# Dave-he/unet-watermark

Hardware: AMD Instinct MI355X
Metric: train_images_per_sec (higher is better)
Workload: dtype f32 storage and accumulation; the convolution products of the encoder and decoder layers (3x3, 7x7 stem, stride-2 and 1x1 layers: forward, data gradients, and the weight gradients of the stride-1 3x3 layers and the stem) as fp16x3 splits - every fp32 operand = two fp16 halves (22 mantissa bits), a*b; 1 GPU; Unet-resnet34 512x512 bs16/GPU train step: fwd + Dice + bwd + Adam (BASELINE.json configs[1]); global_batch=16, parallelism=dp1, grad_allreduce=none

## Files before the change

### include/uwm.h

```cpp
#ifndef UWM_H
#define UWM_H
#include <stddef.h>
#include <stdint.h>

#ifdef __cplusplus
extern "C" {
#endif

typedef struct uwm_model* uwm_handle;
typedef void* uwm_stream;

enum { UWM_ENC_RESNET18 = 18, UWM_ENC_RESNET34 = 34, UWM_ENC_RESNET50 = 50,
       UWM_ENC_EFFICIENTNET_B0 = 100, UWM_ENC_EFFICIENTNET_B1 = 101, UWM_ENC_EFFICIENTNET_B2 = 102,
       UWM_ENC_EFFICIENTNET_B3 = 103, UWM_ENC_EFFICIENTNET_B4 = 104, UWM_ENC_EFFICIENTNET_B5 = 105,
       UWM_ENC_EFFICIENTNET_B6 = 106, UWM_ENC_EFFICIENTNET_B7 = 107 };
enum { UWM_ARCH_UNET = 0, UWM_ARCH_UNETPLUSPLUS = 1 };
enum { UWM_T_F32 = 0, UWM_T_I64 = 1, UWM_T_U8 = 2, UWM_T_I32 = 3 };
enum { UWM_KIND_CONV_W = 0, UWM_KIND_BIAS = 1, UWM_KIND_BN_GAMMA = 2, UWM_KIND_BN_BETA = 3,
       UWM_KIND_BN_MEAN = 4, UWM_KIND_BN_VAR = 5 };
enum { UWM_ARENA_PARAM = 0, UWM_ARENA_BUFFER = 1 };
enum { UWM_PREC_F32 = 0, UWM_PREC_BF16X3 = 1, UWM_PREC_BF16X3_ALL = 2, UWM_PREC_F16X3 = 3, UWM_PREC_F16X3_ALL = 4,
       UWM_PREC_F16X1 = 5, UWM_PREC_F16X3_BWD2 = 6 };

typedef struct {
// ... 49 lines not shown

size_t uwm_predict_workspace_bytes(uwm_handle h, int N, int H, int W, int with_logits);
int  uwm_predict_u8(uwm_handle h, const uint8_t* images, const float* mean, const float* std, float threshold,
                    int apply_sigmoid, int out_h, int out_w, uint8_t* mask, float* logits, void* workspace,
                    size_t workspace_bytes, int N, int H, int W, uwm_stream stream);

typedef struct { long long offset; int h, w; } uwm_image_desc;
enum { UWM_INTER_NEAREST = 0, UWM_INTER_LINEAR = 1 };
int  uwm_resize_u8(const uint8_t* src, size_t src_bytes, const uwm_image_desc* descs, int N, int C, int H, int W, int interp,
                   uint8_t* out, uwm_stream stream);
int  uwm_op_resize_norm_u8_nhwc4(const uint8_t* src, size_t src_bytes, const uwm_image_desc* descs, int N, int C, int H, int W,
                                 const float* mean, const float* std, float* out, uwm_stream stream);
int  uwm_resize_threshold_ragged(const float* logits, int ld, int N, int h, int w, const uwm_image_desc* out_descs, float threshold,
                                 int apply_sigmoid, uint8_t* mask, size_t mask_bytes, uwm_stream stream);
int  uwm_predict_images_u8(uwm_handle h, const uint8_t* src, size_t src_bytes, const uwm_image_desc* in_descs, const float* mean,
                           const float* std, float threshold, int apply_sigmoid, const uwm_image_desc* out_descs, uint8_t* mask,
                           size_t mask_bytes, float* logits, void* workspace, size_t workspace_bytes, int N, int H, int W,
                           uwm_stream stream);

int  uwm_backward(uwm_handle h, const float* dlogits, void* workspace, int stage_begin, int stage_end,
                  uwm_stream stream);

int  uwm_loss(const float* logits, int ld, const void* target, int target_dtype, long long npix,
              float w_dice, float w_bce, float smooth, float eps, void* scratch, float* loss_out,
              float* dlogits, int ldd, float grad_scale, uwm_stream stream);

int  uwm_loss_sums(const float* logits, int ld, const void* target, int target_dtype, long long npix, void* scratch,
                   uwm_stream stream);
int  uwm_loss_apply(const float* logits, int ld, const void* target, int target_dtype, long long npix, long long npix_total,
                    float w_dice, float w_bce, float smooth, float eps, const void* scratch, float* loss_out,
                    float* dlogits, int ldd, float grad_scale, uwm_stream stream);

int  uwm_stats(const float* logits, int ld, const void* target, int target_dtype, int N, long long hw,
               float threshold, int apply_sigmoid, long long* out, uwm_stream stream);
int  uwm_threshold(const float* logits, int ld, long long npix, float threshold, int apply_sigmoid,
                   uint8_t* mask, uwm_stream stream);

int  uwm_adam(float* p, const float* g, float* m, float* v, long long n, float lr, float beta1, float beta2,
              float eps, float weight_decay, long long step, float grad_scale, uwm_stream stream);
int  uwm_adam_clip(float* p, const float* g, float* m, float* v, long long n, float lr, float beta1, float beta2,
                   float eps, float weight_decay, long long step, float grad_scale, float max_norm, void* scratch,
                   uwm_stream stream);
int  uwm_adam_graph(float* p, const float* g, float* m, float* v, long long n, float* hyper, void* clip_scratch,
                    uwm_stream stream);
int  uwm_adamw(float* p, const float* g, float* m, float* v, long long n, float lr, float beta1, float beta2,
               float eps, float weight_decay, long long step, float grad_scale, uwm_stream stream);
int  uwm_adamw_clip(float* p, const float* g, float* m, float* v, long long n, float lr, float beta1, float beta2,
                    float eps, float weight_decay, long long step, float grad_scale, float max_norm, void* scratch,
                    uwm_stream stream);
int  uwm_adamw_graph(float* p, const float* g, float* m, float* v, long long n, float* hyper, void* clip_scratch,
                     uwm_stream stream);
int  uwm_sgd(float* p, const float* g, float* buf, long long n, float lr, float momentum, float weight_decay,
             long long step, float grad_scale, float max_norm, void* scratch, uwm_stream stream);
int  uwm_scale(float* p, long long n, float s, uwm_stream stream);
int  uwm_set_join_stream(uwm_handle h, uwm_stream stream);
int  uwm_allreduce_grads(uwm_handle h, void* nccl_comm, int stage_begin, int stage_end, uwm_stream stream);
float* uwm_grad_arena(uwm_handle h);
int  uwm_preprocess_u8(const uint8_t* images, int N, int H, int W, int C, const float* mean, const float* std,
                       const int* flags, float* out_nchw, uwm_stream stream);
int  uwm_preprocess_mask_u8(const uint8_t* masks, int N, int H, int W, int threshold, const int* flags, uint8_t* out,
                            uwm_stream stream);
typedef struct {
  int flags;
  int hue, sat, val;
  double minv[6];
  unsigned char lut[256];
} uwm_aug_desc;
int  uwm_augment_u8(const uint8_t* images, const uint8_t* masks, const uwm_aug_desc* descs, int N, int H, int W, int C,
                    const float* mean, const float* std, int mask_threshold, float* out_nchw, uint8_t* out_masks, uint8_t* out_u8,
                    uwm_stream stream);
int  uwm_set_winograd(int on);
int  uwm_set_winograd_mode(uwm_handle h, int mode);
int  uwm_get_winograd_mode(uwm_handle h);
int  uwm_set_precision(uwm_handle h, int mode);
int  uwm_get_precision(uwm_handle h);
int  uwm_set_precision_fill(uwm_handle h, int min_workgroups);
int  uwm_set_routing_batch(uwm_handle h, int batch);
int  uwm_routing_enable(uwm_handle h, int on);
long long uwm_routing_dump(uwm_handle h, char* buf, long long cap, int clear);
int  uwm_set_drop_connect(uwm_handle h, const float* rowscale);
int  uwm_op_depthwise(int mode, const float* a, const float* b, int k, int stride, int pad_begin, int N, int H, int W, int C,
                      int Ho, int Wo, const float* addend, float* out, float* scratch, uwm_stream stream);
long long uwm_op_depthwise_scratch_floats(int k, int N, int C, int Ho, int Wo);
int  uwm_op_swish(const float* y, const float* scale, const float* shift, long long npix, int C, float* out, uwm_stream stream);
int  uwm_op_swish_pool(const float* y, const float* scale, const float* shift, int N, long long hw, int C, float* act_out,
                       float* pool, float* part, uwm_stream stream);
int  uwm_op_se_reduce(const float* a, const float* b, int N, long long hw, int C, float mult, float* out, float* part,
                      uwm_stream stream);
long long uwm_op_se_scratch_floats(int N, int C);
int  uwm_op_se_fc(const float* pool, const float* w1, const float* b1, int K1pad, const float* w2, const float* b2, int K2pad,
                  int N, int C, int nsq, float* hpre, float* hid, float* s, uwm_stream stream);
int  uwm_op_se_fc_backward(float* gs, const float* s, const float* hpre, const float* pool, const float* w1, int K1pad,
                           const float* w2, int K2pad, int N, int C, int nsq, float* gpool, float* acc1, float* gw1, float* gb1,
                           float* gw2, float* gb2, uwm_stream stream);
int  uwm_op_se_scale(const float* a, const float* s, int N, long long hw, int C, float* out, uwm_stream stream);
int  uwm_op_mb_out(const float* y, const float* scale, const float* shift, const float* rowscale, const float* id, int N,
                   long long hw, int C, float* out, uwm_stream stream);
int  uwm_op_rowscale(const float* g, const float* rowscale, int N, long long hw, int C, float* out, uwm_stream stream);
int  uwm_op_bn_stats(const float* y, long long npix, int C, const float* gamma, const float* beta, float eps, float momentum,
                     int update_running, float* run_mean, float* run_var, double* sums2c, float* mean, float* rstd,
                     float* scale, float* shift, uwm_stream stream);
int  uwm_num_mbconv_blocks(uwm_handle h);
float uwm_mbconv_drop_rate(uwm_handle h, int block);
int  uwm_resize_threshold(const float* logits, int ld, int N, int h, int w, int H, int W, float threshold,
                          int apply_sigmoid, uint8_t* mask, float* resized, uwm_stream stream);

enum { UWM_MASK_WATERMARK = 0, UWM_MASK_TEXT = 1, UWM_MASK_MIXED = 2 };
enum { UWM_MORPH_RECT = 0, UWM_MORPH_ELLIPSE = 2 };
int    uwm_mask_element(int shape, int kw, int kh, uint8_t* out);
size_t uwm_mask_workspace_bytes(int N, int H, int W);
int    uwm_optimize_mask(const uint8_t* in, uint8_t* out, int N, int H, int W, int mask_type, long long* summary,
                         void* workspace, size_t workspace_bytes, uwm_stream stream);
int    uwm_op_morph(const uint8_t* in, uint8_t* out, int N, int H, int W, int dilate, int shape, int kw, int kh,
                    int iterations, void* workspace, size_t workspace_bytes, uwm_stream stream);
int    uwm_op_components(const uint8_t* in, int32_t* labels ,
                         int32_t* areas , int N, int H, int W,
                         void* workspace, size_t workspace_bytes, uwm_stream stream);

int  uwm_set_side_stream(uwm_handle h, int on);

int  uwm_prof_enable(int on);
int  uwm_prof_collect(double* out, int max_classes);
const char* uwm_prof_class_name(int cls);

int  uwm_debug_lookup(uwm_handle h, const char* key, long long* offset, long long* count);

typedef struct {
  const float* ptr; const float* scale; const float* shift;
  int C, H, W, up, relu;
} uwm_src;
int  uwm_op_preprocess_u8_nhwc4(const uint8_t* images, long long npix, int C, const float* mean, const float* std, float* out,
                                uwm_stream stream);
int  uwm_op_set_igemm_f16x3(int on);
int  uwm_op_conv(const uwm_src* s0, const uwm_src* s1, const float* w, int wrows, int Kpad, int kh, int kw, int stride,
                 int pad, int N, int Cout, const float* bias, float* y, double* stats, int cfg, uwm_stream stream);
int  uwm_op_dgrad(const float* dy, int N, int Ho, int Wo, int Cout, const float* wd, int Cin, int KpadD, int kh, int kw,
                  int stride, int pad, int H, int W, const float* addend, const float* mask, const float* mscale,
                  const float* mshift, float* dx, uwm_stream stream);
int  uwm_op_wgrad(const uwm_src* s0, const uwm_src* s1, const float* dy, int N, int Ho, int Wo, int Cout, int wrows,
                  int Kpad, int kh, int kw, int stride, int pad, float* dw, int force_igemm, uwm_stream stream);
int  uwm_op_pack_dgrad(const float* w, int Cout, int Kpad, int ntaps, int Cin, float* wd, int KpadD, int CoutP,
                       uwm_stream stream);
int  uwm_op_maxpool(const uwm_src* in, int N, float* out, uint8_t* idx, uwm_stream stream);
int  uwm_op_maxpool_backward(const float* gout, const uint8_t* idx, const float* addend, const uwm_src* in, int N,
                             float* gin, uwm_stream stream);
int  uwm_op_bn_backward(const float* g, const float* y, const float* mean, const float* rstd, const float* gamma,
                        double* scratch2c, float* dy, float* dgamma, float* dbeta, long long npix, int C, uwm_stream stream);
int  uwm_op_bn_backward_act(const float* g, const float* y, const float* mean, const float* rstd, const float* gamma,
                            const float* scale, const float* shift, const float* se_s, const float* gpool, int N, long long hw,
                            int C, double* scratch2c, float* dy, float* dgamma, float* dbeta, float* xmax, uwm_stream stream);
int  uwm_op_dgrad_upsplit(const float* dy, int N, int H, int W, int Cout, const float* wd, int C0, int C1, int KpadD,
                          float* gprev, const float* pmask, const float* pscale, const float* pshift, float* gskip,
                          uwm_stream stream);
int  uwm_op_upsplit(const float* dcat, int N, int H, int W, int C0, int C1, float* gprev, const float* pmask,
                    const float* pscale, const float* pshift, float* gskip, uwm_stream stream);
int  uwm_op_residual(const float* y, const float* s2, const float* b2, const float* id, const float* sd, const float* bd,
                     float* out, long long npix, int C, uwm_stream stream);

#ifdef __cplusplus
}
#endif
#endif
```

### unet-watermark_amd/_lib.py

```python
from __future__ import annotations

import ctypes as C
import os
import subprocess
import sys
from pathlib import Path

os.environ.setdefault("GPU_MAX_HW_QUEUES", "8")

_PKG_DIR = Path(__file__).resolve().parent
_CSRC = _PKG_DIR / "csrc"
LIB_PATH = _PKG_DIR / "libuwm.so"
SOURCES = ["uwm_route.hip", "conv_igemm.hip", "conv_patch.hip", "conv_patch16.hip", "conv_wino.hip", "conv_wino8.hip", "conv_wino_x3.hip", "conv_f16x3.hip", "conv_f16x3v2.hip", "conv_stem_f16x3.hip", "conv_up2.hip", "conv_up2_f16.hip", "conv_c16_f16.hip", "conv_gemm.hip", "conv_head.hip", "mbconv.hip", "wgrad_igemm.hip", "wgrad_patch.hip", "wgrad_wino.hip", "wgrad_f16x3.hip", "wgrad_c16.hip", "wgrad_gemm.hip", "wgrad_stem.hip", "elementwise.hip", "loss.hip", "mask_post.hip", "resize_u8.hip", "augment_u8.hip", "uwm_model.hip"]
HIP_ARCH = "gfx950"
EXTRA_FLAGS = {name: ["-Xclang", "-target-feature", "-Xclang", "-packed-fp32-ops"]
               for name in ("conv_f16x3.hip", "conv_f16x3v2.hip", "wgrad_f16x3.hip", "conv_stem_f16x3.hip")}


class uwm_unet_desc(C.Structure):
    _fields_ = [("encoder", C.c_int), ("in_channels", C.c_int), ("classes", C.c_int),
                ("decoder_channels", C.c_int * 5), ("bn_eps", C.c_float), ("bn_momentum", C.c_float), ("arch", C.c_int)]


class uwm_tensor_info(C.Structure):
    _fields_ = [("name", C.c_char * 96), ("kind", C.c_int), ("arena", C.c_int), ("ndim", C.c_int),
                ("offset", C.c_longlong), ("shape", C.c_longlong * 4), ("stride", C.c_longlong * 4)]


class uwm_src(C.Structure):
    _fields_ = [("ptr", C.c_void_p), ("scale", C.c_void_p), ("shift", C.c_void_p),
                ("C", C.c_int), ("H", C.c_int), ("W", C.c_int), ("up", C.c_int), ("relu", C.c_int)]


KIND_CONV_W, KIND_BIAS, KIND_BN_GAMMA, KIND_BN_BETA, KIND_BN_MEAN, KIND_BN_VAR = range(6)
ARENA_PARAM, ARENA_BUFFER = 0, 1
ENC = {"resnet18": 18, "resnet34": 34, "resnet50": 50, **{f"efficientnet-b{i}": 100 + i for i in range(8)}}
ARCH = {"Unet": 0, "UnetPlusPlus": 1}
PREC = {"f32": 0, "bf16x3": 1, "bf16x3_all": 2, "f16x3": 3, "f16x3_all": 4, "f16x1": 5, "f16x3_bwd2": 6}
P, I, L, F, Z = C.c_void_p, C.c_int, C.c_longlong, C.c_float, C.c_size_t

SIGNATURES = {
    "uwm_last_error": (C.c_char_p, []),
    "uwm_version": (I, []),
    "uwm_create": (I, [C.POINTER(uwm_unet_desc), C.POINTER(P)]),
    "uwm_destroy": (None, [P]),
    "uwm_param_arena_floats": (L, [P]),
    "uwm_buffer_arena_floats": (L, [P]),
    "uwm_param_count": (L, [P]),
    "uwm_num_tensors": (I, [P]),
    "uwm_tensor_info_get": (I, [P, I, C.POINTER(uwm_tensor_info)]),
    "uwm_logits_channels": (I, [P]),
    "uwm_num_stages": (I, [P]),
    "uwm_stage_range": (I, [P, I, C.POINTER(L), C.POINTER(L)]),
    "uwm_bind": (I, [P, P, P, P]),
    "uwm_workspace_bytes": (Z, [P, I, I, I, I]),
    "uwm_conv_flops": (I, [P, I, I, C.POINTER(C.c_double), C.POINTER(C.c_double)]),
    "uwm_forward": (I, [P, P, P, P, Z, I, I, I, I, P]),
    "uwm_backward": (I, [P, P, P, I, I, P]),
    "uwm_frozen_bytes": (Z, [P]),
    "uwm_freeze": (I, [P, P, Z, I, I, I, P]),
    "uwm_unfreeze": (I, [P]),
    "uwm_is_frozen": (I, [P]),
    "uwm_frozen_serves": (I, [P, I, I, I]),
    "uwm_prep_launches": (L, [P]),
    "uwm_predict_workspace_bytes": (Z, [P, I, I, I, I]),
    "uwm_predict_u8": (I, [P, P, C.POINTER(C.c_float), C.POINTER(C.c_float), F, I, I, I, P, P, P, Z, I, I, I, P]),
    "uwm_resize_u8": (I, [P, Z, P, I, I, I, I, I, P, P]),
    "uwm_op_resize_norm_u8_nhwc4": (I, [P, Z, P, I, I, I, I, C.POINTER(C.c_float), C.POINTER(C.c_float), P, P]),
    "uwm_resize_threshold_ragged": (I, [P, I, I, I, I, P, F, I, P, Z, P]),
    "uwm_predict_images_u8": (I, [P, P, Z, P, C.POINTER(C.c_float), C.POINTER(C.c_float), F, I, P, P, Z, P, P, Z, I, I, I, P]),
    "uwm_op_preprocess_u8_nhwc4": (I, [P, L, I, C.POINTER(C.c_float), C.POINTER(C.c_float), P, P]),
    "uwm_loss": (I, [P, I, P, I, L, F, F, F, F, P, P, P, I, F, P]),
    "uwm_loss_sums": (I, [P, I, P, I, L, P, P]),
    "uwm_loss_apply": (I, [P, I, P, I, L, L, F, F, F, F, P, P, P, I, F, P]),
    "uwm_stats": (I, [P, I, P, I, I, L, F, I, P, P]),
    "uwm_threshold": (I, [P, I, L, F, I, P, P]),
    "uwm_adam": (I, [P, P, P, P, L, F, F, F, F, F, L, F, P]),
    "uwm_adam_clip": (I, [P, P, P, P, L, F, F, F, F, F, L, F, F, P, P]),
    "uwm_adam_graph": (I, [P, P, P, P, L, P, P, P]),
    "uwm_adamw": (I, [P, P, P, P, L, F, F, F, F, F, L, F, P]),
    "uwm_adamw_clip": (I, [P, P, P, P, L, F, F, F, F, F, L, F, F, P, P]),
    "uwm_adamw_graph": (I, [P, P, P, P, L, P, P, P]),
    "uwm_sgd": (I, [P, P, P, L, F, F, F, L, F, F, P, P]),
    "uwm_scale": (I, [P, L, F, P]),
    "uwm_set_winograd": (I, [I]),
    "uwm_set_winograd_mode": (I, [P, I]),
    "uwm_get_winograd_mode": (I, [P]),
    "uwm_set_precision": (I, [P, I]),
    "uwm_get_precision": (I, [P]),
    "uwm_set_precision_fill": (I, [P, I]),
    "uwm_set_routing_batch": (I, [P, I]),
    "uwm_routing_enable": (I, [P, I]),
    "uwm_routing_dump": (L, [P, C.c_char_p, L, I]),
    "uwm_allreduce_grads": (I, [P, P, I, I, P]),
    "uwm_grad_arena": (P, [P]),
    "uwm_set_join_stream": (I, [P, P]),
    "uwm_set_drop_connect": (I, [P, P]),
    "uwm_op_depthwise": (I, [I, P, P, I, I, I, I, I, I, I, I, I, P, P, P, P]),
    "uwm_op_depthwise_scratch_floats": (L, [I, I, I, I, I]),
    "uwm_op_swish": (I, [P, P, P, L, I, P, P]),
    "uwm_op_swish_pool": (I, [P, P, P, I, L, I, P, P, P, P]),
    "uwm_op_se_reduce": (I, [P, P, I, L, I, F, P, P, P]),
    "uwm_op_se_scratch_floats": (L, [I, I]),
    "uwm_op_se_fc": (I, [P, P, P, I, P, P, I, I, I, I, P, P, P, P]),
    "uwm_op_se_fc_backward": (I, [P, P, P, P, P, I, P, I, I, I, I, P, P, P, P, P, P, P]),
    "uwm_op_se_scale": (I, [P, P, I, L, I, P, P]),
    "uwm_op_mb_out": (I, [P, P, P, P, P, I, L, I, P, P]),
    "uwm_op_rowscale": (I, [P, P, I, L, I, P, P]),
    "uwm_op_bn_stats": (I, [P, L, I, P, P, F, F, I, P, P, P, P, P, P, P, P]),
    "uwm_num_mbconv_blocks": (I, [P]),
    "uwm_mbconv_drop_rate": (F, [P, I]),
    "uwm_preprocess_u8": (I, [P, I, I, I, I, C.POINTER(C.c_float), C.POINTER(C.c_float), P, P, P]),
    "uwm_preprocess_mask_u8": (I, [P, I, I, I, I, P, P, P]),
    "uwm_augment_u8": (I, [P, P, P, I, I, I, I, C.POINTER(C.c_float), C.POINTER(C.c_float), I, P, P, P, P]),
    "uwm_resize_threshold": (I, [P, I, I, I, I, I, I, F, I, P, P, P]),
    "uwm_mask_element": (I, [I, I, I, P]),
    "uwm_mask_workspace_bytes": (Z, [I, I, I]),
    "uwm_optimize_mask": (I, [P, P, I, I, I, I, P, P, Z, P]),
    "uwm_op_morph": (I, [P, P, I, I, I, I, I, I, I, I, P, Z, P]),
    "uwm_op_components": (I, [P, P, P, I, I, I, P, Z, P]),
    "uwm_set_side_stream": (I, [P, I]),
    "uwm_prof_enable": (I, [I]),
    "uwm_prof_collect": (I, [C.POINTER(C.c_double), I]),
    "uwm_prof_class_name": (C.c_char_p, [I]),
    "uwm_debug_lookup": (I, [P, C.c_char_p, C.POINTER(L), C.POINTER(L)]),
    "uwm_op_set_igemm_f16x3": (I, [I]),
    "uwm_op_conv": (I, [C.POINTER(uwm_src), C.POINTER(uwm_src), P, I, I, I, I, I, I, I, I, P, P, P, I, P]),
    "uwm_op_dgrad": (I, [P, I, I, I, I, P, I, I, I, I, I, I, I, I, P, P, P, P, P, P]),
    "uwm_op_wgrad": (I, [C.POINTER(uwm_src), C.POINTER(uwm_src), P, I, I, I, I, I, I, I, I, I, I, P, I, P]),
    "uwm_op_pack_dgrad": (I, [P, I, I, I, I, P, I, I, P]),
    "uwm_op_maxpool": (I, [C.POINTER(uwm_src), I, P, P, P]),
    "uwm_op_maxpool_backward": (I, [P, P, P, C.POINTER(uwm_src), I, P, P]),
    "uwm_op_bn_backward": (I, [P, P, P, P, P, P, P, P, P, L, I, P]),
    "uwm_op_bn_backward_act": (I, [P, P, P, P, P, P, P, P, P, I, L, I, P, P, P, P, P, P]),
    "uwm_op_dgrad_upsplit": (I, [P, I, I, I, I, P, I, I, I, P, P, P, P, P, P]),
    "uwm_op_upsplit": (I, [P, I, I, I, I, I, P, P, P, P, P, P]),
    "uwm_op_residual": (I, [P, P, P, P, P, P, P, L, I, P]),
}

_lib = None


def build_library(force: bool = False, verbose: bool = False) -> Path:
    srcs = [_CSRC / s for s in SOURCES]
    hdrs = [_CSRC / "uwm_kernels.h", _PKG_DIR.parent / "include" / "uwm.h"] + sorted(_CSRC.glob("*.inc"))
    if LIB_PATH.exists() and not force:
        newest = max(p.stat().st_mtime for p in srcs + hdrs)
        if LIB_PATH.stat().st_mtime >= newest:
            return LIB_PATH
    hipcc = os.environ.get("HIPCC", "/opt/rocm/bin/hipcc")
    objdir = _PKG_DIR / "build"
    objdir.mkdir(exist_ok=True)
    procs = []
    hdr_m = max(p.stat().st_mtime for p in hdrs + [Path(__file__)])
    for s in srcs:
        o = objdir / (s.stem + ".o")
        if not force and o.exists() and o.stat().st_mtime >= max(s.stat().st_mtime, hdr_m):
            procs.append((None, None, o))
            continue
        cmd = [hipcc, f"--offload-arch={HIP_ARCH}", "-O3", "-std=c++17", "-fPIC"] + EXTRA_FLAGS.get(s.name, []) + ["-c", str(s), "-o", str(o)]
        procs.append((cmd, subprocess.Popen(cmd, stdout=subprocess.PIPE, stderr=subprocess.STDOUT), o))
    objs = []
    for cmd, p, o in procs:
        if p is None:
            objs.append(str(o))
            continue
        out, _ = p.communicate()
        if p.returncode != 0:
            raise RuntimeError(f"hipcc failed: {' '.join(cmd)}\n{out.decode(errors='replace')}")
        if verbose and out:
            sys.stderr.write(out.decode(errors="replace"))
        objs.append(str(o))
    cmd = [hipcc, f"--offload-arch={HIP_ARCH}", "-shared", "-fPIC", "-o", str(LIB_PATH)] + objs
    r = subprocess.run(cmd, stdout=subprocess.PIPE, stderr=subprocess.STDOUT)
    if r.returncode != 0:
        raise RuntimeError(f"link failed: {' '.join(cmd)}\n{r.stdout.decode(errors='replace')}")
    return LIB_PATH


def lib():
    global _lib
    if _lib is not None:
        return _lib
    global LIB_PATH
    if os.environ.get("UWM_LIB"):
        LIB_PATH = Path(os.environ["UWM_LIB"])
    if not LIB_PATH.exists():
        raise RuntimeError(
            f"{LIB_PATH} not found: the HIP extension is not built. Run `python -c 'import __graft_entry__ as g; "
            f"g.build()'` (needs hipcc). There is no CPU fallback for this path.")
    try:
        h = C.CDLL(str(LIB_PATH))
    except OSError as e:
        raise RuntimeError(f"cannot load {LIB_PATH}: {e}") from e
    for name, (res, args) in SIGNATURES.items():
        fn = getattr(h, name)
        fn.restype = res
        fn.argtypes = args
    _lib = h
    return _lib


def check(rc: int, exc=RuntimeError):
    if rc != 0:
        msg = lib().uwm_last_error().decode(errors="replace")
        raise exc(msg)


def stream_ptr(device=None) -> int:
    import torch
    return torch.cuda.current_stream(device).cuda_stream


class _NoGuard:
    def __enter__(self):
        return self

    def __exit__(self, *a):
        return False


_NOGUARD = _NoGuard()


def on_device(t):
    import torch
    if t.device.type == "cuda" and t.device.index is not None and t.device.index != torch.cuda.current_device():
        return torch.cuda.device(t.device)
    return _NOGUARD


_DT = None


def target_dtype_code(t) -> int:
    import torch
    global _DT
    if _DT is None:
        _DT = {torch.float32: 0, torch.int64: 1, torch.uint8: 2, torch.int32: 3, torch.bool: 2}
    if t.dtype not in _DT:
        raise TypeError(f"unsupported target dtype {t.dtype}")
    return _DT[t.dtype]
```

### unet-watermark_amd/csrc/conv_head.hip

```cpp
#include "uwm_kernels.h"

namespace uwm {

typedef float f4 __attribute__((ext_vector_type(4)));

constexpr int kHeadTH = 4;
template <int CQ, int NCO, int TH = kHeadTH>
__global__ __launch_bounds__(256, 3) void conv_head_kernel(const ConvArgs a, int tilesW, int tilesH, int ntiles) {
  constexpr int C = CQ * 4, COLS = 256 / CQ, PW = COLS + 2;
  constexpr int NV = (TH + 2) * PW * CQ, NR = (NV + 255) / 256;
  extern __shared__ __attribute__((aligned(16))) float smem[];
  f4* const ws = (f4*)smem;
  f4* const xs0 = ws + NCO * 9 * CQ;
  for (int i = threadIdx.x; i < NCO * 9 * CQ; i += 256) {
    const int co = i / (9 * CQ), r = i - co * 9 * CQ;
    ws[i] = co < a.wrows ? *(const f4*)(a.w + (size_t)co * a.Kpad + r * 4) : (f4){0.f, 0.f, 0.f, 0.f};
  }
  const int H = a.Ho, W = a.Wo;
  const bool lazy = a.s0.scale != nullptr;
  const int relu = a.s0.relu;
  static_assert(256 % CQ == 0, "a thread stages ONE channel quad");
  const int q = threadIdx.x % CQ, col = threadIdx.x / CQ;
  f4 lsc = {1.f, 1.f, 1.f, 1.f}, lsh = {0.f, 0.f, 0.f, 0.f};
  if (lazy) { lsc = *(const f4*)(a.s0.scale + q * 4); lsh = *(const f4*)(a.s0.shift + q * 4); }
  int srow[NR], spx[NR];
#pragma unroll
  for (int rd = 0; rd < NR; ++rd) {
    const int it = rd * 256 + threadIdx.x;
    srow[rd] = it / (PW * CQ); spx[rd] = (it - srow[rd] * (PW * CQ)) / CQ;
  }
  f4 pv[NR]; unsigned pok = 0;
  auto tile_origin = [&](int t, int& n, int& ho0, int& w0) {
    const int tw = t % tilesW; t /= tilesW;
    const int th = t % tilesH; n = t / tilesH;
    ho0 = th * TH; w0 = tw * COLS;
  };
  auto tile_load = [&](int t) {
    int n, ho0, w0; tile_origin(t, n, ho0, w0);
    const float* xn = a.s0.ptr + (size_t)n * H * W * C + q * 4;
    pok = 0;
#pragma unroll
    for (int rd = 0; rd < NR; ++rd) {
      const int hi = ho0 - 1 + srow[rd], wi = w0 - 1 + spx[rd];
      const bool ok = (rd * 256 + (int)threadIdx.x) < NV && hi >= 0 && hi < H && wi >= 0 && wi < W;
      const int hc = min(max(hi, 0), H - 1), wc = min(max(wi, 0), W - 1);
      pv[rd] = *(const f4*)(xn + ((size_t)hc * W + wc) * C);
      pok |= (ok ? 1u : 0u) << rd;
    }
  };
  auto tile_store = [&](int buf) {
    f4* const xb = xs0 + buf * NV;
#pragma unroll
    for (int rd = 0; rd < NR; ++rd) {
      f4 v = pv[rd];
      if (lazy) {
        v = v * lsc + lsh;
        if (relu) { v.x = fmaxf(v.x, 0.f); v.y = fmaxf(v.y, 0.f); v.z = fmaxf(v.z, 0.f); v.w = fmaxf(v.w, 0.f); }
      }
      if (!((pok >> rd) & 1u)) v = (f4){0.f, 0.f, 0.f, 0.f};
      if (rd * 256 + (int)threadIdx.x < NV) xb[rd * 256 + threadIdx.x] = v;
    }
  };
  int t = blockIdx.x;
  tile_load(t);
  tile_store(0);
  __syncthreads();
  f4 wr[NCO == 1 ? 9 : 1];
  if (NCO == 1) {
#pragma unroll
    for (int k = 0; k < 9; ++k) wr[k] = ws[k * CQ + q];
  }
  for (int it = 0; t < ntiles; ++it, t += gridDim.x) {
    const int cur = it & 1;
    const int tn = t + (int)gridDim.x;
    tile_load(tn < ntiles ? tn : t);
    int n, ho0, w0; tile_origin(t, n, ho0, w0);
    const f4* const xs = xs0 + cur * NV;
    f4 res[TH];
#pragma unroll
    for (int j = 0; j < TH; ++j) res[j] = (f4){0.f, 0.f, 0.f, 0.f};
#pragma unroll 1
    for (int co = 0; co < NCO; ++co) {
      float acc[TH];
#pragma unroll
      for (int j = 0; j < TH; ++j) acc[j] = 0.f;
      const f4* const wc = ws + co * 9 * CQ + q;
#pragma unroll
      for (int rr = 0; rr < TH + 2; ++rr)
#pragma unroll
        for (int s_ = 0; s_ < 3; ++s_) {
          const f4 v = xs[(rr * PW + col + s_) * CQ + q];
#pragma unroll
          for (int j = 0; j < TH; ++j) {
            const int r = rr - j;
            if (r >= 0 && r < 3) {
              const f4 wv = NCO == 1 ? wr[r * 3 + s_] : wc[(r * 3 + s_) * CQ];
              acc[j] += v.x * wv.x + v.y * wv.y + v.z * wv.z + v.w * wv.w;
            }
          }
        }
      const float b = (a.bias && co < a.wrows) ? a.bias[co] : 0.f;
#pragma unroll
      for (int j = 0; j < TH; ++j) {
        float v = acc[j];
#pragma unroll
        for (int d = 1; d < CQ; d <<= 1) v += __shfl_xor(v, d);
        v += b;
        if (co == 0) res[j].x = v; else if (co == 1) res[j].y = v; else if (co == 2) res[j].z = v; else res[j].w = v;
      }
    }
    const int wo = w0 + col;
    if (wo < W) {
#pragma unroll
      for (int j = 0; j < TH; ++j) {
        const int ho = ho0 + j;
        if ((j % CQ) == q && ho < H) *(f4*)(a.out + (((size_t)n * H + ho) * W + wo) * 4) = res[j];
      }
    }
    tile_store(cur ^ 1);
    __syncthreads();
  }
}

constexpr int kHeadDTH = 8;
template <int CQ, int NCO, int TH = kHeadDTH>
__global__ __launch_bounds__(256, TH >= 8 ? 2 : (TH >= 4 ? 3 : 4)) void conv_head_dgrad_kernel(const ConvArgs a) {
  constexpr int C = CQ * 4, COLS = 256 / CQ, PW = COLS + 2;
  __shared__ f4 ws[9 * NCO * CQ];
  __shared__ float gs[(TH + 2) * PW * NCO];
  for (int i = threadIdx.x; i < 9 * NCO * CQ; i += 256) {
    const int q = i % CQ, tc = i / CQ, co = tc % NCO, tap = tc / NCO;
    f4 v;
    v.x = a.w[(size_t)(q * 4 + 0) * a.Kpad + tap * 4 + co]; v.y = a.w[(size_t)(q * 4 + 1) * a.Kpad + tap * 4 + co];
    v.z = a.w[(size_t)(q * 4 + 2) * a.Kpad + tap * 4 + co]; v.w = a.w[(size_t)(q * 4 + 3) * a.Kpad + tap * 4 + co];
    ws[i] = v;
  }
  const int H = a.Ho, W = a.Wo;
  const int n = blockIdx.z, ho0 = blockIdx.y * TH, w0 = blockIdx.x * COLS;
  const float* gn = a.s0.ptr + (size_t)n * H * W * 4;
  for (int i = threadIdx.x; i < (TH + 2) * PW * NCO; i += 256) {
    const int co = i % NCO, px = i / NCO, row = px / PW, cx = px - row * PW;
    const int hh = ho0 - 1 + row, ww = w0 - 1 + cx;
    gs[i] = (hh >= 0 && hh < H && ww >= 0 && ww < W) ? gn[((size_t)hh * W + ww) * 4 + co] : 0.f;
  }
  __syncthreads();
  const int col = threadIdx.x / CQ, q = threadIdx.x % CQ;
  const int wo = w0 + col;
  const bool live = wo < W;
  f4 mk[TH];
#pragma unroll
  for (int j = 0; j < TH; ++j) {
    const size_t o = (((size_t)n * H + min(ho0 + j, H - 1)) * W + min(wo, W - 1)) * C + q * 4;
    mk[j] = a.mask ? *(const f4*)(a.mask + o) : (f4){0.f, 0.f, 0.f, 0.f};
  }
  f4 acc[TH];
#pragma unroll
  for (int j = 0; j < TH; ++j) acc[j] = (f4){0.f, 0.f, 0.f, 0.f};
#pragma unroll 1
  for (int co = 0; co < NCO; ++co) {
    const f4* const wc = ws + co * CQ + q;
    const float* const gc = gs + col * NCO + co;
#pragma unroll
    for (int rr = 0; rr < TH + 2; ++rr)
#pragma unroll
      for (int s2 = 0; s2 < 3; ++s2) {
        const float gv = gc[(rr * PW + s2) * NCO];
#pragma unroll
        for (int j = 0; j < TH; ++j) {
          const int r = j + 2 - rr;
          if (r >= 0 && r < 3) acc[j] += wc[(r * 3 + (2 - s2)) * NCO * CQ] * gv;
        }
      }
  }
  const bool bnb = a.bnb_mean != nullptr;
  f4 ps_ = {0.f, 0.f, 0.f, 0.f}, pq_ = {0.f, 0.f, 0.f, 0.f}, bmu = ps_, brs = ps_, msc = {1.f, 1.f, 1.f, 1.f}, msh = ps_;
  if (bnb) { bmu = *(const f4*)(a.bnb_mean + q * 4); brs = *(const f4*)(a.bnb_rstd + q * 4); }
  if (a.mask && a.mscale) { msc = *(const f4*)(a.mscale + q * 4); msh = *(const f4*)(a.mshift + q * 4); }
#pragma unroll
  for (int j = 0; j < TH; ++j) {
    const int ho = ho0 + j;
    if (ho >= H || !live) continue;
    const size_t o = (((size_t)n * H + ho) * W + wo) * C + q * 4;
    f4 v = acc[j];
    if (a.addend) v += *(const f4*)(a.addend + o);
    if (a.mask) {
      const f4 yr = mk[j];
      const f4 m = yr * msc + msh;
      v.x = m.x > 0.f ? v.x : 0.f; v.y = m.y > 0.f ? v.y : 0.f; v.z = m.z > 0.f ? v.z : 0.f; v.w = m.w > 0.f ? v.w : 0.f;
      if (bnb) { ps_ += v; pq_ += v * ((yr - bmu) * brs); }
    }
    *(f4*)(a.out + o) = v;
  }
  if (bnb) {
    float v8[8] = {ps_.x, ps_.y, ps_.z, ps_.w, pq_.x, pq_.y, pq_.z, pq_.w};
#pragma unroll
    for (int i = 0; i < 8; ++i)
#pragma unroll
      for (int d = CQ; d < 64; d <<= 1) v8[i] += __shfl_xor(v8[i], d);
    __shared__ float red[4][CQ * 8];
    const int lane = threadIdx.x & 63, wave = threadIdx.x >> 6;
    if (lane < CQ) {
#pragma unroll
      for (int i = 0; i < 8; ++i) red[wave][lane * 8 + i] = v8[i];
    }
    __syncthreads();
    if (threadIdx.x < CQ * 8) {
      const int qq = threadIdx.x / 8, e = threadIdx.x % 8;
      const double sacc = ((double)red[0][threadIdx.x] + (double)red[1][threadIdx.x]) + ((double)red[2][threadIdx.x] + (double)red[3][threadIdx.x]);
      const unsigned wg = blockIdx.x + gridDim.x * (blockIdx.y + gridDim.y * blockIdx.z);
      const size_t srep_off = a.srep > 1 ? (size_t)(wg & (unsigned)(a.srep - 1)) * a.sstride : 0;
      if (e < 4) atomicAdd(a.ssum + srep_off + qq * 4 + e, sacc); else atomicAdd(a.ssq + srep_off + qq * 4 + (e - 4), sacc);
    }
  }
}

bool conv_head_dgrad_applicable(const ConvArgs& a) {
  return a.ntaps == 9 && a.kw == 3 && a.smul == 1 && a.sdiv == 1 && a.rmul == -1 && a.off == 1 && a.Ctot == 4 && a.C0 == 4 && a.s0.C == 4 &&
         (a.Cout == 8 || a.Cout == 16 || a.Cout == 32) && a.wrows == a.Cout && a.s0.up == 0 && !a.s0.scale && a.Ho == a.Hl && a.Wo == a.Wl &&
         (!a.ssum || a.bnb_mean) && !a.bias && !a.out_up;
}
template <int CQ>
static hipError_t launch_head_dgrad(const ConvArgs& a, hipStream_t st) {
  const dim3 g((unsigned)((a.Wo + 256 / CQ - 1) / (256 / CQ)), (unsigned)((a.Ho + kHeadDTH - 1) / kHeadDTH), (unsigned)a.N);
  if (a.live_ch == 1) UWM_LAUNCH(30, a.flops, a.bytes, (conv_head_dgrad_kernel<CQ, 1>), g, dim3(256), 0, st, a);
  else UWM_LAUNCH(30, a.flops, a.bytes, (conv_head_dgrad_kernel<CQ, 4>), g, dim3(256), 0, st, a);
  return hipGetLastError();
}
hipError_t launch_conv_head_dgrad(const ConvArgs& a, hipStream_t st) {
  if (!conv_head_dgrad_applicable(a)) return hipErrorInvalidValue;
  switch (a.Cout) {
    case 8: return launch_head_dgrad<2>(a, st);
    case 16: return launch_head_dgrad<4>(a, st);
    default: return launch_head_dgrad<8>(a, st);
  }
}

bool conv_head_applicable(const ConvArgs& a) {
  return a.ntaps == 9 && a.kw == 3 && a.smul == 1 && a.sdiv == 1 && a.rmul == 1 && a.off == -1 && a.Cout == 4 && a.wrows >= 1 && a.wrows <= 4 &&
         (a.Ctot == 8 || a.Ctot == 16 || a.Ctot == 32) && a.C0 == a.Ctot && a.s0.C == a.Ctot && a.s0.up == 0 && a.Ho == a.Hl && a.Wo == a.Wl &&
         !a.ssum && !a.addend && !a.mask && !a.out_up;
}

template <int CQ, int NCO>
static hipError_t launch_head_(const ConvArgs& a, hipStream_t st) {
  constexpr int COLS = 256 / CQ, TH = kHeadTH;
  const size_t lds = sizeof(float) * 4 * ((size_t)NCO * 9 * CQ + (size_t)2 * (TH + 2) * (COLS + 2) * CQ);
  static DevOnce lds_attr;
  { hipError_t e = lds_attr.set_max_lds((const void*)conv_head_kernel<CQ, NCO>, lds); if (e != hipSuccess) return e; }
  const int tilesW = (a.Wo + COLS - 1) / COLS, tilesH = (a.Ho + TH - 1) / TH;
  const long ntiles = (long)a.N * tilesH * tilesW;
  static const int per_cu = dbg_int("UWM_HEADF_WGS", 3);
  const long cap = (long)per_cu * device_cu_count();
  UWM_LAUNCH(30, a.flops, a.bytes, (conv_head_kernel<CQ, NCO>), dim3((unsigned)(ntiles < cap ? ntiles : cap)), dim3(256), lds, st, a, tilesW, tilesH, (int)ntiles);
  return hipGetLastError();
}
template <int CQ>
static hipError_t launch_head(const ConvArgs& a, hipStream_t st) {
  return a.wrows == 1 ? launch_head_<CQ, 1>(a, st) : launch_head_<CQ, 4>(a, st);
}

hipError_t launch_conv_head(const ConvArgs& a, hipStream_t st) {
  if (!conv_head_applicable(a)) return hipErrorInvalidValue;
  switch (a.Ctot) {
    case 8: return launch_head<2>(a, st);
    case 16: return launch_head<4>(a, st);
    default: return launch_head<8>(a, st);
  }
}

}
```

### unet-watermark_amd/csrc/elementwise.hip

```cpp
#include "uwm_kernels.h"
#include <vector>
#include <mutex>
#include <cstdlib>

namespace uwm {

typedef float f4 __attribute__((ext_vector_type(4)));
static constexpr int kMaxBlocks = 256 * 8;

static inline unsigned nblocks(size_t work, int per_block) {
  size_t b = (work + per_block - 1) / per_block;
  if (b > (size_t)kMaxBlocks) b = kMaxBlocks;
  if (b < 1) b = 1;
  return (unsigned)b;
}

__global__ void nchw_to_nhwc4_kernel(const float* __restrict__ x, float* __restrict__ y, int C, size_t HW,
                                     size_t total, int CP) {
  for (size_t i = blockIdx.x * (size_t)blockDim.x + threadIdx.x; i < total; i += (size_t)gridDim.x * blockDim.x) {
    const size_t n = i / HW, p = i - n * HW;
    const float* xp = x + n * C * HW + p;
    float* yp = y + i * CP;
    for (int c0 = 0; c0 < CP; c0 += 4) {
      f4 v;
// ... 145 lines not shown
      }
    }
    *(f4*)(out + i * 4) = best;
    if (idx) *(uchar4*)(idx + i * 4) = make_uchar4((unsigned char)bi[0], (unsigned char)bi[1], (unsigned char)bi[2], (unsigned char)bi[3]);
  }
}
hipError_t launch_maxpool_fwd(const Src& in, float* out, uint8_t* idx, int N, int Ho, int Wo, hipStream_t st) {
  const size_t total = (size_t)N * Ho * Wo * (in.C / 4);
  hipLaunchKernelGGL(maxpool_fwd_kernel, dim3(nblocks(total, 256)), dim3(256), 0, st, in, out, idx, Ho, Wo, total);
  return hipGetLastError();
}

__global__ __launch_bounds__(256) void maxpool_bwd_kernel(const float* __restrict__ gout, const uint8_t* __restrict__ idx,
                                   const float* __restrict__ addend, const Src in, float* __restrict__ gin, int Ho,
                                   int Wo, size_t total, const float* __restrict__ bn_mean, const float* __restrict__ bn_rstd,
                                   double* ssum, double* ssq, int srep, int sstride) {
  const int C4 = in.C / 4;
  f4 sg = {0.f, 0.f, 0.f, 0.f}, sgy = {0.f, 0.f, 0.f, 0.f};
  for (size_t i = blockIdx.x * (size_t)blockDim.x + threadIdx.x; i < total; i += (size_t)gridDim.x * blockDim.x) {
    const int c = (int)(i % C4) * 4;
    size_t p = i / C4;
    const int w = (int)(p % in.W); p /= in.W;
    const int h = (int)(p % in.H); const int n = (int)(p / in.H);
    f4 g = addend ? *(const f4*)(addend + i * 4) : (f4){0.f, 0.f, 0.f, 0.f};
    const int ho0 = h >> 1, ho1 = (h + 1) >> 1, wo0 = w >> 1, wo1 = (w + 1) >> 1;
    for (int a = 0; a < 2; ++a) {
      const int ho = a ? ho1 : ho0;
      if ((a && ho1 == ho0) || ho >= Ho) continue;
      const int r = h - (2 * ho - 1);
      for (int b = 0; b < 2; ++b) {
        const int wo = b ? wo1 : wo0;
        if ((b && wo1 == wo0) || wo >= Wo) continue;
        const int s = w - (2 * wo - 1);
        const size_t o = ((size_t)((size_t)n * Ho + ho) * Wo + wo) * in.C + c;
        const uchar4 id = *(const uchar4*)(idx + o);
        const f4 go = *(const f4*)(gout + o);
        const int t = r * 3 + s;
        if (id.x == t) g.x += go.x;
        if (id.y == t) g.y += go.y;
        if (id.z == t) g.z += go.z;
        if (id.w == t) g.w += go.w;
      }
    }
    if (in.scale && in.relu) {
      const f4 yr = *(const f4*)(in.ptr + i * 4);
      const f4 z = yr * *(const f4*)(in.scale + c) + *(const f4*)(in.shift + c);
      g.x = z.x > 0.f ? g.x : 0.f; g.y = z.y > 0.f ? g.y : 0.f; g.z = z.z > 0.f ? g.z : 0.f; g.w = z.w > 0.f ? g.w : 0.f;
      if (bn_mean) { sg += g; sgy += g * (yr - *(const f4*)(bn_mean + c)); }
    }
    *(f4*)(gin + i * 4) = g;
  }
  if (bn_mean) {
    __shared__ float red[256 * 8];
    const int c = (int)(threadIdx.x % C4) * 4;
    sgy = sgy * *(const f4*)(bn_rstd + c);
    float* r = red + threadIdx.x * 8;
    r[0] = sg.x; r[1] = sg.y; r[2] = sg.z; r[3] = sg.w; r[4] = sgy.x; r[5] = sgy.y; r[6] = sgy.z; r[7] = sgy.w;
    __syncthreads();
    const size_t srep_off = srep > 1 ? (size_t)(blockIdx.x & (unsigned)(srep - 1)) * sstride : 0;
    const int tr = 256 / C4;
    for (int t = threadIdx.x; t < C4 * 8; t += 256) {
      const int q = t / 8, e = t % 8;
      double acc = 0.0;
      for (int k = 0; k < tr; ++k) acc += (double)red[(k * C4 + q) * 8 + e];
      if (e < 4) atomicAdd(ssum + srep_off + q * 4 + e, acc); else atomicAdd(ssq + srep_off + q * 4 + (e - 4), acc);
    }
  }
}
hipError_t launch_maxpool_bwd(const float* gout, const uint8_t* idx, const float* addend, const Src& in, float* gin,
                              int N, int Ho, int Wo, hipStream_t st, const float* bn_mean, const float* bn_rstd, double* ssum,
                              double* ssq, int srep, int sstride) {
  const size_t total = (size_t)N * in.H * in.W * (in.C / 4);
  if (bn_mean && (!bn_rstd || !ssum || !ssq || !in.scale || !in.relu || (in.C & 3) || 256 % (in.C / 4))) return hipErrorInvalidValue;
  hipLaunchKernelGGL(maxpool_bwd_kernel, dim3(nblocks(total, 256)), dim3(256), 0, st, gout, idx, addend, in, gin, Ho,
                     Wo, total, bn_mean, bn_rstd, ssum, ssq, srep, sstride);
  return hipGetLastError();
}

__global__ __launch_bounds__(256) void bn_bwd_reduce_kernel(const float* __restrict__ g, const float* __restrict__ y,
                                                            const float* __restrict__ mean, const float* __restrict__ rstd,
                                                            double* dgamma, double* dbeta, size_t npix, int C, int CW) {
  __shared__ float red[256 * 8];
  const int c0 = blockIdx.y * CW;
  const int tc = CW / 4;
  const int tr = 256 / tc;
  const int cx = threadIdx.x % tc, rx = threadIdx.x / tc;
  const int c = c0 + cx * 4;
  f4 sg = {0, 0, 0, 0}, sgy = {0, 0, 0, 0};
  if (rx < tr) {
    const f4 mu = *(const f4*)(mean + c), rs = *(const f4*)(rstd + c);
    const size_t ps = (size_t)gridDim.x * tr;
    size_t p = (size_t)blockIdx.x * tr + rx;
    f4 s2 = {0, 0, 0, 0};
    for (; p + 3 * ps < npix; p += 4 * ps) {
      const f4 g0 = *(const f4*)(g + p * C + c), g1 = *(const f4*)(g + (p + ps) * C + c), g2 = *(const f4*)(g + (p + 2 * ps) * C + c),
               g3 = *(const f4*)(g + (p + 3 * ps) * C + c);
      const f4 y0 = *(const f4*)(y + p * C + c), y1 = *(const f4*)(y + (p + ps) * C + c), y2 = *(const f4*)(y + (p + 2 * ps) * C + c),
               y3 = *(const f4*)(y + (p + 3 * ps) * C + c);
      sg += (g0 + g1) + (g2 + g3);
      s2 += (g0 * (y0 - mu) + g1 * (y1 - mu)) + (g2 * (y2 - mu) + g3 * (y3 - mu));
    }
    for (; p < npix; p += ps) {
      const f4 gv = *(const f4*)(g + p * C + c);
      sg += gv; s2 += gv * (*(const f4*)(y + p * C + c) - mu);
    }
    sgy = s2 * rs;
  }
  float* r = red + threadIdx.x * 8;
  r[0] = sg.x; r[1] = sg.y; r[2] = sg.z; r[3] = sg.w; r[4] = sgy.x; r[5] = sgy.y; r[6] = sgy.z; r[7] = sgy.w;
  __syncthreads();
  for (int t = threadIdx.x; t < tc * 8; t += 256) {
    const int q = t / 8, e = t % 8;
    double s = 0.0;
    for (int k = 0; k < tr; ++k) s += (double)red[(k * tc + q) * 8 + e];
    if (e < 4) atomicAdd(dbeta + c0 + q * 4 + e, s); else atomicAdd(dgamma + c0 + q * 4 + (e - 4), s);
  }
}
hipError_t launch_bn_bwd_reduce(const float* g, const float* y, const float* mean, const float* rstd, double* dgamma,
                                double* dbeta, size_t npix, int C, hipStream_t st) {
  int CW = 0;
  for (int d = 1; d <= C && !CW; ++d) if (C % d == 0 && C / d <= 1024 && (C / d) % 4 == 0) CW = C / d;
  if (!CW) return hipErrorInvalidValue;
  const int tr = 256 / (CW / 4);
  unsigned nb = nblocks(npix, tr * 8);
  hipLaunchKernelGGL(bn_bwd_reduce_kernel, dim3(nb, C / CW), dim3(256), 0, st, g, y, mean, rstd, dgamma, dbeta, npix, C, CW);
  return hipGetLastError();
}

__global__ __launch_bounds__(256, 6) void bn_bwd_apply_kernel(const float* __restrict__ g, const float* __restrict__ y, const float* __restrict__ mean,
                                    const float* __restrict__ rstd, const float* __restrict__ gamma,
                                    const double* __restrict__ dgamma, const double* __restrict__ dbeta, float* __restrict__ dy,
                                    float* gamma_grad, float* beta_grad, size_t n4, int C, float invM,
                                    const double* __restrict__ rep, int nrep, int rep_stride, float* xmax) {
  __shared__ double part[256 * 4];
  __shared__ float wmax[4];
  float amax = 0.f;
  const size_t stride = (size_t)gridDim.x * blockDim.x;
  size_t i = blockIdx.x * (size_t)blockDim.x + threadIdx.x;
  const int Q = C >> 2;
  const int c = (int)((i * 4) % (size_t)C);
  f4 g0, g1, g2, g3, y0, y1, y2, y3;
  bool full = i + 3 * stride < n4;
  if (full) {
    g0 = *(const f4*)(g + i * 4); g1 = *(const f4*)(g + (i + stride) * 4); g2 = *(const f4*)(g + (i + 2 * stride) * 4); g3 = *(const f4*)(g + (i + 3 * stride) * 4);
    y0 = *(const f4*)(y + i * 4); y1 = *(const f4*)(y + (i + stride) * 4); y2 = *(const f4*)(y + (i + 2 * stride) * 4); y3 = *(const f4*)(y + (i + 3 * stride) * 4);
  }
  const f4 mu = *(const f4*)(mean + c), rs = *(const f4*)(rstd + c), gm = *(const f4*)(gamma + c);
  f4 dbq, dgq;
  {
    double sq[4];
#pragma unroll
    for (int half = 0; half < 2; ++half) {
      if (rep) {
        const int nq = Q < 256 ? Q : 256, L = 256 / nq;
        const int q0 = (int)(((size_t)blockIdx.x * 256) % (size_t)Q);
        const int j = threadIdx.x % nq, l = threadIdx.x / nq;
        if (half) __syncthreads();
        if (l < L) {
          const int cj = ((q0 + j) % Q) * 4 + half * C;
          double b0 = 0, b1 = 0, b2 = 0, b3 = 0;
          for (int r = l; r < nrep; r += L) {
            const double* pr = rep + (size_t)r * rep_stride + cj;
            b0 += pr[0]; b1 += pr[1]; b2 += pr[2]; b3 += pr[3];
          }
          double* o = part + (l * nq + j) * 4;
          o[0] = b0; o[1] = b1; o[2] = b2; o[3] = b3;
        }
        __syncthreads();
#pragma unroll
        for (int e = 0; e < 4; ++e) sq[e] = 0.0;
        for (int k = 0; k < L; ++k) {
          const double* o = part + (k * nq + j) * 4;
#pragma unroll
          for (int e = 0; e < 4; ++e) sq[e] += o[e];
        }
      } else {
        const double* src = half ? dgamma : dbeta;
#pragma unroll
        for (int e = 0; e < 4; ++e) sq[e] = src[c + e];
      }
      float* gout = half ? gamma_grad : beta_grad;
      if (gout && i < (size_t)Q) {
#pragma unroll
        for (int e = 0; e < 4; ++e) gout[c + e] = (float)sq[e];
      }
      f4 q4; q4.x = (float)sq[0] * invM; q4.y = (float)sq[1] * invM; q4.z = (float)sq[2] * invM; q4.w = (float)sq[3] * invM;
      if (half) dgq = q4; else dbq = q4;
    }
  }
  if (i >= n4 && !xmax) return;
  const f4 dg = dgq, db = dbq;
  const f4 A = gm * rs, B = -(gm * rs * rs * dg), K = -(A * db) - B * mu;
  auto amax4 = [&](const f4& v) { amax = fmaxf(fmaxf(amax, fmaxf(fabsf(v.x), fabsf(v.y))), fmaxf(fabsf(v.z), fabsf(v.w))); };
  while (full) {
    g0 = A * g0 + B * y0 + K; g1 = A * g1 + B * y1 + K; g2 = A * g2 + B * y2 + K; g3 = A * g3 + B * y3 + K;
    if (xmax) { amax4(g0); amax4(g1); amax4(g2); amax4(g3); }
    *(f4*)(dy + i * 4) = g0;
    *(f4*)(dy + (i + stride) * 4) = g1;
    *(f4*)(dy + (i + 2 * stride) * 4) = g2;
    *(f4*)(dy + (i + 3 * stride) * 4) = g3;
    i += 4 * stride;
    full = i + 3 * stride < n4;
    if (full) {
      g0 = *(const f4*)(g + i * 4); g1 = *(const f4*)(g + (i + stride) * 4); g2 = *(const f4*)(g + (i + 2 * stride) * 4); g3 = *(const f4*)(g + (i + 3 * stride) * 4);
      y0 = *(const f4*)(y + i * 4); y1 = *(const f4*)(y + (i + stride) * 4); y2 = *(const f4*)(y + (i + 2 * stride) * 4); y3 = *(const f4*)(y + (i + 3 * stride) * 4);
    }
  }
  for (; i < n4; i += stride) {
    const f4 o = A * *(const f4*)(g + i * 4) + B * *(const f4*)(y + i * 4) + K;
    if (xmax) amax4(o);
    *(f4*)(dy + i * 4) = o;
  }
  if (xmax) {
#pragma unroll
    for (int d = 32; d >= 1; d >>= 1) amax = fmaxf(amax, __shfl_xor(amax, d));
    if ((threadIdx.x & 63) == 0) wmax[threadIdx.x >> 6] = amax;
    __syncthreads();
    if (threadIdx.x == 0) {
      const float mx = fmaxf(fmaxf(wmax[0], wmax[1]), fmaxf(wmax[2], wmax[3]));
      if (mx > 0.f) atomicMax((unsigned*)xmax + (blockIdx.x & 31), __float_as_uint(mx));
    }
  }
}
hipError_t launch_bn_bwd_apply(const float* g, const float* y, const float* mean, const float* rstd, const float* gamma,
                               const double* dgamma, const double* dbeta, float* dy, float* gamma_grad, float* beta_grad,
                               size_t npix, int C, hipStream_t st, const double* rep, int nrep, int rep_stride, hipEvent_t done, float* xmax) {
  const size_t n4 = npix * C / 4;
  unsigned nb = nblocks(n4, 256 * 4);
  const unsigned q = (unsigned)(C / 4);
  unsigned unit = q;
  { unsigned a = q, b = 256; while (b) { unsigned t = a % b; a = b; b = t; } unit = q / a; }
  nb = ((nb + unit - 1) / unit) * unit;
  if ((size_t)nb * 256 < q) nb = ((q + 255) / 256 + unit - 1) / unit * unit;
  if (done)
    hipExtLaunchKernelGGL(bn_bwd_apply_kernel, dim3(nb), dim3(256), 0, st, nullptr, done, 0, g, y, mean, rstd, gamma, dgamma,
                          dbeta, dy, gamma_grad, beta_grad, n4, C, (float)(1.0 / (double)npix), rep, rep ? (nrep < 1 ? 1 : nrep) : 0, rep_stride, xmax);
  else
    hipLaunchKernelGGL(bn_bwd_apply_kernel, dim3(nb), dim3(256), 0, st, g, y, mean, rstd, gamma, dgamma,
                       dbeta, dy, gamma_grad, beta_grad, n4, C, (float)(1.0 / (double)npix), rep, rep ? (nrep < 1 ? 1 : nrep) : 0, rep_stride, xmax);
  return hipGetLastError();
}

__global__ void upsplit_prev_kernel(const float* __restrict__ dcat, int H, int W, int C0, int Ct, float* __restrict__ gprev,
                                    const float* __restrict__ pmask, const float* __restrict__ pscale,
                                    const float* __restrict__ pshift, size_t total, int accumulate) {
  const int C4 = C0 / 4, H2 = H / 2, W2 = W / 2;
  for (size_t i = blockIdx.x * (size_t)blockDim.x + threadIdx.x; i < total; i += (size_t)gridDim.x * blockDim.x) {
    const int c = (int)(i % C4) * 4;
    size_t p = i / C4;
    const int w2 = (int)(p % W2); p /= W2;
    const int h2 = (int)(p % H2); const int n = (int)(p / H2);
    const float* b = dcat + ((size_t)((size_t)n * H + 2 * h2) * W + 2 * w2) * Ct + c;
    f4 g = *(const f4*)b + *(const f4*)(b + Ct) + *(const f4*)(b + (size_t)W * Ct) + *(const f4*)(b + (size_t)W * Ct + Ct);
    if (pmask) {
      f4 z = *(const f4*)(pmask + i * 4);
      if (pscale) z = z * *(const f4*)(pscale + c) + *(const f4*)(pshift + c);
      g.x = z.x > 0.f ? g.x : 0.f; g.y = z.y > 0.f ? g.y : 0.f; g.z = z.z > 0.f ? g.z : 0.f; g.w = z.w > 0.f ? g.w : 0.f;
    }
    if (accumulate) g += *(const f4*)(gprev + i * 4);
    *(f4*)(gprev + i * 4) = g;
  }
}
__global__ void upsplit_skip_kernel(const float* __restrict__ dcat, int C0, int C1, float* __restrict__ gskip, size_t total) {
  const int C4 = C1 / 4, Ct = C0 + C1;
  for (size_t i = blockIdx.x * (size_t)blockDim.x + threadIdx.x; i < total; i += (size_t)gridDim.x * blockDim.x) {
    const int c = (int)(i % C4) * 4;
    const size_t p = i / C4;
    *(f4*)(gskip + i * 4) = *(const f4*)(dcat + p * Ct + C0 + c);
  }
}
hipError_t launch_upsplit(const float* dcat, int N, int H, int W, int C0, int C1, float* gprev, const float* pmask,
                          const float* pscale, const float* pshift, float* gskip, hipStream_t st, int accumulate_prev) {
  const size_t t0 = (size_t)N * (H / 2) * (W / 2) * (C0 / 4);
  hipLaunchKernelGGL(upsplit_prev_kernel, dim3(nblocks(t0, 256)), dim3(256), 0, st, dcat, H, W, C0, C0 + C1, gprev, pmask,
                     pscale, pshift, t0, accumulate_prev);
  if (C1 > 0 && gskip) {
    const size_t t1 = (size_t)N * H * W * (C1 / 4);
    hipLaunchKernelGGL(upsplit_skip_kernel, dim3(nblocks(t1, 256)), dim3(256), 0, st, dcat, C0, C1, gskip, t1);
  }
  return hipGetLastError();
}

__global__ void preprocess_u8_kernel(const uint8_t* __restrict__ img, int H, int W, int C, PreArgs pa,
                                     const int* __restrict__ flags, float* __restrict__ out, size_t total) {
  for (size_t i = blockIdx.x * (size_t)blockDim.x + threadIdx.x; i < total; i += (size_t)gridDim.x * blockDim.x) {
    const int x = (int)(i % W); size_t r = i / W;
    const int y = (int)(r % H); const int n = (int)(r / H);
    int sy, sx; aug_src(flags ? flags[n] : 0, H, W, y, x, sy, sx);
    const uint8_t* p = img + (((size_t)n * H + sy) * W + sx) * C;
    for (int c = 0; c < C; ++c) out[(((size_t)n * C + c) * H + y) * W + x] = pre_norm(p[c], pa.mul[c], pa.add[c]);
  }
}
template <int C>
__global__ __launch_bounds__(256) void preprocess_u8_nhwc4_kernel(const uint8_t* __restrict__ img, PreArgs pa, float* __restrict__ out,
                                                                  size_t npix) {
  __shared__ uint32_t raw[256 * C];
  const int t = threadIdx.x;
  const size_t p0 = (size_t)blockIdx.x * 1024, nbytes = npix * C, b0 = p0 * C;
  const uint32_t* src = (const uint32_t*)(img + b0);
#pragma unroll
  for (int i = 0; i < C; ++i) {
    const int d = t + 256 * i;
    const size_t b = b0 + 4 * (size_t)d;
    uint32_t v = 0u;
    if (b + 4 <= nbytes) v = __builtin_nontemporal_load(src + d);
    else
      for (int k = 0; k < 4; ++k) if (b + k < nbytes) v |= (uint32_t)img[b + k] << (8 * k);
    raw[d] = v;
  }
  __syncthreads();
  const uint8_t* rb = (const uint8_t*)raw;
#pragma unroll
  for (int k = 0; k < 4; ++k) {
    const int p = t + 256 * k;
    if (p0 + p < npix) {
      float v[4] = {0.f, 0.f, 0.f, 0.f};
#pragma unroll
      for (int c = 0; c < C; ++c) v[c] = pre_norm(rb[p * C + c], pa.mul[c], pa.add[c]);
      f4 o; o.x = v[0]; o.y = v[1]; o.z = v[2]; o.w = v[3];
      __builtin_nontemporal_store(o, (f4*)(out + (p0 + p) * 4));
    }
  }
}
__global__ void preprocess_mask_kernel(const uint8_t* __restrict__ m, int H, int W, int thr, const int* __restrict__ flags,
                                       uint8_t* __restrict__ out, size_t total) {
  for (size_t i = blockIdx.x * (size_t)blockDim.x + threadIdx.x; i < total; i += (size_t)gridDim.x * blockDim.x) {
    const int x = (int)(i % W); size_t r = i / W;
    const int y = (int)(r % H); const int n = (int)(r / H);
// ... 356 lines not shown
```

### unet-watermark_amd/csrc/uwm_abi.inc

```
extern "C" {

const char* uwm_last_error(void) { return g_err; }
int uwm_version(void) { return 1; }

int uwm_create(const uwm_unet_desc* desc, uwm_handle* out) {
  if (!desc || !out) return fail("uwm_create: null argument");
  uwm_model* m = new uwm_model();
  m->desc = *desc;
  if (m->desc.bn_eps <= 0.f) m->desc.bn_eps = 1e-5f;
  if (m->desc.bn_momentum <= 0.f) m->desc.bn_momentum = 0.1f;
  if (build_model(m)) { delete m; return 1; }
  const char* e = getenv("UWM_SIDE_STREAM");
  m->use_side = e ? atoi(e) : 1;
  if (const char* pe = getenv("UWM_PRECISION")) {
    static const char* names[7] = {"f32", "bf16x3", "bf16x3_all", "f16x3", "f16x3_all", "f16x1", "f16x3_bwd2"};
    int found = -1;
    for (int i = 0; i < 7; ++i) if (!strcmp(pe, names[i]) || (pe[0] == '0' + i && !pe[1])) found = i;
    if (found < 0) { delete m; return fail("uwm_create: UWM_PRECISION=%s is not a precision mode (f32 | bf16x3 | bf16x3_all | f16x3 | f16x3_all | f16x1 | f16x3_bwd2 or 0..6)", pe); }
    m->prec = found; m->plan.prec = found; m->prec_from_env = found != UWM_PREC_F32;
  }
  if (const char* pf = getenv("UWM_F16X3_MIN_WGS")) m->f3_min_wgs = atoi(pf) > 0 ? atoi(pf) : 0;
  m->wino_mode = winograd_mode();
  m->plan.wino_mode = m->wino_mode;
  *out = m; return 0;
// ... 683 lines not shown
  h->f3_min_wgs = min_workgroups; return 0;
}
int uwm_set_routing_batch(uwm_handle h, int batch) {
  if (!h || batch < 0 || batch > 255) return fail("uwm_set_routing_batch: batch must be 0 (= the real batch) .. 255");
  h->route_n = batch; return 0;
}
int uwm_routing_enable(uwm_handle h, int on) {
  if (!h) return fail("uwm_routing_enable: null handle");
  h->route_log_on = on != 0; if (!on) h->route_log.clear();
  return 0;
}
long long uwm_routing_dump(uwm_handle h, char* buf, long long cap, int clear) {
  if (!h) return -1;
  const long long need = (long long)h->route_log.size() + 1;
  if (buf && cap > 0) {
    const long long n = need <= cap ? need - 1 : cap - 1;
    memcpy(buf, h->route_log.data(), (size_t)n); buf[n] = 0;
  }
  if (clear) h->route_log.clear();
  return need;
}

typedef int (*nccl_allreduce_fn)(const void*, void*, size_t, int, int, void*, hipStream_t);
static nccl_allreduce_fn g_allreduce = nullptr;
static int resolve_rccl() {
  if (g_allreduce) return 0;
  void* sym = dlsym(RTLD_DEFAULT, "ncclAllReduce");
  if (!sym) {
    void* lib = dlopen("librccl.so.1", RTLD_NOW | RTLD_GLOBAL);
    if (!lib) lib = dlopen("librccl.so", RTLD_NOW | RTLD_GLOBAL);
    if (lib) sym = dlsym(lib, "ncclAllReduce");
  }
  if (!sym) return fail("uwm_allreduce_grads: ncclAllReduce not found (load RCCL in the host process first)");
  g_allreduce = (nccl_allreduce_fn)sym; return 0;
}
int uwm_allreduce_grads(uwm_handle h, void* comm, int sb, int se, uwm_stream stream) {
  if (!h || !comm) return fail("uwm_allreduce_grads: null argument");
  if (!h->grads) return fail("uwm_allreduce_grads: no gradient arena bound");
  if (sb < 0 || se > h->nstages || sb >= se) return fail("uwm_allreduce_grads: bad stage range [%d,%d)", sb, se);
  if (resolve_rccl()) return 1;
  DeviceGuard guard(h->device);
  for (int k = sb; k < se; ++k) {
    const long long b = h->stage_begin[k], e = h->stage_begin[k + 1];
    if (e <= b) continue;
    const int rc = g_allreduce(h->grads + b, h->grads + b, (size_t)(e - b),  7,  0, comm, (hipStream_t)stream);
    if (rc != 0) return fail("uwm_allreduce_grads: ncclAllReduce failed on bucket %d (ncclResult_t %d)", k, rc);
  }
  return 0;
}
float* uwm_grad_arena(uwm_handle h) { return h ? h->grads : nullptr; }
static Src to_src(const uwm_src* s) { return mk_src(s->ptr, s->C, s->H, s->W, s->scale, s->shift, s->relu, s->up); }

static int g_op_ig16 = 0;
static int op_ig_bank(const float* w, int rows, int Kpad, int slot, hipStream_t st, const float** bank) {
  static float* buf[2] = {nullptr, nullptr}; static size_t cap[2] = {0, 0};
  const size_t n = (size_t)rows * Kpad;
  if (n > cap[slot]) {
    if (buf[slot]) HIPCHK(hipFree(buf[slot]));
    buf[slot] = nullptr; cap[slot] = 0;
    HIPCHK(hipMalloc((void**)&buf[slot], n * sizeof(float)));
    cap[slot] = n;
  }
  WinoJobs jobs; memset(&jobs, 0, sizeof(jobs)); jobs.n = 1;
  jobs.j[0].w = w; jobs.j[0].ut = buf[slot]; jobs.j[0].rows = rows; jobs.j[0].Kpad = Kpad; jobs.j[0].mode = 3; jobs.j[0].src_rows = rows;
  LCHK(launch_f16x3_weights_multi(jobs, st));
  *bank = buf[slot];
  return 0;
}
int uwm_op_set_igemm_f16x3(int on) { g_op_ig16 = on == 2 ? 2 : (on != 0); return 0; }
int uwm_op_conv(const uwm_src* s0, const uwm_src* s1, const float* w, int wrows, int Kpad, int kh, int kw, int stride,
                int pad, int N, int Cout, const float* bias, float* y, double* stats, int cfg, uwm_stream stream) {
  if (!s0 || !w || !y) return fail("uwm_op_conv: null argument");
  ConvArgs a; memset(&a, 0, sizeof(a));
  a.s0 = to_src(s0); a.C0 = a.s0.C;
  if (s1) { a.s1 = to_src(s1); a.Ctot = a.C0 + a.s1.C; } else { a.s1 = a.s0; a.Ctot = a.C0; }
  a.Hl = a.s0.H << a.s0.up; a.Wl = a.s0.W << a.s0.up;
  a.w = w; a.wrows = wrows; a.Kpad = Kpad; a.ntaps = kh * kw; a.kw = kw;
  a.N = N; a.Ho = (a.Hl + 2 * pad - kh) / stride + 1; a.Wo = (a.Wl + 2 * pad - kw) / stride + 1;
  a.Cout = Cout; a.M = N * a.Ho * a.Wo;
  a.smul = stride; a.rmul = 1; a.off = -pad; a.sdiv = 1;
  a.out = y; a.bias = bias;
  if (stats) { a.ssum = stats; a.ssq = stats + Cout; }
  a.dv_ctot = make_fastdiv(a.Ctot); a.dv_kw = make_fastdiv(a.kw);
  a.ig16 = g_op_ig16 != 0;
  if (g_op_ig16 == 1 && !(Kpad & 31) && cfg < 6 && conv_route(a, cfg).k == kConvIgemm && op_ig_bank(w, wrows, Kpad, 0, (hipStream_t)stream, &a.wbank)) return 1;
  if (cfg == 610) {
    static float* sbuf = nullptr;
    if (!sbuf) HIPCHK(hipMalloc((void**)&sbuf, stem_f16x3_bank_floats() * sizeof(float)));
    if (kh != 7 || kw != 7 || a.Ctot != 4 || wrows != 64) return fail("uwm_op_conv: cfg 610 is the 7x7 stem (4 stored input channels, 64 outputs)");
    LCHK(launch_stem_f16x3_weights(w, Kpad, a.Ctot, sbuf, (hipStream_t)stream));
    a.wu = sbuf;
    LCHK(launch_conv_stem_f16x3(a, (hipStream_t)stream));
    return 0;
  }
  const bool reuse_bank = cfg >= 1600 && cfg <= 1607;
  if (reuse_bank) cfg -= 1000;
  if (cfg == 604 || cfg == 606) return fail("uwm_op_conv: cfg %d names a removed conv_f16x3v2 form (607 is its kernel)", reuse_bank ? cfg + 1000 : cfg);
  if (cfg >= 600 && cfg <= 607) {
    if (!op_wino_shape(a, kh, kw, stride, pad)) return fail("uwm_op_conv: cfg 600 (fp16x3) needs 3x3 s1 p1, Ho >= 8, Wo >= 16");
    if (op_f16x3_prepare(a, (hipStream_t)stream, cfg - 600, reuse_bank)) return 1;
  } else if (((cfg >= 300 && cfg < 500) || (cfg < 0 && winograd_mode() != 0)) && op_wino_shape(a, kh, kw, stride, pad)) {
    if (op_wino_prepare(a, 0, (hipStream_t)stream, cfg == 400)) return 1;
  } else if (cfg >= 300 && cfg < 500) return fail("uwm_op_conv: cfg 300 (Winograd) needs 3x3 s1 p1, channels %% 8 == 0, Ho >= 8, Wo >= 16");
  LCHK(launch_conv(a, (hipStream_t)stream, cfg));
  return 0;
}
int uwm_op_dgrad(const float* dy, int N, int Ho, int Wo, int Cout, const float* wd, int Cin, int KpadD, int kh, int kw,
                 int stride, int pad, int H, int W, const float* addend, const float* mask, const float* mscale,
                 const float* mshift, float* dx, uwm_stream stream) {
  if (!dy || !wd || !dx) return fail("uwm_op_dgrad: null argument");
  ConvArgs a; memset(&a, 0, sizeof(a));
  a.s0 = mk_src(dy, Cout, Ho, Wo); a.s1 = a.s0; a.C0 = Cout; a.Ctot = Cout;
  a.w = wd; a.wrows = Cin; a.Kpad = KpadD; a.ntaps = kh * kw; a.kw = kw;
  a.N = N; a.Ho = H; a.Wo = W; a.Cout = Cin; a.M = N * H * W;
  a.Hl = Ho; a.Wl = Wo; a.smul = 1; a.rmul = -1; a.off = pad; a.sdiv = stride;
  a.out = dx; a.addend = addend; a.mask = mask; a.mscale = mscale; a.mshift = mshift;
  a.dv_ctot = make_fastdiv(a.Ctot); a.dv_kw = make_fastdiv(a.kw);
  if (g_op_ig16) {
    static float* xm = nullptr;
    if (!xm) HIPCHK(hipMalloc((void**)&xm, 32 * sizeof(float)));
    LCHK(launch_absmax32(dy, (size_t)N * Ho * Wo * Cout, xm, (hipStream_t)stream));
    a.ig16 = 1; a.xmax = xm;
  }
  if (winograd_mode() != 0 && op_wino_shape(a, kh, kw, stride, pad) && op_wino_prepare(a, 1, (hipStream_t)stream)) return 1;
  if (g_op_ig16 == 1 && !(KpadD & 31)) {
    const ConvKernel k = conv_route(a, -1).k;
    if ((k == kConvIgemm || k == kConvS2Dgrad) && op_ig_bank(wd, Cin, KpadD, 0, (hipStream_t)stream, &a.wbank)) return 1;
  }
  LCHK(launch_conv(a, (hipStream_t)stream));
  return 0;
}
int uwm_op_dgrad_upsplit(const float* dy, int N, int H, int W, int Cout, const float* wd, int C0, int C1, int KpadD,
                         float* gprev, const float* pmask, const float* pscale, const float* pshift, float* gskip,
                         uwm_stream stream) {
  if (!dy || !wd || !gprev || (C1 > 0 && !gskip)) return fail("uwm_op_dgrad_upsplit: null argument");
  ConvArgs a; memset(&a, 0, sizeof(a));
  a.s0 = mk_src(dy, Cout, H, W); a.s1 = a.s0; a.C0 = Cout; a.Ctot = Cout;
  a.w = wd; a.wrows = C0 + C1; a.Kpad = KpadD; a.ntaps = 9; a.kw = 3;
  a.N = N; a.Ho = H; a.Wo = W; a.Cout = C0 + C1; a.M = N * H * W;
  a.Hl = H; a.Wl = W; a.smul = 1; a.rmul = -1; a.off = 1; a.sdiv = 1;
  a.out = gskip; a.out_up = gprev; a.up_c0 = C0; a.up_mask = pmask; a.up_mscale = pscale; a.up_mshift = pshift;
  a.dv_ctot = make_fastdiv(a.Ctot); a.dv_kw = make_fastdiv(a.kw);
  if (!op_wino_shape(a, 3, 3, 1, 1) || (H & 1) || (W & 1)) return fail("uwm_op_dgrad_upsplit: needs even H >= 8, W >= 16, channels %% 8 == 0");
  if (g_op_ig16) {
    static float* xm = nullptr;
    if (!xm) HIPCHK(hipMalloc((void**)&xm, 32 * sizeof(float)));
    LCHK(launch_absmax32(dy, (size_t)N * H * W * Cout, xm, (hipStream_t)stream));
    a.ig16 = 1; a.xmax = xm;
  }
  if (op_wino_prepare(a, 1, (hipStream_t)stream)) return 1;
  LCHK(launch_conv(a, (hipStream_t)stream));
  return 0;
}
int uwm_op_wgrad(const uwm_src* s0, const uwm_src* s1, const float* dy, int N, int Ho, int Wo, int Cout, int wrows, int Kpad,
                 int kh, int kw, int stride, int pad, float* dw, int force_igemm, uwm_stream stream) {
  if (!s0 || !dy || !dw) return fail("uwm_op_wgrad: null argument");
  WgradArgs a; memset(&a, 0, sizeof(a));
  a.s0 = to_src(s0); a.C0 = a.s0.C;
  if (s1) { a.s1 = to_src(s1); a.Ctot = a.C0 + a.s1.C; } else { a.s1 = a.s0; a.Ctot = a.C0; }
  a.dy = dy; a.dw = dw; a.wrows = wrows; a.Kpad = Kpad; a.ntaps = kh * kw; a.kw = kw;
  a.N = N; a.Ho = Ho; a.Wo = Wo; a.Cout = Cout; a.M = N * Ho * Wo;
  a.Hl = a.s0.H << a.s0.up; a.Wl = a.s0.W << a.s0.up; a.stride = stride; a.pad = pad;
  a.dv_ctot = make_fastdiv(a.Ctot); a.dv_kw = make_fastdiv(a.kw);
  a.force_igemm = force_igemm;
  if ((force_igemm & 0xff) == 6 || (force_igemm & 0xff) == 7) {
    static float* xm = nullptr;
    if (!xm) HIPCHK(hipMalloc((void**)&xm, 32 * sizeof(float)));
    LCHK(launch_absmax32(dy, (size_t)N * Ho * Wo * Cout, xm, (hipStream_t)stream));
    a.prec = 2; a.xmax = xm;
  }
  LCHK(launch_wgrad(a, (hipStream_t)stream));
  return 0;
}
int uwm_op_pack_dgrad(const float* w, int Cout, int Kpad, int ntaps, int Cin, float* wd, int KpadD, int CoutP,
                      uwm_stream stream) {
  if (!w || !wd) return fail("uwm_op_pack_dgrad: null argument");
  LCHK(launch_pack_dgrad(w, Cout, Kpad, ntaps, Cin, wd, KpadD, CoutP, (hipStream_t)stream));
  return 0;
}
int uwm_op_bn_backward(const float* g, const float* y, const float* mean, const float* rstd, const float* gamma,
                       double* scratch2c, float* dy, float* dgamma, float* dbeta, long long npix, int C, uwm_stream stream) {
  if (!g || !y || !mean || !rstd || !gamma || !scratch2c || !dy || !dgamma || !dbeta || npix < 1) return fail("uwm_op_bn_backward: bad argument");
  hipStream_t st = (hipStream_t)stream;
  HIPCHK(hipMemsetAsync(scratch2c, 0, 2 * (size_t)C * sizeof(double), st));
  LCHK(launch_bn_bwd_reduce(g, y, mean, rstd, scratch2c, scratch2c + C, (size_t)npix, C, st));
  LCHK(launch_bn_bwd_apply(g, y, mean, rstd, gamma, scratch2c, scratch2c + C, dy, dgamma, dbeta, (size_t)npix, C, st));
  return 0;
}
int uwm_op_bn_backward_act(const float* g, const float* y, const float* mean, const float* rstd, const float* gamma,
                           const float* scale, const float* shift, const float* se_s, const float* gpool, int N, long long hw,
                           int C, double* scratch2c, float* dy, float* dgamma, float* dbeta, float* xmax, uwm_stream stream) {
  if (!g || !y || !mean || !rstd || !gamma || !scale || !shift || !scratch2c || !dy || !dgamma || !dbeta || N < 1 || hw < 1 ||
      C < 4 || (C & 3) || (!se_s != !gpool))
    return fail("uwm_op_bn_backward_act: bad argument");
  hipStream_t st = (hipStream_t)stream;
  HIPCHK(hipMemsetAsync(scratch2c, 0, 2 * (size_t)C * sizeof(double), st));
  if (xmax) HIPCHK(hipMemsetAsync(xmax, 0, 32 * sizeof(float), st));
  LCHK(launch_bn_bwd_act(g, y, mean, rstd, gamma, scale, shift, se_s, gpool, N, (size_t)hw, scratch2c, scratch2c + C, dy, dgamma,
                         dbeta, C, st, xmax));
  return 0;
}
int uwm_op_upsplit(const float* dcat, int N, int H, int W, int C0, int C1, float* gprev, const float* pmask,
                   const float* pscale, const float* pshift, float* gskip, uwm_stream stream) {
  if (!dcat || !gprev) return fail("uwm_op_upsplit: null argument");
  LCHK(launch_upsplit(dcat, N, H, W, C0, C1, gprev, pmask, pscale, pshift, gskip, (hipStream_t)stream));
  return 0;
}
int uwm_op_residual(const float* y, const float* s2, const float* b2, const float* id, const float* sd, const float* bd,
                    float* out, long long npix, int C, uwm_stream stream) {
  if (!y || !s2 || !b2 || !id || !out) return fail("uwm_op_residual: null argument");
  LCHK(launch_residual(y, s2, b2, id, sd, bd, out, (size_t)npix, C, (hipStream_t)stream));
  return 0;
}
int uwm_op_maxpool_backward(const float* gout, const uint8_t* idx, const float* addend, const uwm_src* in, int N, float* gin,
                            uwm_stream stream) {
  if (!gout || !idx || !in || !gin) return fail("uwm_op_maxpool_backward: null argument");
  Src s = to_src(in);
  LCHK(launch_maxpool_bwd(gout, idx, addend, s, gin, N, (s.H - 1) / 2 + 1, (s.W - 1) / 2 + 1, (hipStream_t)stream));
  return 0;
}
int uwm_op_maxpool(const uwm_src* in, int N, float* out, uint8_t* idx, uwm_stream stream) {
  if (!in || !out) return fail("uwm_op_maxpool: null argument");
  Src s = to_src(in);
  LCHK(launch_maxpool_fwd(s, out, idx, N, (s.H - 1) / 2 + 1, (s.W - 1) / 2 + 1, (hipStream_t)stream));
  return 0;
}

}
```

### unet-watermark_amd/csrc/uwm_backward.inc

```
static int do_backward(uwm_model* m, const float* dlogits, float* ws, int sb, int se, hipStream_t st) {
  const Plan& p = m->plan;
  const int N = p.N, H = p.H, W = p.W;
  Ctx c{m, ws, st, N};
  c.wst = (m->use_side && m->side) ? m->side : st;
  const int h1 = H / 2, w1 = W / 2;
  int sh[4], sw[4];
  { int h = H / 4, w = W / 4; for (int s = 0; s < 4; ++s) { if (s > 0) { h /= 2; w /= 2; } sh[s] = h; sw[s] = w; } }
  std::vector<size_t> first_blk(4); { size_t b = 0; for (int s = 0; s < 4; ++s) { first_blk[s] = b; b += m->stages[s].size(); } }
  const bool effnet = !m->mb.empty();
  auto feat_blk = [&](int s) -> size_t { return effnet ? (size_t)m->feat_blk[s] : first_blk[s] + m->stages[s].size() - 1; };
  auto feat_src = [&](int s) {
    return mk_src(c.F(p.xn[feat_blk(s)]), m->featC[s], sh[s], sw[s]);
  };
  auto feat_mask = [&](const Src& f) -> const float* { return effnet ? nullptr : f.ptr; };
  Src f1 = effnet ? mk_src(c.F(p.stem_a), m->f1C, h1, w1) : lazy_src(c, m->stem, h1, w1);

  std::vector<char>& out_sums = m->out_sums;
  if (sb <= 0 || out_sums.size() != first_blk[3] + m->stages[3].size()) out_sums.assign(first_blk[3] + m->stages[3].size(), 0);
  if (sb <= 0 || m->dy_max_made.size() != m->bns.size()) m->dy_max_made.assign(m->bns.size(), 0);
  m->disp_cov.clear();
  if (sb <= 0) m->rq = ReduceQueue();
  if (sb <= 0 && se > 0) {
    HIPCHK(hipMemsetAsync(m->grads, 0, (size_t)m->param_floats * sizeof(float), st));
    HIPCHK(hipMemsetAsync(c.D(p.stat_d), 0, p.stat_d_count * sizeof(double), st));
    if (p.se_gs_floats) HIPCHK(hipMemsetAsync(c.F(p.se_gs_all), 0, p.se_gs_floats * sizeof(float), st));
    if (m->packed_in_fwd && m->pack_mode == pack_key(m)) {
      HIPCHK(hipStreamWaitEvent(st, m->ev_pack, 0));
      m->packed_in_fwd = false;
    } else {
      if (m->packed_in_fwd) { HIPCHK(hipStreamWaitEvent(st, m->ev_pack, 0)); m->packed_in_fwd = false; }
      for (size_t ci = 0; ci < m->convs.size(); ++ci) {
        const ConvL& cv = m->convs[ci];
        if (cv.dgrad && (!(cv.wud_off && p.wino_ok(ci)) || cv.CoutP == 16 || c16_f16_on(m, ci, true)))
          LCHK(launch_pack_dgrad(m->params + cv.w_off, cv.Cout, cv.Kpad, cv.k * cv.k, cv.CinP, c.F(cv.wd_off), cv.KpadD,
                                 cv.CoutP, st));
      }
      LCHK(wino_jobs(c, true, st));
    }
    const ConvL& hd = m->convs[m->head];
    const int last_c2 = m->nodes.empty() ? m->dec.back().c2 : m->nodes.back().c2;
    Src d4 = lazy_src(c, last_c2, H, W);
    LCHK(run_wgrad(c, m->head, d4, nullptr, dlogits, H, W));
    LCHK(launch_colsum(dlogits, (size_t)N * H * W, hd.CoutP, m->grads + hd.bias_off, (double*)c.F(p.colsum_scr), st));
    bool head_sums = false;
    LCHK(run_dgrad(c, m->head, dlogits, H, W, H, W, c.F(p.g[last_c2]), nullptr, d4.ptr, d4.scale, d4.shift, nullptr,
                   m->convs[last_c2].bn, &head_sums));
    int h = H, w = W;
    bool c2_sums = head_sums;
    for (int i = (int)m->dec.size() - 1; i >= 0; --i) {
      const DecL& dl = m->dec[i];
      const size_t npix = (size_t)N * h * w;
      LCHK(run_bn_bwd(c, dl.c2, c.F(p.g[dl.c2]), c.F(p.g[dl.c2]), npix, c2_sums));
      c2_sums = false;
      Src a1 = lazy_src(c, dl.c1, h, w);
      LCHK(run_wgrad(c, dl.c2, a1, nullptr, c.F(p.g[dl.c2]), h, w));
      bool c1_sums = false;
      LCHK(run_dgrad(c, dl.c2, c.F(p.g[dl.c2]), h, w, h, w, c.F(p.g[dl.c1]), nullptr, a1.ptr, a1.scale, a1.shift, nullptr,
                     m->convs[dl.c1].bn, &c1_sums));
      LCHK(run_bn_bwd(c, dl.c1, c.F(p.g[dl.c1]), c.F(p.g[dl.c1]), npix, c1_sums));
      Src prev = (i == 0) ? feat_src(3) : lazy_src(c, m->dec[i - 1].c2, h / 2, w / 2);
      prev.up = 1;
      Src skip; const Src* sp = nullptr;
      if (i < 3) { skip = feat_src(2 - i); sp = &skip; } else if (i == 3) { skip = f1; sp = &skip; }
      LCHK(run_wgrad(c, dl.c1, prev, sp, c.F(p.g[dl.c1]), h, w));
      float* gprev = (i == 0) ? c.F(p.gx[feat_blk(3)]) : c.F(p.g[m->dec[i - 1].c2]);
      const float* pm = (i == 0) ? feat_mask(prev) : prev.ptr;
      const ConvL& c1v = m->convs[dl.c1];
      if (c1v.wud_off && p.wino_ok((size_t)dl.c1) && !(h & 1) && !(w & 1)) {
        UpSplit us{gprev, dl.C0, pm, prev.scale, prev.shift, 0};
        LCHK(run_dgrad(c, dl.c1, c.F(p.g[dl.c1]), h, w, h, w, dl.C1 > 0 ? c.F(p.gskip[i]) : nullptr, nullptr, nullptr, nullptr,
                       nullptr, &us, i > 0 ? m->convs[m->dec[i - 1].c2].bn : -1, &c2_sums));
      } else {
        LCHK(run_dgrad(c, dl.c1, c.F(p.g[dl.c1]), h, w, h, w, c.F(p.dcat[i]), nullptr, nullptr, nullptr, nullptr));
        LCHK(launch_upsplit(c.F(p.dcat[i]), N, h, w, dl.C0, dl.C1, gprev, pm, prev.scale, prev.shift,
                            dl.C1 > 0 ? c.F(p.gskip[i]) : nullptr, st));
      }
      h /= 2; w /= 2;
    }
    if (!m->nodes.empty()) {
      std::vector<char> ginit(5 + m->nodes.size(), 0);
      ginit[5 + m->nodes.size() - 1] = 1;
      auto tensor_src = [&](int id) -> Src {
        if (id == 0) return f1;
        if (id < 5) return feat_src(id - 1);
        const NodeL& nd = m->nodes[id - 5];
        return lazy_src(c, nd.c2, H >> nd.lvl, W >> nd.lvl);
      };
      auto tensor_grad = [&](int id) -> float* {
        if (id < 4) return c.F(p.gskip[3 - id]);
        if (id == 4) return c.F(p.gx[feat_blk(3)]);
        return c.F(p.g[m->nodes[id - 5].c2]);
      };
      for (int i = (int)m->nodes.size() - 1; i >= 0; --i) {
        const NodeL& nd = m->nodes[i];
        const int nh = H >> nd.lvl, nw = W >> nd.lvl;
        const size_t npix = (size_t)N * nh * nw;
        if (!ginit[5 + i]) return fail("internal: UnetPlusPlus node %d has no consumer", i);
        LCHK(run_bn_bwd(c, nd.c2, c.F(p.g[nd.c2]), c.F(p.g[nd.c2]), npix, i == (int)m->nodes.size() - 1 && head_sums));
        Src a1 = lazy_src(c, nd.c1, nh, nw);
        LCHK(run_wgrad(c, nd.c2, a1, nullptr, c.F(p.g[nd.c2]), nh, nw));
        bool c1_sums = false;
        LCHK(run_dgrad(c, nd.c2, c.F(p.g[nd.c2]), nh, nw, nh, nw, c.F(p.g[nd.c1]), nullptr, a1.ptr, a1.scale, a1.shift, nullptr,
                       m->convs[nd.c1].bn, &c1_sums));
        LCHK(run_bn_bwd(c, nd.c1, c.F(p.g[nd.c1]), c.F(p.g[nd.c1]), npix, c1_sums));
        Src prev = tensor_src(nd.prev); prev.up = 1;
        Src skip; const Src* sp = nullptr;
        if (nd.skips.size() == 1) { skip = tensor_src(nd.skips[0]); sp = &skip; }
        else if (nd.skips.size() > 1) { skip = mk_src(c.F(p.cat[i]), nd.C1, nh, nw); sp = &skip; }
        LCHK(run_wgrad(c, nd.c1, prev, sp, c.F(p.g[nd.c1]), nh, nw));
        float* gprev = tensor_grad(nd.prev);
        const float* pm = nd.prev < 5 ? feat_mask(prev) : prev.ptr;
        const int acc_prev = ginit[nd.prev]; ginit[nd.prev] = 1;
        const ConvL& c1v = m->convs[nd.c1];
        const float* gcat; int gcc, gco;
        if (c1v.wud_off && p.wino_ok((size_t)nd.c1) && !(nh & 1) && !(nw & 1)) {
          UpSplit us{gprev, nd.C0, pm, prev.scale, prev.shift, acc_prev};
          LCHK(run_dgrad(c, nd.c1, c.F(p.g[nd.c1]), nh, nw, nh, nw, nd.C1 > 0 ? c.F(p.gcat) : nullptr, nullptr, nullptr, nullptr,
                         nullptr, &us));
          gcat = c.F(p.gcat); gcc = nd.C1; gco = 0;
        } else {
          LCHK(run_dgrad(c, nd.c1, c.F(p.g[nd.c1]), nh, nw, nh, nw, c.F(p.dcat[0]), nullptr, nullptr, nullptr, nullptr));
          LCHK(launch_upsplit(c.F(p.dcat[0]), N, nh, nw, nd.C0, nd.C1, gprev, pm, prev.scale, prev.shift, nullptr, st, acc_prev));
          gcat = c.F(p.dcat[0]); gcc = nd.C0 + nd.C1; gco = nd.C0;
        }
        int coff = 0;
        for (int id : nd.skips) {
          const Src t = tensor_src(id);
          const bool lazy_mask = id >= 5;
          LCHK(launch_split_accum(gcat, gcc, gco + coff, t.C, npix, tensor_grad(id), lazy_mask ? t.ptr : nullptr,
                                  lazy_mask ? t.scale : nullptr, lazy_mask ? t.shift : nullptr, ginit[id], st));
          ginit[id] = 1;
          coff += t.C;
        }
      }
      for (int id = 0; id < 5; ++id) if (!ginit[id]) return fail("internal: UnetPlusPlus feature %d received no gradient", id);
    }
  }
  for (int k = (sb < 1 ? 1 : sb); effnet && k < se && k <= 4; ++k) {
    const int s = 4 - k;
    const int lo = s == 0 ? 0 : m->feat_blk[s - 1] + 1;
    for (int bi = m->feat_blk[s]; bi >= lo; --bi) {
      const MBL& b = m->mb[bi];
      const int ho = p.mh[bi], wo = p.mw[bi], hi = ho * b.stride, wi = wo * b.stride;
      const size_t npo = (size_t)N * ho * wo, npi = (size_t)N * hi * wi;
      const float* dz = c.F(p.gx[bi]);
      float* gO = c.F(p.g[b.cp]); float* gM = c.F(p.g[b.cdw]);
      const float* rs = (b.skip && b.drop > 0.f && m->keep_fwd) ? m->keep_fwd + (size_t)bi * N : nullptr;
      const float* g2 = dz;
      if (rs) { LCHK(launch_rowscale(dz, rs, N, (size_t)ho * wo, b.Cout, gO, st)); g2 = gO; }
      LCHK(run_bn_bwd(c, b.cp, g2, gO, npo));
      Src a2 = mk_src(c.F(p.a2[bi]), b.mid, ho, wo);
      LCHK(run_wgrad(c, b.cp, a2, nullptr, gO, ho, wo));
      LCHK(run_dgrad(c, b.cp, gO, ho, wo, ho, wo, gM, nullptr, nullptr, nullptr, nullptr));
      float* pool = c.F(p.se_pool[bi]); float* sv = c.F(p.se[bi]); float* hpre = sv + (size_t)N * b.mid;
      float* gs = c.F(p.se_gs[bi]); float* acc1 = gs + (size_t)N * b.mid; float* gpool = c.F(p.se_g);
      LCHK(launch_se_reduce_hw(gM, c.F(p.a1[bi]), N, (size_t)ho * wo, b.mid, 1.f, gs, c.F(p.se_part), st));
      const ConvL& cr = m->convs[b.cr]; const ConvL& cx = m->convs[b.cx];
      LCHK(launch_se_fc_bwd(gs, sv, hpre, pool, m->params + cr.w_off, cr.Kpad, m->params + cx.w_off, cx.Kpad, N, b.mid, b.nsq,
                            gpool, acc1, m->grads + cr.w_off, m->grads + cr.bias_off, m->grads + cx.w_off, m->grads + cx.bias_off, st));
      LCHK(run_bn_bwd_act(c, b.cdw, gM, gM, N, (size_t)ho * wo, sv, gpool));
      Src in = bi == 0 ? f1 : mk_src(c.F(p.xn[bi - 1]), b.Cin, hi, wi);
      float* gin = bi == 0 ? c.F(p.g[m->stem]) : c.F(p.gx[bi - 1]);
      const float* addend = nullptr;
      if (b.skip) addend = dz;
      else if (bi == 0) addend = c.F(p.gskip[3]);
      else for (int fs = 0; fs < 3; ++fs) if (bi - 1 == m->feat_blk[fs]) addend = c.F(p.gskip[2 - fs]);
      const ConvL& dw = m->convs[b.cdw];
      const float* dwin = b.ce >= 0 ? c.F(p.a0[bi]) : in.ptr;
      {
        hipStream_t ws_ = st;
        if (c.wst && c.wst != st) { HIPCHK(hipEventRecord(m->ev_fork, st)); HIPCHK(hipStreamWaitEvent(c.wst, m->ev_fork, 0)); ws_ = c.wst; }
        LCHK(launch_dw_wgrad(dwin, gM, b.k, b.stride, b.pb, N, hi, wi, b.mid, ho, wo, m->grads + dw.w_off, c.F(p.dw_part), ws_));
      }
      if (b.ce >= 0) {
        float* gI = c.F(p.g[b.ce]);
        LCHK(launch_dw_dgrad(gM, m->params + dw.w_off, b.k, b.stride, b.pb, N, hi, wi, b.mid, ho, wo, nullptr, gI, st));
        LCHK(run_bn_bwd_act(c, b.ce, gI, gI, N, (size_t)hi * wi, nullptr, nullptr));
        LCHK(run_wgrad(c, b.ce, in, nullptr, gI, hi, wi));
        LCHK(run_dgrad(c, b.ce, gI, hi, wi, hi, wi, gin, addend, nullptr, nullptr, nullptr));
      } else {
        LCHK(launch_dw_dgrad(gM, m->params + dw.w_off, b.k, b.stride, b.pb, N, hi, wi, b.mid, ho, wo, addend, gin, st));
      }
    }
    if (s == 0) {
      float* g = c.F(p.g[m->stem]);
      LCHK(run_bn_bwd_act(c, m->stem, g, g, N, (size_t)h1 * w1, nullptr, nullptr));
      Src x4 = mk_src(c.F(p.x4), m->CinP, H, W);
      LCHK(run_wgrad(c, m->stem, x4, nullptr, g, h1, w1));
    }
  }
  for (int k = (sb < 1 ? 1 : sb); !effnet && k < se && k <= 4; ++k) {
    const int s = 4 - k;
    const int h = sh[s], w = sw[s];
    const size_t npix = (size_t)N * h * w;
    for (int b = (int)m->stages[s].size() - 1; b >= 0; --b) {
      const BlockL& bl = m->stages[s][b];
      const size_t bi = first_blk[s] + b;
      const float* dz = c.F(p.gx[bi]);
      const int lc = bl.last();
      const int hin = h * bl.stride, win = w * bl.stride;
      LCHK(run_bn_bwd(c, lc, dz, c.F(p.g[lc]), npix, out_sums[bi] != 0));
      if (bl.cd >= 0) LCHK(run_bn_bwd(c, bl.cd, dz, c.F(p.g[bl.cd]), npix));
      int hc1 = h, wc1 = w;
      if (bl.c3 >= 0) {
        Src a2 = lazy_src(c, bl.c2, h, w);
        LCHK(run_wgrad(c, bl.c3, a2, nullptr, c.F(p.g[bl.c3]), h, w));
        bool c2_sums = false;
        LCHK(run_dgrad(c, bl.c3, c.F(p.g[bl.c3]), h, w, h, w, c.F(p.g[bl.c2]), nullptr, a2.ptr, a2.scale, a2.shift, nullptr,
                       m->convs[bl.c2].bn, &c2_sums));
        LCHK(run_bn_bwd(c, bl.c2, c.F(p.g[bl.c2]), c.F(p.g[bl.c2]), npix, c2_sums));
        hc1 = hin; wc1 = win;
      }
      Src a1 = lazy_src(c, bl.c1, hc1, wc1);
      LCHK(run_wgrad(c, bl.c2, a1, nullptr, c.F(p.g[bl.c2]), h, w));
      bool c1_sums = false;
      LCHK(run_dgrad(c, bl.c2, c.F(p.g[bl.c2]), h, w, hc1, wc1, c.F(p.g[bl.c1]), nullptr, a1.ptr, a1.scale, a1.shift, nullptr,
                     m->convs[bl.c1].bn, &c1_sums));
      LCHK(run_bn_bwd(c, bl.c1, c.F(p.g[bl.c1]), c.F(p.g[bl.c1]), (size_t)N * hc1 * wc1, c1_sums));
      Src in; float* gin; const float* in_mask;
      if (b > 0) { in = mk_src(c.F(p.xn[bi - 1]), bl.Cin, hin, win); gin = c.F(p.gx[bi - 1]); in_mask = in.ptr; }
      else if (s > 0) { in = feat_src(s - 1); gin = c.F(p.gx[first_blk[s] - 1]); in_mask = in.ptr; }
      else { in = mk_src(c.F(p.pool), 64, hin, win); gin = c.F(p.g_pool); in_mask = nullptr; }
      LCHK(run_wgrad(c, bl.c1, in, nullptr, c.F(p.g[bl.c1]), hc1, wc1));
      const float* addend;
      if (bl.cd >= 0) {
        LCHK(run_wgrad(c, bl.cd, in, nullptr, c.F(p.g[bl.cd]), h, w));
        const float* gs = (b == 0 && s > 0) ? c.F(p.gskip[3 - s]) : nullptr;
        LCHK(run_dgrad(c, bl.cd, c.F(p.g[bl.cd]), h, w, hin, win, c.F(p.tmp), gs, nullptr, nullptr, nullptr));
        addend = c.F(p.tmp);
      } else {
        addend = dz;
      }
      int pbn = -1; const float* py = nullptr; size_t pbi = 0;
      if (b > 0) { pbi = bi - 1; const int plc = m->stages[s][b - 1].last(); pbn = m->convs[plc].bn; py = c.F(p.y[plc]); }
      else if (s > 0) { pbi = first_blk[s] - 1; const int plc = m->stages[s - 1].back().last(); pbn = m->convs[plc].bn; py = c.F(p.y[plc]); }
      bool psums = false;
      LCHK(run_dgrad(c, bl.c1, c.F(p.g[bl.c1]), hc1, wc1, hin, win, gin, addend, in_mask, nullptr, nullptr, nullptr, pbn, &psums, py));
      if (pbn >= 0) out_sums[pbi] = psums ? 1 : 0;
    }
    if (s == 0) {
      const BNL& sb = m->bns[m->convs[m->stem].bn];
      static const bool no_fuse = dbg_flag("UWM_NO_BN_FUSE");
      const bool pool_sums = !no_fuse && f1.scale && f1.relu && sb.C == f1.C && (256 % (f1.C / 4)) == 0;
      LCHK(launch_wgrad_reduce_multi(m->rq, c.wst));
      LCHK(launch_maxpool_bwd(c.F(p.g_pool), (const uint8_t*)c.F(p.pool_idx), c.F(p.gskip[3]), f1, c.F(p.g[m->stem]), N,
                              sh[0], sw[0], st, pool_sums ? c.F(sb.f_off) : nullptr, pool_sums ? c.F(sb.f_off) + sb.C : nullptr,
                              c.D(sb.d_off) + 2 * sb.C, c.D(sb.d_off) + 3 * sb.C, sb.nrep, 2 * sb.C));
      LCHK(run_bn_bwd(c, m->stem, c.F(p.g[m->stem]), c.F(p.g[m->stem]), (size_t)N * h1 * w1, pool_sums));
      Src x4 = mk_src(c.F(p.x4), m->CinP, H, W);
      LCHK(run_wgrad(c, m->stem, x4, nullptr, c.F(p.g[m->stem]), h1, w1));
    }
// ... 10 lines not shown
```

### unet-watermark_amd/csrc/uwm_kernels.h

```cpp
#pragma once
#include <hip/hip_runtime.h>
#include <hip/hip_ext.h>
#include <stdint.h>
#include <stddef.h>
#include <atomic>

namespace uwm {

struct Src {
  const float* ptr;
  const float* scale;
  const float* shift;
  int C, H, W;
  int up;
  int relu;
};

struct FastDiv {
  unsigned mg, d;
};
static inline FastDiv make_fastdiv(unsigned d) {
  FastDiv f; f.d = d; f.mg = (d <= 1) ? 0u : (unsigned)((0x100000000ull / d) + 1ull); return f;
}

struct DevOnce {
  std::atomic<unsigned long long> mask{0};
  hipError_t set_max_lds(const void* fn, size_t bytes) {
    int dev = 0; hipError_t e = hipGetDevice(&dev);
    if (e != hipSuccess) return e;
    if (dev < 64 && ((mask.load(std::memory_order_acquire) >> dev) & 1ull)) return hipSuccess;
    e = hipFuncSetAttribute(fn, hipFuncAttributeMaxDynamicSharedMemorySize, (int)bytes);
    if (e == hipSuccess && dev < 64) mask.fetch_or(1ull << dev, std::memory_order_release);
    return e;
  }
};
bool dbg_flag(const char* name);
int dbg_int(const char* name, int dflt);
int device_cu_count();

struct ConvArgs {
  Src s0, s1;
  int C0, Ctot;
  const float* w;
  int wrows, Kpad, ntaps, kw;
  int N, Ho, Wo, Cout, M;
  int Hl, Wl;
  int smul, rmul, off, sdiv;
  float* out;
  const float* bias;
  const float* addend;
  const float* mask;
  const float* mscale; const float* mshift;
  double* ssum; double* ssq;
  int srep, sstride;
  const float* bnb_mean; const float* bnb_rstd;
  const float* bnb_y;
  FastDiv dv_ctot, dv_kw;
  double flops;
  double bytes;
  float* out_up; int up_c0; const float* up_mask; const float* up_mscale; const float* up_mshift;
  int up_accum;
  int pc_ntaps[4]; unsigned pc_taps[4];
  int live_ch;
  const float* wu;
  int wu_ncb;
  int wino;
  int prec;
  int wu_rinv_off;
  const float* xmax;
  int route_n;
  int ig16;
  int nprod;
  const float* wbank;
  int wu_layout;
};

template <class A> static inline int route_N(const A& a) { return a.route_n > 0 ? a.route_n : a.N; }
template <class A> static inline long route_M(const A& a) { return a.N > 0 ? (long)a.M / a.N * route_N(a) : (long)a.M; }

#if defined(__HIPCC__)
typedef unsigned uwm_u2 __attribute__((ext_vector_type(2)));
__device__ __forceinline__ void uwm_split4(float x0, float x1, float x2, float x3, uwm_u2& hi, uwm_u2& lo) {
  typedef _Float16 h2_ __attribute__((ext_vector_type(2)));
  const h2_ a = {(_Float16)x0, (_Float16)x1}, b = {(_Float16)x2, (_Float16)x3};
  hi.x = __builtin_bit_cast(unsigned, a); hi.y = __builtin_bit_cast(unsigned, b);
  unsigned l0, l1;
  asm("v_fma_mixlo_f16 %0, %1, -1.0, %2 op_sel_hi:[1,0,0]\n\t"
      "v_fma_mixhi_f16 %0, %1, -1.0, %3 op_sel:[1,0,0] op_sel_hi:[1,0,0]"
      : "=&v"(l0) : "v"(hi.x), "v"(x0), "v"(x1));
  asm("v_fma_mixlo_f16 %0, %1, -1.0, %2 op_sel_hi:[1,0,0]\n\t"
      "v_fma_mixhi_f16 %0, %1, -1.0, %3 op_sel:[1,0,0] op_sel_hi:[1,0,0]"
      : "=&v"(l1) : "v"(hi.y), "v"(x2), "v"(x3));
  lo.x = l0; lo.y = l1;
}
constexpr float kIgWScale = 4096.f;
__device__ __forceinline__ void ig_bank_unit(const float* __restrict__ src, float* __restrict__ dst, size_t i, int Kpad) {
  typedef float f4_ __attribute__((ext_vector_type(4)));
  const size_t g = i >> 3;
  const int unit = (int)(i & 7), row = (int)((g * 32) / (size_t)Kpad);
  const f4_ w4 = *(const f4_*)(src + i * 4) * kIgWScale;
  uwm_u2 hi, lo;
  uwm_split4(__builtin_amdgcn_fmed3f(w4.x, -65504.f, 65504.f), __builtin_amdgcn_fmed3f(w4.y, -65504.f, 65504.f),
             __builtin_amdgcn_fmed3f(w4.z, -65504.f, 65504.f), __builtin_amdgcn_fmed3f(w4.w, -65504.f, 65504.f), hi, lo);
  char* rb = (char*)(dst + g * 32);
  const int sw = (row >> 1) & 7;
  *(uwm_u2*)(rb + (((unit >> 1) ^ sw) << 4) + (unit & 1) * 8) = hi;
  *(uwm_u2*)(rb + ((((unit >> 1) + 4) ^ sw) << 4) + (unit & 1) * 8) = lo;
}
#endif

struct ReduceJob { const float* part; float* dw; unsigned long long n4; int nsplit; unsigned block0; };
struct ReduceQueue {
  enum { kMax = 48 };
  ReduceJob j[kMax]; int n = 0; unsigned blocks = 0; size_t used_floats = 0;
};
struct ReduceJobs { ReduceJob j[ReduceQueue::kMax]; int n; };

struct WgradArgs {
  Src s0, s1; int C0, Ctot;
  const float* dy;
  float* dw;
  int wrows, Kpad, ntaps, kw;
  int N, Ho, Wo, Cout, M;
  int Hl, Wl, stride, pad;
  int nsplit, msplit;
  float* part;
  size_t part_floats;
  int force_igemm;
  FastDiv dv_ctot, dv_kw;
  double flops;
  double bytes;
  int wino;
  int prec;
  const float* xmax;
  ReduceQueue* rq;
  int cu_share;
  int route_n;
  int nprod;
};

enum { kProfClasses = 64 };
void prof_enable(bool on);
bool prof_on();
void prof_pair(int cls, double flops, double bytes, hipEvent_t* e0, hipEvent_t* e1);
void route_note(const char* kernel);
const char* route_last();
#define UWM_LAUNCH(cls, flops, bytes, kernel, grid, block, lds, st, ...)                                     \
  do {                                                                                                       \
    route_note(#kernel);                                                                                     \
    if (prof_on()) {                                                                                         \
      hipEvent_t e0_, e1_; prof_pair((cls), (flops), (bytes), &e0_, &e1_);                                   \
      hipExtLaunchKernelGGL(kernel, grid, block, lds, st, e0_, e1_, 0, __VA_ARGS__);                         \
    } else {                                                                                                 \
      hipLaunchKernelGGL(kernel, grid, block, lds, st, __VA_ARGS__);                                         \
    }                                                                                                        \
  } while (0)
int  prof_collect(double* out );
const char* prof_class_name(int cls);

enum ConvKernel { kConvInvalid = 0, kConvUp2, kConvUp2F16, kConvUp2Dgrad, kConvUp2DgradF16, kConvC16F16, kConvC32F16, kConvGemm, kConvHead,
                  kConvHeadDgrad, kConvF16x3, kConvF16x3v2, kConvWinoX3, kConvWino, kConvWino8, kConvPatch16, kConvPatch, kConvS2Dgrad, kConvIgemm };
struct ConvRoute { ConvKernel k; int v; };
ConvRoute conv_route(const ConvArgs& a, int force_cfg);
hipError_t launch_conv(const ConvArgs& a, hipStream_t st, int force_cfg = -1);
bool conv_epilogue_carries_bnb(const ConvArgs& a);
enum WgradKernel { kWgradInvalid = 0, kWgradGemm, kWgradUp2, kWgradF16x3, kWgradStem, kWgradC16, kWgradWino, kWgradPatch, kWgradIgemm };
struct WgradRoute { WgradKernel k; int v; };
WgradRoute wgrad_route(const WgradArgs& a);
hipError_t launch_wgrad(const WgradArgs& a, hipStream_t st);
hipError_t launch_conv_igemm(const ConvArgs& a, hipStream_t st, int cfg);
bool conv_s2_dgrad_applicable(const ConvArgs& a);
hipError_t launch_conv_s2_dgrad(const ConvArgs& a, hipStream_t st, int cfg);
hipError_t launch_wgrad_igemm(const WgradArgs& a, hipStream_t st, bool f16);
bool wgrad_patch_applicable(const WgradArgs& a);
hipError_t launch_wgrad_patch(const WgradArgs& a, hipStream_t st);
bool wgrad_wino_applicable(const WgradArgs& a);
hipError_t launch_wgrad_wino(const WgradArgs& a, hipStream_t st);
size_t wgrad_wino_scratch_floats();
float* wgrad_op_scratch();
bool wgrad_c16_applicable(const WgradArgs& a);
hipError_t launch_wgrad_c16(const WgradArgs& a, hipStream_t st);
hipError_t launch_wgrad_reduce(const float* part, int nsplit, size_t n4, float* dw, hipStream_t st, ReduceQueue* rq = nullptr);
hipError_t launch_wgrad_reduce_multi(ReduceQueue& q, hipStream_t st);
bool wgrad_f16x3_applicable(const WgradArgs& a);
hipError_t launch_wgrad_f16x3(const WgradArgs& a, hipStream_t st);
bool wgrad_stem_applicable(const WgradArgs& a);
hipError_t launch_wgrad_stem(const WgradArgs& a, hipStream_t st);
bool wgrad_gemm_applicable(const WgradArgs& a);
hipError_t launch_wgrad_gemm(const WgradArgs& a, hipStream_t st);
bool wgrad_gemm_preferred(const WgradArgs& a);
bool wgrad_up2_applicable(const WgradArgs& a);
hipError_t launch_wgrad_up2(const WgradArgs& a, hipStream_t st);
bool conv_gemm_applicable(const ConvArgs& a);
hipError_t launch_conv_gemm(const ConvArgs& a, hipStream_t st, int bn);
bool conv_gemm_preferred(const ConvArgs& a);
bool conv_up2_applicable(const ConvArgs& a);
hipError_t launch_conv_up2(const ConvArgs& a, hipStream_t st);
bool conv_up2_dgrad_applicable(const ConvArgs& a);
hipError_t launch_conv_up2_dgrad(const ConvArgs& a, hipStream_t st);
hipError_t launch_conv_up2_f16(const ConvArgs& a, hipStream_t st);
hipError_t launch_conv_up2_dgrad_f16(const ConvArgs& a, hipStream_t st);
bool conv_c16_f16_applicable(const ConvArgs& a);
hipError_t launch_conv_c16_f16(const ConvArgs& a, hipStream_t st);
bool conv_c32_f16_applicable(const ConvArgs& a);
hipError_t launch_conv_c32_f16(const ConvArgs& a, hipStream_t st);
bool wgrad_up2_f16_shape(const WgradArgs& a);
int wgrad_up2_f16_parts(const WgradArgs& a);
hipError_t launch_wgrad_up2_f16(const WgradArgs& a, hipStream_t st);
bool conv_patch_applicable(const ConvArgs& a);
bool conv_patch16_applicable(const ConvArgs& a);
hipError_t launch_conv_patch16(const ConvArgs& a, hipStream_t st);
hipError_t launch_conv_patch(const ConvArgs& a, hipStream_t st, int bn);
bool conv_wino_applicable(const ConvArgs& a);
hipError_t launch_conv_wino(const ConvArgs& a, hipStream_t st, int bn = 0);
bool conv_head_applicable(const ConvArgs& a);
hipError_t launch_conv_head(const ConvArgs& a, hipStream_t st);
bool conv_head_dgrad_applicable(const ConvArgs& a);
hipError_t launch_conv_head_dgrad(const ConvArgs& a, hipStream_t st);
bool conv_wino8_applicable(const ConvArgs& a);
hipError_t launch_conv_wino8(const ConvArgs& a, hipStream_t st);
size_t wino_weights_floats(int wrows, int Ctot);
int wino_ncb(int wrows);
hipError_t launch_wino_weights(const float* w, int wrows, int Kpad, int Ctot, int mirror, float* ut, hipStream_t st);
struct WinoJob { const float* w; float* ut; int rows, chans, Kpad, mode, src_rows, pad_; };
struct WinoJobs { static constexpr int kMax = 56; WinoJob j[kMax]; int n; };
hipError_t launch_wino_weights_multi(const WinoJobs& jobs, hipStream_t st);
hipError_t launch_wino_weights_x3_multi(const WinoJobs& jobs, hipStream_t st);
int f16x3_nj(int rows);
size_t f16x3_bank_floats(int rows, int chans);
size_t f16x3_rinv_off(int rows, int chans);
hipError_t launch_f16x3_weights_multi(const WinoJobs& jobs, hipStream_t st);
bool conv_f16x3_applicable(const ConvArgs& a);
static inline __host__ __device__ size_t f16x3_rinv_off_floats(int rows, int chans) { return (size_t)(chans / 16) * 5 * (size_t)(((rows + 63) / 64) * 4) * 512; }
bool f16x3v2_shape(int Ho, int Wo, int rows, int chans);
int f16x3v2_nf(int rows);
hipError_t launch_f16x3v2_weights_multi(const WinoJobs& jobs, hipStream_t st);
bool conv_f16x3v2_applicable(const ConvArgs& a);
hipError_t launch_conv_f16x3v2(const ConvArgs& a, hipStream_t st, bool four_wave = false);
size_t stem_f16x3_bank_floats();
hipError_t launch_stem_f16x3_weights(const float* w, int Kpad, int cin_p, float* bank, hipStream_t st);
bool conv_stem_f16x3_applicable(const ConvArgs& a);
hipError_t launch_conv_stem_f16x3(const ConvArgs& a, hipStream_t st);
hipError_t launch_conv_f16x3(const ConvArgs& a, hipStream_t st, int variant = 0);
bool conv_wino_x3_applicable(const ConvArgs& a);
hipError_t launch_conv_wino_x3(const ConvArgs& a, hipStream_t st);
bool winograd_enabled();
void winograd_set_mode(int mode);
int winograd_mode();
static inline int wino_mode_of(int wino) { return wino > 0 ? wino - 1 : winograd_mode(); }

hipError_t launch_nchw_to_nhwc4(const float* x, float* y, int N, int C, int H, int W, int CP, hipStream_t st);
hipError_t launch_bn_finalize(const double* ssum, const double* ssq, const float* gamma, const float* beta,
                              float* run_mean, float* run_var, float* mean, float* rstd, float* scale, float* shift,
                              int C, double count, float eps, float momentum, int update_running, hipStream_t st,
                              int nrep = 1, int rep_stride = 0);
hipError_t launch_bn_eval(const float* gamma, const float* beta, const float* run_mean, const float* run_var,
                          float* scale, float* shift, int C, float eps, hipStream_t st);
struct BnEvalJob { unsigned g_off, rm_off, out_off; int C; float eps; };
struct BnEvalJobs { static constexpr int kMax = 128; BnEvalJob j[kMax]; int n; };
hipError_t launch_bn_eval_multi(const float* params, const float* buffers, float* out, const BnEvalJobs& jobs, hipStream_t st);
hipError_t launch_residual(const float* y, const float* s2, const float* b2, const float* id, const float* sd,
                           const float* bd, float* out, size_t npix, int C, hipStream_t st);
hipError_t launch_maxpool_fwd(const Src& in, float* out, uint8_t* idx, int N, int Ho, int Wo, hipStream_t st);
hipError_t launch_maxpool_bwd(const float* gout, const uint8_t* idx, const float* addend, const Src& in, float* gin,
                              int N, int Ho, int Wo, hipStream_t st, const float* bn_mean = nullptr, const float* bn_rstd = nullptr,
                              double* ssum = nullptr, double* ssq = nullptr, int srep = 0, int sstride = 0);
hipError_t launch_bn_bwd_reduce(const float* g, const float* y, const float* mean, const float* rstd,
                                double* dgamma, double* dbeta, size_t npix, int C, hipStream_t st);
hipError_t launch_bn_bwd_apply(const float* g, const float* y, const float* mean, const float* rstd,
                               const float* gamma, const double* dgamma, const double* dbeta, float* dy,
                               float* gamma_grad, float* beta_grad, size_t npix, int C, hipStream_t st,
                               const double* rep = nullptr, int nrep = 0, int rep_stride = 0, hipEvent_t done = nullptr,
                               float* xmax = nullptr);
hipError_t launch_upsplit(const float* dcat, int N, int H, int W, int C0, int C1, float* gprev,
                          const float* pmask, const float* pscale, const float* pshift, float* gskip,
                          hipStream_t st, int accumulate_prev = 0);
hipError_t launch_concat_copy(const Src& s, size_t npix, float* dst, int Cd, int dst_off, hipStream_t st);
hipError_t launch_split_accum(const float* gcat, int Cc, int off, int C, size_t npix, float* dst, const float* m,
                              const float* mscale, const float* mshift, int accumulate, hipStream_t st);
hipError_t launch_pack_dgrad(const float* w, int Cout, int Kpad, int ntaps, int Cin, float* wd, int KpadD,
                             int CoutP, hipStream_t st);
hipError_t launch_colsum(const float* g, size_t npix, int C, float* out, double* scratch, hipStream_t st);
size_t colsum_scratch_doubles(int C);
hipError_t launch_adam(float* p, const float* g, float* m, float* v, size_t n, float lr, float b1, float b2,
                       float eps, float wd, float bc1, float bc2, float gscale, hipStream_t st,
                       const double* sumsq = nullptr, float max_norm = 0.f, bool decoupled = false);
hipError_t launch_adam_graph(float* p, const float* g, float* m, float* v, size_t n, float* hyp , const double* sumsq, hipStream_t st,
                             bool decoupled = false);
hipError_t launch_sumsq(const float* g, size_t n, double* out, hipStream_t st);
hipError_t launch_sgd(float* p, const float* g, float* buf, size_t n, float lr, float momentum, float wd, int first, float gscale,
                      hipStream_t st, const double* sumsq = nullptr, float max_norm = 0.f);
hipError_t launch_resize_threshold(const float* logits, int ld, int N, int h, int w, int H, int W, float thr,
                                   int apply_sigmoid, uint8_t* out, float* out_f, hipStream_t st);
hipError_t launch_scale(float* p, size_t n, float s, hipStream_t st);
hipError_t launch_absmax32(const float* x, size_t n, float* out32, hipStream_t st);
hipError_t launch_preprocess_u8(const uint8_t* img, int N, int H, int W, int C, const float* mean, const float* std,
                                const int* flags, float* out, hipStream_t st);
hipError_t launch_preprocess_u8_nhwc4(const uint8_t* img, size_t npix, int C, const float* mean, const float* std, float* out,
                                      hipStream_t st);
hipError_t launch_preprocess_mask(const uint8_t* m, int N, int H, int W, int thr, const int* flags, uint8_t* out, hipStream_t st);
struct PreArgs { float mul[4], add[4]; };
__device__ __forceinline__ float pre_norm(uint32_t b, float mul, float add) { return fmaf((float)b, mul, add); }
static inline PreArgs make_pre_args(int C, const float* mean, const float* std) {
  PreArgs pa;
  for (int c = 0; c < 4; ++c) { pa.mul[c] = 0.f; pa.add[c] = 0.f; }
  for (int c = 0; c < C; ++c) { pa.mul[c] = 1.f / (255.f * std[c]); pa.add[c] = -mean[c] / std[c]; }
  return pa;
}
__device__ __forceinline__ void aug_src(int flags, int H, int W, int y, int x, int& sy, int& sx) {
  const int k = (flags >> 2) & 3;
  int fy = y, fx = x;
  if (k == 1) { fy = x; fx = W - 1 - y; }
  else if (k == 2) { fy = H - 1 - y; fx = W - 1 - x; }
  else if (k == 3) { fy = H - 1 - x; fx = y; }
  if (flags & 1) fx = W - 1 - fx;
  if (flags & 2) fy = H - 1 - fy;
  sy = fy; sx = fx;
}
struct AugDesc { int flags, hue, sat, val; double minv[6]; unsigned char lut[256]; };
hipError_t launch_augment_u8(const uint8_t* img, const AugDesc* descs, int N, int H, int W, int C, const float* mean, const float* std,
                             float* out_f, uint8_t* out_u8, hipStream_t st);
hipError_t launch_augment_mask(const uint8_t* m, const AugDesc* descs, int N, int H, int W, int thr, uint8_t* out, hipStream_t st);
__device__ __forceinline__ float resize_logit(const float* __restrict__ b, int ld, int h, int w, float sy, float sx, int Y, int X,
                                              int apply_sigmoid) {
  float fy = ((float)Y + 0.5f) * sy - 0.5f, fx = ((float)X + 0.5f) * sx - 0.5f;
  fy = fmaxf(fy, 0.f); fx = fmaxf(fx, 0.f);
  int y0 = (int)fy, x0 = (int)fx;
  y0 = min(y0, h - 1); x0 = min(x0, w - 1);
  const int y1 = min(y0 + 1, h - 1), x1 = min(x0 + 1, w - 1);
  const float wy = fy - (float)y0, wx = fx - (float)x0;
  const float v00 = b[((size_t)y0 * w + x0) * ld], v01 = b[((size_t)y0 * w + x1) * ld];
  const float v10 = b[((size_t)y1 * w + x0) * ld], v11 = b[((size_t)y1 * w + x1) * ld];
  float v = (1.f - wy) * ((1.f - wx) * v00 + wx * v01) + wy * ((1.f - wx) * v10 + wx * v11);
  if (apply_sigmoid) v = 1.f / (1.f + expf(-v));
  return v;
}
constexpr int kResizeRowsPerBlock = 4;
struct ImageDesc { long long offset; int h, w; };
hipError_t launch_resize_u8(const uint8_t* src, size_t src_bytes, const ImageDesc* descs, int N, int C, int H, int W, int interp,
                            uint8_t* out, hipStream_t st);
hipError_t launch_resize_norm_u8_nhwc4(const uint8_t* src, size_t src_bytes, const ImageDesc* descs, int N, int C, int H, int W,
                                       const float* mean, const float* std, float* out, hipStream_t st);
hipError_t launch_resize_threshold_ragged(const float* logits, int ld, int N, int h, int w, const ImageDesc* out_descs, float thr,
                                          int apply_sigmoid, uint8_t* mask, size_t mask_bytes, hipStream_t st);

hipError_t launch_swish_fwd(const float* y, const float* sc, const float* sh, int C, float* out, size_t npix, hipStream_t st);
hipError_t launch_dw_fwd(const float* x, const float* w, int k, int stride, int pb, int N, int H, int W, int C,
                         int Ho, int Wo, float* y, hipStream_t st);
hipError_t launch_dw_dgrad(const float* dy, const float* w, int k, int stride, int pb, int N, int H, int W, int C,
                           int Ho, int Wo, const float* addend, float* dx, hipStream_t st);
size_t dw_wgrad_scratch_floats(int k, int N, int C, int Ho, int Wo);
hipError_t launch_dw_wgrad(const float* x, const float* dy, int k, int stride, int pb, int N, int H, int W, int C,
                           int Ho, int Wo, float* dw, float* scratch, hipStream_t st);
hipError_t launch_bn_bwd_act(const float* g, const float* y, const float* mean, const float* rstd, const float* gamma, const float* scale,
                             const float* shift, const float* se_s, const float* gpool, int N, size_t hw, double* dgamma, double* dbeta,
                             float* dy, float* gamma_grad, float* beta_grad, int C, hipStream_t st,
                             float* xmax = nullptr);
hipError_t launch_colstats(const float* y, size_t npix, int C, double* ssum, double* ssq, hipStream_t st);
size_t se_reduce_scratch_floats(int N, int C);
hipError_t launch_se_reduce_hw(const float* a, const float* b, int N, size_t hw, int C, float scale, float* out, float* part, hipStream_t st);
hipError_t launch_swish_pool(const float* y, const float* sc, const float* sh, float* act_out, int N, size_t hw, int C, float* pool,
                             float* part, hipStream_t st);
hipError_t launch_se_fc_fwd(const float* pool, const float* w1, const float* b1, int K1pad, const float* w2, const float* b2,
                            int K2pad, int N, int C, int nsq, float* hpre, float* hid , float* s, hipStream_t st);
hipError_t launch_se_fc_bwd(float* gs, const float* s, const float* hpre, const float* pool, const float* w1, int K1pad,
                            const float* w2, int K2pad, int N, int C, int nsq, float* gpool, float* acc1, float* gw1,
                            float* gb1, float* gw2, float* gb2, hipStream_t st);
hipError_t launch_se_scale(const float* a, const float* s, int N, size_t hw, int C, float* out, hipStream_t st);
hipError_t launch_mb_out(const float* y, const float* sc, const float* sh, const float* rowscale, const float* id, int N, size_t hw,
                         int C, float* out, hipStream_t st);
hipError_t launch_rowscale(const float* g, const float* rowscale, int N, size_t hw, int C, float* out, hipStream_t st);
// ... 23 lines not shown
```

### unet-watermark_amd/csrc/uwm_launch.inc

```
struct Ctx {
  uwm_model* m; float* ws; hipStream_t st; int N;
  hipStream_t wst = nullptr;
  float* fz = nullptr;
  float* F(size_t off) const { return ws + off; }
  const float* bn_ss(const BNL& b) const { return fz ? fz + b.fz_off : ws + b.f_off + 2 * b.C; }
  float* wu(const ConvL& cv) const { return fz ? fz + cv.fz_wu : ws + cv.wu_off; }
  double* D(size_t doff) const { return (double*)ws + doff; }
};
static Src mk_src(const float* ptr, int C, int H, int W, const float* scale = nullptr, const float* shift = nullptr,
                  int relu = 0, int up = 0) {
  Src s; s.ptr = ptr; s.scale = scale; s.shift = shift; s.C = C; s.H = H; s.W = W; s.up = up; s.relu = relu; return s;
}
static Src lazy_src(const Ctx& c, int conv, int H, int W, int relu = 1, int up = 0) {
  const ConvL& cv = c.m->convs[conv];
  const BNL& b = c.m->bns[cv.bn];
  return mk_src(c.F(c.m->plan.y[conv]), cv.CoutP, H, W, c.bn_ss(b), c.bn_ss(b) + b.C, relu, up);
}

static thread_local bool g_err_own = false;
static hipError_t fail_launch(const char* fmt, ...) {
  va_list ap; va_start(ap, fmt); vsnprintf(g_err, sizeof(g_err), fmt, ap); va_end(ap);
  g_err_own = true;
  return hipErrorInvalidValue;
}

static bool dy_max_needed(const uwm_model* m, size_t ci) {
  return m->convs[ci].bn >= 0 && (f3_dgrad_on(m, ci) || conv_ig16(m, ci, true) || wgrad_f16_on(m, ci));
}
static hipError_t dy_max_slot(const Ctx& c, int ci, const char* pass, const float** slot) {
  const ConvL& cv = c.m->convs[ci];
  if (!dy_max_needed(c.m, (size_t)ci) || cv.bn >= (int)c.m->dy_max_made.size() || !c.m->dy_max_made[cv.bn])
    return fail_launch("internal: the fp16x3 %s of %s has no max|dY| producer (dy_max_needed / run_bn_bwd*)", pass, cv.name.c_str());
  *slot = (const float*)c.D(c.m->bns[cv.bn].xmax_off());
  return hipSuccess;
}

static hipError_t route_rec(const Ctx& c, const char* pass, int ci, hipError_t e) {
  if (c.m->route_log_on && e == hipSuccess) { c.m->route_log += pass; c.m->route_log += ' '; c.m->route_log += c.m->convs[ci].name; c.m->route_log += ' '; c.m->route_log += route_last(); c.m->route_log += '\n'; }
  return e;
}

static hipError_t run_conv_fwd(const Ctx& c, int ci, const Src& s0, const Src* s1, int Ho, int Wo, float* out,
                               bool stats, int cfg = -1) {
  const ConvL& cv = c.m->convs[ci];
  ConvArgs a; memset(&a, 0, sizeof(a));
  a.s0 = s0; a.C0 = s0.C;
  if (s1) { a.s1 = *s1; a.Ctot = s0.C + s1->C; } else { a.s1 = s0; a.Ctot = s0.C; }
  a.w = c.m->params + cv.w_off; a.wrows = cv.Cout; a.Kpad = cv.Kpad; a.ntaps = cv.k * cv.k; a.kw = cv.k;
  a.N = c.N; a.Ho = Ho; a.Wo = Wo; a.Cout = cv.CoutP; a.M = c.N * Ho * Wo;
  a.Hl = s0.H << s0.up; a.Wl = s0.W << s0.up;
  a.smul = cv.stride; a.rmul = 1; a.off = -cv.pad; a.sdiv = 1;
  a.out = out; a.bias = cv.bias_off >= 0 ? c.m->params + cv.bias_off : nullptr;
  if (stats && cv.bn >= 0) {
    const BNL& b = c.m->bns[cv.bn];
    a.ssum = c.D(b.d_off) + 2 * b.C; a.ssq = a.ssum + b.C; a.srep = b.nrep; a.sstride = 2 * b.C;
  }
  a.dv_ctot = make_fastdiv(a.Ctot); a.dv_kw = make_fastdiv(a.kw);
  a.flops = 2.0 * (double)a.M * cv.Cout * cv.Cin * cv.k * cv.k;
  a.bytes = 4.0 * ((double)c.N * s0.H * s0.W * s0.C + (s1 ? (double)c.N * s1->H * s1->W * s1->C : 0.0) + (double)cv.Cout * cv.Kpad +
                   (double)a.M * cv.CoutP);
  if (ci == c.m->stem && cfg < 0 && stem_f3_on(c.m)) {
    a.wu = c.wu(cv);
    if (conv_stem_f16x3_applicable(a)) return route_rec(c, "fwd", ci, launch_conv_stem_f16x3(a, c.st));
    a.wu = nullptr;
  }
  if (cv.wu_off && !cv.stem7() && !cv.igb() && a.Ctot == cv.CinP && c.m->plan.wino_ok((size_t)ci)) {
    a.wu = c.wu(cv); a.wu_ncb = wino_ncb(cv.Cout);
    if (c.m->plan.prec == UWM_PREC_BF16X3_ALL && cv.x3()) {
      if (a.C0 != cv.c0 && a.C0 != a.Ctot) return hipErrorInvalidValue;
      a.prec = 1;
    }
    if (f3_fwd_on(c.m, (size_t)ci)) {
      a.prec = 2; a.wu_layout = f3_layout(c.m, (size_t)ci, false); a.nprod = f3_nprod(c.m, false);
      a.wu_ncb = a.wu_layout == 1 ? f16x3v2_nf(cv.Cout) : f16x3_nj(cv.Cout); a.wu_rinv_off = (int)f16x3_rinv_off(cv.Cout, cv.CinP);
    }
  }
  a.wino = c.m->plan.wino_mode + 1; a.route_n = c.m->route_n;
  if (conv_ig16(c.m, (size_t)ci, false)) a.ig16 = 1;
  if (ig_bank_on(c.m, (size_t)ci, false) && a.Ctot == cv.CinP && cfg < 0) a.wbank = c.wu(cv);
  return route_rec(c, "fwd", ci, launch_conv(a, c.st, cfg));
}

struct UpSplit { float* gprev; int C0; const float* pmask; const float* pscale; const float* pshift; int accumulate = 0; };
static hipError_t run_dgrad(const Ctx& c, int ci, const float* dy, int Ho, int Wo, int Hin, int Win, float* dx,
                            const float* addend, const float* mask, const float* mscale, const float* mshift,
                            const UpSplit* us = nullptr, int bn_fuse = -1, bool* fused = nullptr, const float* bn_y = nullptr) {
  const ConvL& cv = c.m->convs[ci];
  ConvArgs a; memset(&a, 0, sizeof(a));
  a.s0 = mk_src(dy, cv.CoutP, Ho, Wo); a.s1 = a.s0; a.C0 = cv.CoutP; a.Ctot = cv.CoutP;
  a.w = c.F(cv.wd_off); a.wrows = cv.CinP; a.Kpad = cv.KpadD; a.ntaps = cv.k * cv.k; a.kw = cv.k;
  a.N = c.N; a.Ho = Hin; a.Wo = Win; a.Cout = cv.CinP; a.M = c.N * Hin * Win;
  a.Hl = Ho; a.Wl = Wo; a.smul = 1; a.rmul = -1; a.off = cv.pad; a.sdiv = cv.stride;
  a.out = dx; a.addend = addend; a.mask = mask; a.mscale = mscale; a.mshift = mshift; a.live_ch = cv.Cout;
  a.dv_ctot = make_fastdiv(a.Ctot); a.dv_kw = make_fastdiv(a.kw);
  a.flops = 2.0 * (double)c.N * Ho * Wo * cv.Cout * cv.Cin * cv.k * cv.k;
  a.bytes = 4.0 * ((double)c.N * Ho * Wo * cv.CoutP + (double)cv.CinP * cv.KpadD +
                   (double)a.M * cv.CinP * (1.0 + (addend ? 1.0 : 0.0) + (mask ? 1.0 : 0.0)));
  if (cv.wud_off && c.m->plan.wino_ok((size_t)ci)) {
    a.wu = c.F(cv.wud_off); a.wu_ncb = wino_ncb(cv.CinP);
    const int pm = c.m->plan.prec;
    if ((pm == UWM_PREC_BF16X3 || pm == UWM_PREC_BF16X3_ALL) && cv.x3_d()) a.prec = 1;
    if (f3_dgrad_on(c.m, (size_t)ci)) {
      a.prec = 2; a.wu_layout = f3_layout(c.m, (size_t)ci, true); a.nprod = f3_nprod(c.m, true);
      a.wu_ncb = a.wu_layout == 1 ? f16x3v2_nf(cv.CinP) : f16x3_nj(cv.CinP); a.wu_rinv_off = (int)f16x3_rinv_off(cv.CinP, cv.CoutP);
    }
  }
  a.wino = c.m->plan.wino_mode + 1;
  if (conv_ig16(c.m, (size_t)ci, true)) a.ig16 = 1;
  if (ig_bank_on(c.m, (size_t)ci, true)) a.wbank = c.F(cv.wdb_off);
  if (a.prec == 2 || a.ig16) {
    const hipError_t e = dy_max_slot(c, ci, "dgrad", &a.xmax);
    if (e != hipSuccess) return e;
  }
  if (us) { a.out_up = us->gprev; a.up_c0 = us->C0; a.up_mask = us->pmask; a.up_mscale = us->pscale; a.up_mshift = us->pshift; a.up_accum = us->accumulate; }
  if (fused) *fused = false;
  static const bool no_fuse = dbg_flag("UWM_NO_BN_FUSE");
  a.bnb_y = bn_y;
  if (bn_fuse >= 0 && fused && !no_fuse && (us ? (us->pmask != nullptr && !us->accumulate) : (mask != nullptr || bn_y != nullptr)) && conv_epilogue_carries_bnb(a)) {
    const BNL& b = c.m->bns[bn_fuse];
    if (b.C == (us ? us->C0 : cv.CinP)) {
      const float* f = c.F(b.f_off);
      a.bnb_mean = f; a.bnb_rstd = f + b.C;
      a.ssum = c.D(b.d_off) + 2 * b.C; a.ssq = a.ssum + b.C; a.srep = b.nrep; a.sstride = 2 * b.C;
      *fused = true;
    }
  }
  if (!fused || !*fused) a.bnb_y = nullptr;
  a.route_n = c.m->route_n;
  return route_rec(c, "dgrad", ci, launch_conv(a, c.st));
}

static hipError_t run_wgrad(const Ctx& c, int ci, const Src& s0, const Src* s1, const float* dy, int Ho, int Wo) {
  const ConvL& cv = c.m->convs[ci];
  WgradArgs a; memset(&a, 0, sizeof(a));
  a.s0 = s0; a.C0 = s0.C;
  if (s1) { a.s1 = *s1; a.Ctot = s0.C + s1->C; } else { a.s1 = s0; a.Ctot = s0.C; }
  a.dy = dy; a.dw = c.m->grads + cv.w_off; a.wrows = cv.Cout; a.Kpad = cv.Kpad; a.ntaps = cv.k * cv.k; a.kw = cv.k;
  a.N = c.N; a.Ho = Ho; a.Wo = Wo; a.Cout = cv.CoutP; a.M = c.N * Ho * Wo;
  a.Hl = s0.H << s0.up; a.Wl = s0.W << s0.up; a.stride = cv.stride; a.pad = cv.pad;
  a.dv_ctot = make_fastdiv(a.Ctot); a.dv_kw = make_fastdiv(a.kw);
  a.flops = 2.0 * (double)a.M * cv.Cout * cv.Cin * cv.k * cv.k;
  a.bytes = 4.0 * ((double)a.M * cv.CoutP + (double)c.N * s0.H * s0.W * s0.C + (s1 ? (double)c.N * s1->H * s1->W * s1->C : 0.0) +
                   (double)cv.Cout * cv.Kpad);
  a.wino = c.m->plan.wino_mode + 1; a.route_n = c.m->route_n;
  if (f3_wgrad_on(c.m, (size_t)ci)) { a.nprod = f3_nprod(c.m, true); a.cu_share = (c.wst && c.wst != c.st) ? 3 : 0; }
  if (wgrad_f16_on(c.m, (size_t)ci)) {
    a.prec = 2;
    const hipError_t e = dy_max_slot(c, ci, "wgrad", &a.xmax);
    if (e != hipSuccess) return e;
  }
  static const bool no_defer = dbg_flag("UWM_NO_DEFER_REDUCE");
  ReduceQueue& rq = c.m->rq;
  const size_t cap = wgrad_wino_scratch_floats();
  if (rq.n + 1 >= ReduceQueue::kMax || rq.used_floats + cap > kWgParts * cap) {
    hipError_t e = launch_wgrad_reduce_multi(rq, (c.wst && c.wst != c.st) ? c.wst : c.st);
    if (e != hipSuccess) return e;
  }
  a.part = c.F(c.m->plan.wg_part) + rq.used_floats; a.part_floats = cap; a.rq = no_defer ? nullptr : &rq;
  if (c.wst && c.wst != c.st) {
    const bool covered = std::find(c.m->disp_cov.begin(), c.m->disp_cov.end(), dy) != c.m->disp_cov.end();
    hipError_t e = hipSuccess;
    if (!covered) e = hipEventRecord(c.m->ev_fork, c.st);
    if (e != hipSuccess) return e;
    e = hipStreamWaitEvent(c.wst, covered ? c.m->ev_disp : c.m->ev_fork, 0);
    if (e != hipSuccess) return e;
    return route_rec(c, "wgrad", ci, launch_wgrad(a, c.wst));
  }
  return route_rec(c, "wgrad", ci, launch_wgrad(a, c.st));
}

static hipError_t run_bn_finalize(const Ctx& c, int bi, size_t count, int training) {
  uwm_model* m = c.m; const BNL& b = m->bns[bi];
  float* f = c.F(b.f_off);
  const float eps = b.eps > 0.f ? b.eps : m->desc.bn_eps, mom = b.mom > 0.f ? b.mom : m->desc.bn_momentum;
  if (training)
    return launch_bn_finalize(c.D(b.d_off) + 2 * b.C, c.D(b.d_off) + 3 * b.C, m->params + b.g_off, m->params + b.b_off,
                              m->buffers + b.rm_off, m->buffers + b.rv_off, f, f + b.C, f + 2 * b.C, f + 3 * b.C, b.C,
                              (double)count, eps, mom, 1, c.st, b.nrep, 2 * b.C);
  ++m->prep_launches;
  return launch_bn_eval(m->params + b.g_off, m->params + b.b_off, m->buffers + b.rm_off, m->buffers + b.rv_off,
                        f + 2 * b.C, f + 3 * b.C, b.C, eps, c.st);
}

static hipError_t run_bn_bwd(const Ctx& c, int ci, const float* g, float* dy, size_t npix, bool sums_fused = false) {
  uwm_model* m = c.m; const ConvL& cv = m->convs[ci]; const BNL& b = m->bns[cv.bn];
  const float* f = c.F(b.f_off); const float* y = c.F(m->plan.y[ci]);
  double* dg = c.D(b.d_off); double* db = c.D(b.d_off) + b.C;
  hipEvent_t done = nullptr;
  if (c.wst && c.wst != c.st && m->ev_disp && m->disp_fork) {
    hipStreamCaptureStatus cs = hipStreamCaptureStatusNone;
    if (hipStreamIsCapturing(c.st, &cs) != hipSuccess) { cs = hipStreamCaptureStatusNone; (void)hipGetLastError(); }
    if (cs == hipStreamCaptureStatusNone) done = m->ev_disp;
  }
  hipError_t e = hipSuccess;
  float* xmax = dy_max_needed(m, (size_t)ci) ? (float*)c.D(b.xmax_off()) : nullptr;
  if (sums_fused)
    e = launch_bn_bwd_apply(g, y, f, f + b.C, m->params + b.g_off, nullptr, nullptr, dy, m->grads + b.g_off, m->grads + b.b_off,
                            npix, b.C, c.st, c.D(b.d_off) + 2 * b.C, b.nrep, 2 * b.C, done, xmax);
  else {
    e = launch_bn_bwd_reduce(g, y, f, f + b.C, dg, db, npix, b.C, c.st);
    if (e != hipSuccess) return e;
    e = launch_bn_bwd_apply(g, y, f, f + b.C, m->params + b.g_off, dg, db, dy, m->grads + b.g_off, m->grads + b.b_off,
                            npix, b.C, c.st, nullptr, 0, 0, done, xmax);
  }
  if (e == hipSuccess && done) m->disp_cov.push_back(dy);
  if (e == hipSuccess && xmax) m->dy_max_made[cv.bn] = 1;
  return e;
}

static hipError_t run_bn_bwd_act(const Ctx& c, int ci, const float* g, float* dy, int N, size_t hw, const float* se_s, const float* gpool) {
  uwm_model* m = c.m; const ConvL& cv = m->convs[ci]; const BNL& b = m->bns[cv.bn];
  const float* f = c.F(b.f_off);
  float* xmax = dy_max_needed(m, (size_t)ci) ? (float*)c.D(b.xmax_off()) : nullptr;
  const hipError_t e = launch_bn_bwd_act(g, c.F(m->plan.y[ci]), f, f + b.C, m->params + b.g_off, f + 2 * b.C, f + 3 * b.C, se_s, gpool,
                                         N, hw, c.D(b.d_off), c.D(b.d_off) + b.C, dy, m->grads + b.g_off, m->grads + b.b_off, b.C, c.st, xmax);
  if (e == hipSuccess && xmax) m->dy_max_made[cv.bn] = 1;
  return e;
}

#define LCHK(expr)                                                                                     \
  do { hipError_t e_ = (expr); if (e_ != hipSuccess) { if (g_err_own) { g_err_own = false; return 1; }     \
       return fail("launch failed: %s at %s:%d (%s)", hipGetErrorString(e_), __FILE__, __LINE__, #expr); } } while (0)

static hipError_t wino_jobs(const Ctx& c, bool dgrad, hipStream_t st) {
  uwm_model* m = c.m;
  const bool wino_on = m->plan.wino_mode != 0;
  const int prec = m->plan.prec;
  const bool bf = prec == UWM_PREC_BF16X3 || prec == UWM_PREC_BF16X3_ALL;
  for (int x3 = wino_on ? 0 : 2; x3 <= 2; ++x3) {
    WinoJobs jobs; jobs.n = 0;
    auto flush = [&]() { if (jobs.n > 0 && !dgrad) ++m->prep_launches; hipError_t e = x3 == 2 ? launch_f16x3_weights_multi(jobs, st) : (x3 ? launch_wino_weights_x3_multi(jobs, st) : launch_wino_weights_multi(jobs, st)); jobs.n = 0; return e; };
    for (size_t ci = 0; ci < m->convs.size(); ++ci) {
      const ConvL& cv = m->convs[ci];
      if (x3 == 2 && ig_bank_on(m, ci, dgrad)) {
        WinoJob& j = jobs.j[jobs.n++];
        j.chans = 0; j.mode = 3; j.pad_ = 0;
        if (dgrad) { j.w = c.F(cv.wd_off); j.ut = c.F(cv.wdb_off); j.rows = cv.CinP; j.Kpad = cv.KpadD; j.src_rows = cv.CinP; }
        else { j.w = m->params + cv.w_off; j.ut = c.wu(cv); j.rows = cv.Cout; j.Kpad = cv.Kpad; j.src_rows = cv.Cout; }
        if (jobs.n == WinoJobs::kMax) { hipError_t e = flush(); if (e != hipSuccess) return e; }
        continue;
      }
      if (!wino_on || cv.igb() || !m->plan.wino_ok(ci) || !(dgrad ? cv.wud_off : cv.wu_off) || cv.stem7()) continue;
      int kind = 0;
      if (dgrad) { if (bf && cv.x3_d()) kind = 1; if (f3_dgrad_on(m, ci)) kind = 2; }
      else { if (prec == UWM_PREC_BF16X3_ALL && cv.x3()) kind = 1; if (f3_fwd_on(m, ci)) kind = 2; }
      if (kind != x3) continue;
      WinoJob& j = jobs.j[jobs.n++];
      j.w = m->params + cv.w_off; j.Kpad = cv.Kpad; j.pad_ = kind == 2 ? f3_layout(m, ci, dgrad) : 0;
      if (dgrad) { j.ut = c.F(cv.wud_off); j.rows = cv.CinP; j.chans = cv.CoutP; j.mode = 2; j.src_rows = cv.Cout; }
      else { j.ut = c.wu(cv); j.rows = cv.Cout; j.chans = cv.CinP; j.mode = 0; j.src_rows = cv.Cout; }
      if (jobs.n == WinoJobs::kMax) { hipError_t e = flush(); if (e != hipSuccess) return e; }
    }
    hipError_t e = flush();
    if (e != hipSuccess) return e;
  }
  return hipSuccess;
}
```

### unet-watermark_amd/csrc/uwm_route.hip

```cpp
#include "uwm_kernels.h"
#include <stdio.h>
#include <stdlib.h>

namespace uwm {

static int g_winograd = -1;
bool winograd_enabled() {
  if (g_winograd < 0) { const char* e = getenv("UWM_WINOGRAD"); g_winograd = (e && e[0] == '0') ? 0 : 1; }
  return g_winograd != 0;
}
void winograd_set_mode(int mode) { g_winograd = mode; }
int winograd_mode() { (void)winograd_enabled(); return g_winograd; }
int device_cu_count() {
  static int cus[64] = {0};
  int dev = 0; (void)hipGetDevice(&dev);
  if (dev < 0 || dev >= 64) return 256;
  if (!cus[dev] && (hipDeviceGetAttribute(&cus[dev], hipDeviceAttributeMultiprocessorCount, dev) != hipSuccess || cus[dev] <= 0)) cus[dev] = 256;
  return cus[dev];
}

struct RouteSwitches {
  bool trace = dbg_flag("UWM_TRACE_CONV");
  bool no_up2 = dbg_flag("UWM_NO_UP2"), no_up2_wgrad = dbg_flag("UWM_NO_UP2_WGRAD"), no_head = dbg_flag("UWM_NO_CONV_HEAD");
  bool no_bnb_y = dbg_flag("UWM_NO_BNB_Y"), no_igemm_bnb = dbg_flag("UWM_NO_IGEMM_BNB");
  bool no_narrow_1x1 = dbg_flag("UWM_NO_NARROW_1X1"), no_wgrad_ig16 = dbg_flag("UWM_NO_WGRAD_IG16");
};
static const RouteSwitches& switches() { static const RouteSwitches s; return s; }

struct ConvCaps { bool bnb, bnb_y, out_up, bnb_out_up; };
static ConvCaps conv_caps(ConvKernel k) {
  switch (k) {
    case kConvWino:         return {true, true, true, true};
    case kConvWinoX3:       return {true, false, true, true};
    case kConvF16x3:        return {true, true, true, false};
    case kConvUp2Dgrad: case kConvUp2DgradF16: return {true, false, true, true};
    case kConvF16x3v2: case kConvGemm: case kConvS2Dgrad: case kConvIgemm: return {true, true, false, false};
    case kConvC16F16: case kConvC32F16: case kConvPatch16: case kConvHeadDgrad: return {true, false, false, false};
    default:                return {false, false, false, false};
  }
}
ConvRoute conv_route(const ConvArgs& a, int cfg) {
  const RouteSwitches& sw = switches();
  const bool aut = cfg < 0;
  const ConvRoute invalid = {kConvInvalid, 0};
  auto wino = [&](int bn) -> ConvRoute {
    if (bn == 8 || (bn <= 0 && !a.bnb_mean && !a.bnb_y && !a.out_up && conv_wino8_applicable(a))) return {kConvWino8, 0};
    return {kConvWino, bn};
  };
  auto up2 = [&]() -> ConvRoute { return {a.ig16 ? kConvUp2F16 : kConvUp2, 0}; };
  if (cfg == 700) return up2();
  if (cfg == 710 || (aut && a.ig16 && a.prec != 2 && conv_c16_f16_applicable(a))) return {kConvC16F16, 0};
  if (cfg == 711 || (aut && a.ig16 && a.prec != 2 && conv_c32_f16_applicable(a))) return {kConvC32F16, 0};
  if (cfg >= 800 && cfg < 1000) return {kConvGemm, cfg - 800};
  if (cfg == 500) return {kConvHead, 0};
  if ((cfg >= 600 && cfg <= 607) || (aut && a.prec == 2)) {
    const int v = aut ? 0 : cfg - 600;
    if (a.wu_layout == 1) return (v == 4 || v == 6 || !conv_f16x3v2_applicable(a)) ? invalid : ConvRoute{kConvF16x3v2, v == 5};
    return (v >= 4 || !conv_f16x3_applicable(a)) ? invalid : ConvRoute{kConvF16x3, v};
  }
  if (cfg == 400) return {kConvWinoX3, 0};
  if (cfg >= 300) return cfg < 400 ? wino(cfg - 300) : invalid;
  if (a.out_up) {
    if (aut && !sw.no_up2 && conv_up2_dgrad_applicable(a)) return {a.ig16 ? kConvUp2DgradF16 : kConvUp2Dgrad, 0};
    if (a.prec == 1) return conv_wino_x3_applicable(a) ? ConvRoute{kConvWinoX3, 0} : invalid;
    return conv_wino_applicable(a) ? wino(0) : invalid;
  }
  if (cfg == 200) return {kConvPatch16, 0};
  if (aut && !sw.no_up2 && conv_up2_applicable(a)) return up2();
  if (aut && !sw.no_head && conv_head_applicable(a)) return {kConvHead, 0};
  if (aut && !sw.no_head && conv_head_dgrad_applicable(a)) return {kConvHeadDgrad, 0};
  if (aut && wino_mode_of(a.wino) != 0 && conv_wino_applicable(a) && !conv_patch16_applicable(a))
    return a.prec == 1 ? ConvRoute{kConvWinoX3, 0} : wino(0);
  if (cfg >= 100) return {kConvPatch, cfg - 100};
  if (aut && conv_patch16_applicable(a)) return {kConvPatch16, 0};
  if (aut && conv_patch_applicable(a)) {
    const long sp = (long)route_N(a) * ((a.Ho + 7) / 8) * ((a.Wo + 15) / 16);
    int bn = a.Cout >= 128 ? 128 : (a.Cout > 32 ? 64 : (a.Cout > 16 ? 32 : 16));
    if (bn == 128 && sp * ((a.Cout + 127) / 128) < 512) bn = 64;
    return {kConvPatch, bn};
  }
  if (aut && conv_s2_dgrad_applicable(a)) {
    const long t128 = (long)((route_N(a) * (a.Ho >> 1) * (a.Wo >> 1) + 127) / 128) * ((a.Cout + 127) / 128);
    if (a.Cout > 64 && t128 < device_cu_count()) return {kConvS2Dgrad, 4};
    return {kConvS2Dgrad, a.Cout <= 64 ? 1 : 0};
  }
  if (aut && conv_gemm_preferred(a)) return {kConvGemm, 0};
  if (aut) {
    const long tiles128 = (long)((route_M(a) + 127) / 128);
    if (a.Cout <= 16) cfg = 3;
    else if (a.Cout <= 32) cfg = 2;
    else if (a.Cout <= 64) cfg = (tiles128 >= 512) ? 1 : 4;
    else {
      const long b0 = tiles128 * ((a.Cout + 127) / 128);
      const int pad128 = ((a.Cout + 127) / 128) * 128, pad64 = ((a.Cout + 63) / 64) * 64;
      if (!sw.no_narrow_1x1 && a.ntaps == 1 && pad128 * 100 > pad64 * 115 && tiles128 * (pad64 / 64) >= 512) cfg = 1;
      else if (b0 >= 512) cfg = 0;
      else if (tiles128 * ((a.Cout + 63) / 64) >= 512) cfg = 1;
      else cfg = 4;
    }
  }
  return cfg <= 5 ? ConvRoute{kConvIgemm, cfg} : invalid;
}

bool conv_epilogue_carries_bnb(const ConvArgs& a) {
  const ConvKernel k = conv_route(a, -1).k;
  const ConvCaps c = conv_caps(k);
  if (a.out_up) return c.bnb_out_up && !a.bnb_y;
  if (a.bnb_y) return c.bnb_y && a.prec != 1 && !switches().no_bnb_y;
  if (switches().no_igemm_bnb && (k == kConvGemm || k == kConvS2Dgrad || k == kConvIgemm)) return false;
  return c.bnb;
}

hipError_t launch_conv(const ConvArgs& a, hipStream_t st, int force_cfg) {
  if (a.M <= 0 || a.Cout <= 0 || (a.Cout & 3) || (a.Kpad & 31) || (a.Ctot & 3) || (a.C0 & 3)) return hipErrorInvalidValue;
  if (switches().trace)
    fprintf(stderr, "conv %s N=%d Ctot=%d(C0=%d up=%d) Cout=%d Ho=%d Wo=%d Hl=%d Wl=%d taps=%d smul=%d sdiv=%d wino=%d gflop=%.2f\n",
            a.rmul < 0 ? "dgrad" : "fwd", a.N, a.Ctot, a.C0, a.s0.up, a.Cout, a.Ho, a.Wo, a.Hl, a.Wl, a.ntaps, a.smul, a.sdiv,
            (int)(force_cfg < 0 && wino_mode_of(a.wino) != 0 && conv_wino_applicable(a)), a.flops * 1e-9);
  const ConvRoute r = conv_route(a, force_cfg);
  const ConvCaps c = conv_caps(r.k);
  if (a.bnb_mean && (!c.bnb || (a.bnb_y && !c.bnb_y) || (a.out_up && !c.bnb_out_up) || !a.ssum || !a.ssq || !a.bnb_rstd ||
                     !(a.out_up ? a.up_mask : (a.bnb_y ? a.bnb_y : a.mask)) || a.up_accum))
    return hipErrorInvalidValue;
  if (a.out_up && (!c.out_up || ((a.Ho | a.Wo) & 1) || (a.up_c0 & 3) || a.up_c0 > a.Cout || a.addend || a.mask || a.bias || a.bnb_y ||
                   (a.ssum && !a.bnb_mean) || (a.up_c0 < a.Cout && !a.out)))
    return hipErrorInvalidValue;
  switch (r.k) {
    case kConvUp2:         return launch_conv_up2(a, st);
    case kConvUp2F16:      return launch_conv_up2_f16(a, st);
    case kConvUp2Dgrad:    return launch_conv_up2_dgrad(a, st);
    case kConvUp2DgradF16: return launch_conv_up2_dgrad_f16(a, st);
    case kConvC16F16:      return launch_conv_c16_f16(a, st);
    case kConvC32F16:      return launch_conv_c32_f16(a, st);
    case kConvGemm:        return launch_conv_gemm(a, st, r.v);
    case kConvHead:        return launch_conv_head(a, st);
    case kConvHeadDgrad:   return launch_conv_head_dgrad(a, st);
    case kConvF16x3:       return launch_conv_f16x3(a, st, r.v);
    case kConvF16x3v2:     return launch_conv_f16x3v2(a, st, r.v != 0);
    case kConvWinoX3:      return launch_conv_wino_x3(a, st);
    case kConvWino:        return launch_conv_wino(a, st, r.v);
    case kConvWino8:       return launch_conv_wino8(a, st);
    case kConvPatch16:     return launch_conv_patch16(a, st);
    case kConvPatch:       return launch_conv_patch(a, st, r.v);
    case kConvS2Dgrad:     return launch_conv_s2_dgrad(a, st, r.v);
    case kConvIgemm:       return launch_conv_igemm(a, st, r.v);
    default:               return hipErrorInvalidValue;
  }
}

WgradRoute wgrad_route(const WgradArgs& a) {
  const RouteSwitches& sw = switches();
  const int f = a.force_igemm & 0xff;
  const bool aut = f == 0, no_up2 = sw.no_up2 || sw.no_up2_wgrad;
  if (f == 4) return {kWgradGemm, 0};
  if (a.prec == 2 && (aut || f == 6)) {
    if (a.xmax && !no_up2 && wgrad_up2_applicable(a) && wgrad_up2_f16_shape(a)) return {kWgradUp2, 0};
    if (wgrad_f16x3_applicable(a)) return {kWgradF16x3, 0};
  }
  if (f == 6) {
    if (a.prec == 2 && wgrad_stem_applicable(a)) return {kWgradStem, 0};
    if (a.prec == 2 && a.Cout == 16 && wgrad_c16_applicable(a)) return {kWgradC16, 0};
    return {kWgradInvalid, 0};
  }
  if (aut && !no_up2 && wgrad_up2_applicable(a)) return {kWgradUp2, 0};
  if (aut && wgrad_stem_applicable(a)) return {kWgradStem, 0};
  if (aut && wgrad_gemm_preferred(a)) return {kWgradGemm, 0};
  if (aut && wgrad_c16_applicable(a)) return {kWgradC16, 0};
  if (aut && wino_mode_of(a.wino) != 0 && wgrad_wino_applicable(a)) return {kWgradWino, 0};
  if (f != 1 && f != 7 && wgrad_patch_applicable(a)) return {kWgradPatch, 0};
  const bool f16 = !sw.no_wgrad_ig16 && a.prec == 2 && a.xmax && (aut || f == 7) && (a.Ctot & 31) == 0 && (a.Cout & 31) == 0;
  return {kWgradIgemm, f16 ? 1 : 0};
}

hipError_t launch_wgrad(const WgradArgs& a, hipStream_t st) {
  if (switches().trace)
    fprintf(stderr, "wgrad N=%d Ctot=%d(C0=%d) Cout=%d wrows=%d Ho=%d Wo=%d Hl=%d Wl=%d taps=%d stride=%d wino=%d patch=%d gflop=%.2f\n", a.N, a.Ctot,
            a.C0, a.Cout, a.wrows, a.Ho, a.Wo, a.Hl, a.Wl, a.ntaps, a.stride, (int)(wino_mode_of(a.wino) != 0 && wgrad_wino_applicable(a)),
            (int)wgrad_patch_applicable(a), a.flops * 1e-9);
  const WgradRoute r = wgrad_route(a);
  switch (r.k) {
    case kWgradGemm:  return launch_wgrad_gemm(a, st);
    case kWgradUp2:   return launch_wgrad_up2(a, st);
    case kWgradF16x3: return launch_wgrad_f16x3(a, st);
    case kWgradStem:  return launch_wgrad_stem(a, st);
    case kWgradC16:   return launch_wgrad_c16(a, st);
    case kWgradWino:  return launch_wgrad_wino(a, st);
    case kWgradPatch: return launch_wgrad_patch(a, st);
    case kWgradIgemm: return launch_wgrad_igemm(a, st, r.v != 0);
    default:          return hipErrorInvalidValue;
  }
}

}
```

Baseline: 1188 images/s.

## Fuse head dgrad with BN backward apply; enable BN sums in f16x3 upsplit dgrad

Adds an APPLY variant of the segmentation-head dgrad kernel. It recomputes the small head convolution gradient and applies the BN backward formula directly, so the intermediate dy tensor is never written and re-read by a separate BN-apply kernel. It also marks the f16x3 conv kernel as able to accumulate BN-backward sums while writing an upsampled split output, which removes a separate reduction pass in the decoder. The cost is recomputing the head dgrad in a second launch and extra shared-memory fold logic. Test entry points and debug flags are added.

Result: no change. 1188 images/s, median of 2 (+0.0%).

```diff
diff --git a/include/uwm.h b/include/uwm.h
--- a/include/uwm.h
+++ b/include/uwm.h
@@ -225,6 +225,14 @@
 int  uwm_op_dgrad_upsplit(const float* dy, int N, int H, int W, int Cout, const float* wd, int C0, int C1, int KpadD,
                           float* gprev, const float* pmask, const float* pscale, const float* pshift, float* gskip,
                           uwm_stream stream);
+int  uwm_op_dgrad_upsplit_f16x3(const float* dy, int N, int H, int W, int Cout, const float* w, int Kpad, int C0, int C1,
+                                float* gprev, const float* pmask, const float* pscale, const float* pshift, float* gskip,
+                                int eight_wave, const float* bn_mean, const float* bn_rstd, double* sums, int nrep,
+                                uwm_stream stream);
+int  uwm_op_head_dgrad_bn(const float* dlogits, int N, int H, int W, int classes, const float* wd, int C, int KpadD, const float* y,
+                          const float* mean, const float* rstd, const float* gamma, const float* scale, const float* shift,
+                          double* sums, int nrep, int apply_only, float* dy, float* dgamma, float* dbeta, float* xmax,
+                          uwm_stream stream);
 int  uwm_op_upsplit(const float* dcat, int N, int H, int W, int C0, int C1, float* gprev, const float* pmask,
                     const float* pscale, const float* pshift, float* gskip, uwm_stream stream);
 int  uwm_op_residual(const float* y, const float* s2, const float* b2, const float* id, const float* sd, const float* bd,
diff --git a/unet-watermark_amd/_lib.py b/unet-watermark_amd/_lib.py
--- a/unet-watermark_amd/_lib.py
+++ b/unet-watermark_amd/_lib.py
@@ -134,6 +134,8 @@
     "uwm_op_bn_backward": (I, [P, P, P, P, P, P, P, P, P, L, I, P]),
     "uwm_op_bn_backward_act": (I, [P, P, P, P, P, P, P, P, P, I, L, I, P, P, P, P, P, P]),
     "uwm_op_dgrad_upsplit": (I, [P, I, I, I, I, P, I, I, I, P, P, P, P, P, P]),
+    "uwm_op_dgrad_upsplit_f16x3": (I, [P, I, I, I, I, P, I, I, I, P, P, P, P, P, I, P, P, P, I, P]),
+    "uwm_op_head_dgrad_bn": (I, [P, I, I, I, I, P, I, I, P, P, P, P, P, P, P, I, I, P, P, P, P, P]),
     "uwm_op_upsplit": (I, [P, I, I, I, I, I, P, P, P, P, P, P]),
     "uwm_op_residual": (I, [P, P, P, P, P, P, P, L, I, P]),
 }
diff --git a/unet-watermark_amd/csrc/conv_head.hip b/unet-watermark_amd/csrc/conv_head.hip
--- a/unet-watermark_amd/csrc/conv_head.hip
+++ b/unet-watermark_amd/csrc/conv_head.hip
@@ -123,8 +123,9 @@
 }
 
 constexpr int kHeadDTH = 8;
-template <int CQ, int NCO, int TH = kHeadDTH>
-__global__ __launch_bounds__(256, TH >= 8 ? 2 : (TH >= 4 ? 3 : 4)) void conv_head_dgrad_kernel(const ConvArgs a) {
+struct HeadBnApply { const float* gamma; float* dy; float* gamma_grad; float* beta_grad; float* xmax; float invM; };
+template <int CQ, int NCO, bool APPLY = false, int TH = kHeadDTH>
+__global__ __launch_bounds__(256, TH >= 8 ? 2 : (TH >= 4 ? 3 : 4)) void conv_head_dgrad_kernel(const ConvArgs a, const HeadBnApply ap) {
   constexpr int C = CQ * 4, COLS = 256 / CQ, PW = COLS + 2;
   __shared__ f4 ws[9 * NCO * CQ];
   __shared__ float gs[(TH + 2) * PW * NCO];
@@ -138,6 +139,11 @@
   const int H = a.Ho, W = a.Wo;
   const int n = blockIdx.z, ho0 = blockIdx.y * TH, w0 = blockIdx.x * COLS;
   const float* gn = a.s0.ptr + (size_t)n * H * W * 4;
+  double rb[APPLY ? 2 : 1][4];
+  if constexpr (APPLY) {
+    bn_bwd_fold_load(a.ssum, a.srep < 1 ? 1 : a.srep, a.sstride, C, 0, 0, rb[0]);
+    bn_bwd_fold_load(a.ssum, a.srep < 1 ? 1 : a.srep, a.sstride, C, 1, 0, rb[1]);
+  }
   for (int i = threadIdx.x; i < (TH + 2) * PW * NCO; i += 256) {
     const int co = i % NCO, px = i / NCO, row = px / PW, cx = px - row * PW;
     const int hh = ho0 - 1 + row, ww = w0 - 1 + cx;
@@ -176,20 +182,64 @@
   f4 ps_ = {0.f, 0.f, 0.f, 0.f}, pq_ = {0.f, 0.f, 0.f, 0.f}, bmu = ps_, brs = ps_, msc = {1.f, 1.f, 1.f, 1.f}, msh = ps_;
   if (bnb) { bmu = *(const f4*)(a.bnb_mean + q * 4); brs = *(const f4*)(a.bnb_rstd + q * 4); }
   if (a.mask && a.mscale) { msc = *(const f4*)(a.mscale + q * 4); msh = *(const f4*)(a.mshift + q * 4); }
+  const unsigned wg = blockIdx.x + gridDim.x * (blockIdx.y + gridDim.y * blockIdx.z);
+  auto masked = [&](int j, size_t o) -> f4 {
+    f4 v = acc[j];
+    if (a.addend) v += *(const f4*)(a.addend + o);
+    if (a.mask) {
+      const f4 m = mk[j] * msc + msh;
+      v.x = m.x > 0.f ? v.x : 0.f; v.y = m.y > 0.f ? v.y : 0.f; v.z = m.z > 0.f ? v.z : 0.f; v.w = m.w > 0.f ? v.w : 0.f;
+    }
+    return v;
+  };
+  if constexpr (APPLY) {
+    __shared__ double part[2 * 256 * 4];
+    __shared__ double res[2 * CQ * 4];
+    __shared__ float wmax[4];
+    const f4 gm = *(const f4*)(ap.gamma + q * 4);
+    double sb[4], sg[4];
+    bn_bwd_fold_finish_both(rb[0], rb[1], a.srep < 1 ? 1 : a.srep, C, part, res, sb, sg);
+    if (wg == 0 && threadIdx.x < CQ) {
+#pragma unroll
+      for (int e = 0; e < 4; ++e) {
+        if (ap.beta_grad) ap.beta_grad[q * 4 + e] = (float)sb[e];
+        if (ap.gamma_grad) ap.gamma_grad[q * 4 + e] = (float)sg[e];
+      }
+    }
+    f4 dbq, dgq;
+    dbq.x = (float)sb[0] * ap.invM; dbq.y = (float)sb[1] * ap.invM; dbq.z = (float)sb[2] * ap.invM; dbq.w = (float)sb[3] * ap.invM;
+    dgq.x = (float)sg[0] * ap.invM; dgq.y = (float)sg[1] * ap.invM; dgq.z = (float)sg[2] * ap.invM; dgq.w = (float)sg[3] * ap.invM;
+    const f4 A = gm * brs, B = -(gm * brs * brs * dgq), K = -(A * dbq) - B * bmu;
+    float amax = 0.f;
+#pragma unroll
+    for (int j = 0; j < TH; ++j) {
+      const int ho = ho0 + j;
+      if (ho >= H || !live) continue;
+      const size_t o = (((size_t)n * H + ho) * W + wo) * C + q * 4;
+      const f4 d = A * masked(j, o) + B * mk[j] + K;
+      amax = fmaxf(fmaxf(amax, fmaxf(fabsf(d.x), fabsf(d.y))), fmaxf(fabsf(d.z), fabsf(d.w)));
+      *(f4*)(ap.dy + o) = d;
+    }
+    if (ap.xmax) {
+#pragma unroll
+      for (int d = 32; d >= 1; d >>= 1) amax = fmaxf(amax, __shfl_xor(amax, d));
+      if ((threadIdx.x & 63) == 0) wmax[threadIdx.x >> 6] = amax;
+      __syncthreads();
+      if (threadIdx.x == 0) {
+        const float mx = fmaxf(fmaxf(wmax[0], wmax[1]), fmaxf(wmax[2], wmax[3]));
+        if (mx > 0.f) atomicMax((unsigned*)ap.xmax + (wg & 31), __float_as_uint(mx));
+      }
+    }
+    return;
+  }
 #pragma unroll
   for (int j = 0; j < TH; ++j) {
     const int ho = ho0 + j;
     if (ho >= H || !live) continue;
     const size_t o = (((size_t)n * H + ho) * W + wo) * C + q * 4;
-    f4 v = acc[j];
-    if (a.addend) v += *(const f4*)(a.addend + o);
-    if (a.mask) {
-      const f4 yr = mk[j];
-      const f4 m = yr * msc + msh;
-      v.x = m.x > 0.f ? v.x : 0.f; v.y = m.y > 0.f ? v.y : 0.f; v.z = m.z > 0.f ? v.z : 0.f; v.w = m.w > 0.f ? v.w : 0.f;
-      if (bnb) { ps_ += v; pq_ += v * ((yr - bmu) * brs); }
-    }
-    *(f4*)(a.out + o) = v;
+    const f4 v = masked(j, o);
+    if (a.mask && bnb) { ps_ += v; pq_ += v * ((mk[j] - bmu) * brs); }
+    if (a.out) *(f4*)(a.out + o) = v;
   }
   if (bnb) {
     float v8[8] = {ps_.x, ps_.y, ps_.z, ps_.w, pq_.x, pq_.y, pq_.z, pq_.w};
@@ -207,7 +257,6 @@
     if (threadIdx.x < CQ * 8) {
       const int qq = threadIdx.x / 8, e = threadIdx.x % 8;
       const double sacc = ((double)red[0][threadIdx.x] + (double)red[1][threadIdx.x]) + ((double)red[2][threadIdx.x] + (double)red[3][threadIdx.x]);
-      const unsigned wg = blockIdx.x + gridDim.x * (blockIdx.y + gridDim.y * blockIdx.z);
       const size_t srep_off = a.srep > 1 ? (size_t)(wg & (unsigned)(a.srep - 1)) * a.sstride : 0;
       if (e < 4) atomicAdd(a.ssum + srep_off + qq * 4 + e, sacc); else atomicAdd(a.ssq + srep_off + qq * 4 + (e - 4), sacc);
     }
@@ -222,16 +271,37 @@
 template <int CQ>
 static hipError_t launch_head_dgrad(const ConvArgs& a, hipStream_t st) {
   const dim3 g((unsigned)((a.Wo + 256 / CQ - 1) / (256 / CQ)), (unsigned)((a.Ho + kHeadDTH - 1) / kHeadDTH), (unsigned)a.N);
-  if (a.live_ch == 1) UWM_LAUNCH(30, a.flops, a.bytes, (conv_head_dgrad_kernel<CQ, 1>), g, dim3(256), 0, st, a);
-  else UWM_LAUNCH(30, a.flops, a.bytes, (conv_head_dgrad_kernel<CQ, 4>), g, dim3(256), 0, st, a);
+  const HeadBnApply none = {nullptr, nullptr, nullptr, nullptr, nullptr, 0.f};
+  if (a.live_ch == 1) UWM_LAUNCH(30, a.flops, a.bytes, (conv_head_dgrad_kernel<CQ, 1>), g, dim3(256), 0, st, a, none);
+  else UWM_LAUNCH(30, a.flops, a.bytes, (conv_head_dgrad_kernel<CQ, 4>), g, dim3(256), 0, st, a, none);
   return hipGetLastError();
 }
 hipError_t launch_conv_head_dgrad(const ConvArgs& a, hipStream_t st) {
-  if (!conv_head_dgrad_applicable(a)) return hipErrorInvalidValue;
+  if (!conv_head_dgrad_applicable(a) || (!a.out && !(a.bnb_mean && a.mask))) return hipErrorInvalidValue;
   switch (a.Cout) {
     case 8: return launch_head_dgrad<2>(a, st);
     case 16: return launch_head_dgrad<4>(a, st);
     default: return launch_head_dgrad<8>(a, st);
+  }
+}
+template <int CQ, int NCO>
+static hipError_t launch_head_dgrad_apply(const ConvArgs& a, const HeadBnApply& ap, hipStream_t st, hipEvent_t done) {
+  const dim3 g((unsigned)((a.Wo + 256 / CQ - 1) / (256 / CQ)), (unsigned)((a.Ho + kHeadDTH - 1) / kHeadDTH), (unsigned)a.N);
+  if (done) hipExtLaunchKernelGGL((conv_head_dgrad_kernel<CQ, NCO, true>), g, dim3(256), 0, st, nullptr, done, 0, a, ap);
+  else hipLaunchKernelGGL((conv_head_dgrad_kernel<CQ, NCO, true>), g, dim3(256), 0, st, a, ap);
+  return hipGetLastError();
+}
+hipError_t launch_conv_head_dgrad_apply(const ConvArgs& a, const float* gamma, float* dy, float* gamma_grad, float* beta_grad,
+                                        float* xmax, hipStream_t st, hipEvent_t done) {
+  if (!conv_head_dgrad_applicable(a) || !gamma || !dy || !a.mask || !a.mscale || !a.mshift || !a.bnb_mean || !a.bnb_rstd || !a.ssum ||
+      a.ssq != a.ssum + a.Cout || a.addend || (a.srep > 1 && a.sstride < 2 * a.Cout))
+    return hipErrorInvalidValue;
+  const HeadBnApply ap = {gamma, dy, gamma_grad, beta_grad, xmax, (float)(1.0 / ((double)a.N * a.Ho * a.Wo))};
+  const bool one = a.live_ch == 1;
+  switch (a.Cout) {
+    case 8: return one ? launch_head_dgrad_apply<2, 1>(a, ap, st, done) : launch_head_dgrad_apply<2, 4>(a, ap, st, done);
+    case 16: return one ? launch_head_dgrad_apply<4, 1>(a, ap, st, done) : launch_head_dgrad_apply<4, 4>(a, ap, st, done);
+    default: return one ? launch_head_dgrad_apply<8, 1>(a, ap, st, done) : launch_head_dgrad_apply<8, 4>(a, ap, st, done);
   }
 }
 
diff --git a/unet-watermark_amd/csrc/elementwise.hip b/unet-watermark_amd/csrc/elementwise.hip
--- a/unet-watermark_amd/csrc/elementwise.hip
+++ b/unet-watermark_amd/csrc/elementwise.hip
@@ -321,28 +321,7 @@
 #pragma unroll
     for (int half = 0; half < 2; ++half) {
       if (rep) {
-        const int nq = Q < 256 ? Q : 256, L = 256 / nq;
-        const int q0 = (int)(((size_t)blockIdx.x * 256) % (size_t)Q);
-        const int j = threadIdx.x % nq, l = threadIdx.x / nq;
-        if (half) __syncthreads();
-        if (l < L) {
-          const int cj = ((q0 + j) % Q) * 4 + half * C;
-          double b0 = 0, b1 = 0, b2 = 0, b3 = 0;
-          for (int r = l; r < nrep; r += L) {
-            const double* pr = rep + (size_t)r * rep_stride + cj;
-            b0 += pr[0]; b1 += pr[1]; b2 += pr[2]; b3 += pr[3];
-          }
-          double* o = part + (l * nq + j) * 4;
-          o[0] = b0; o[1] = b1; o[2] = b2; o[3] = b3;
-        }
-        __syncthreads();
-#pragma unroll
-        for (int e = 0; e < 4; ++e) sq[e] = 0.0;
-        for (int k = 0; k < L; ++k) {
-          const double* o = part + (k * nq + j) * 4;
-#pragma unroll
-          for (int e = 0; e < 4; ++e) sq[e] += o[e];
-        }
+        bn_bwd_fold_replicas(rep, nrep, rep_stride, C, half, (int)(((size_t)blockIdx.x * 256) % (size_t)Q), part, sq);
       } else {
         const double* src = half ? dgamma : dbeta;
 #pragma unroll
diff --git a/unet-watermark_amd/csrc/uwm_abi.inc b/unet-watermark_amd/csrc/uwm_abi.inc
--- a/unet-watermark_amd/csrc/uwm_abi.inc
+++ b/unet-watermark_amd/csrc/uwm_abi.inc
@@ -859,6 +859,71 @@
   LCHK(launch_conv(a, (hipStream_t)stream));
   return 0;
 }
+int uwm_op_dgrad_upsplit_f16x3(const float* dy, int N, int H, int W, int Cout, const float* w, int Kpad, int C0, int C1,
+                               float* gprev, const float* pmask, const float* pscale, const float* pshift, float* gskip,
+                               int eight_wave, const float* bn_mean, const float* bn_rstd, double* sums, int nrep, uwm_stream stream) {
+  if (!dy || !w || !gprev || !pmask || (C1 > 0 && !gskip)) return fail("uwm_op_dgrad_upsplit_f16x3: null argument");
+  if (N < 1 || (Cout & 31) || C0 < 64 || (C0 & 63) || C1 < 0 || (C1 & 3) || (H & 1) || (W & 1) || H < 8 || W < 16 || Kpad < 9 * (C0 + C1))
+    return fail("uwm_op_dgrad_upsplit_f16x3: needs Cout %% 32 == 0, C0 %% 64 == 0, C1 %% 4 == 0, even H >= 8, W >= 16, Kpad >= 9 (C0 + C1)");
+  if (bn_mean && (!bn_rstd || !sums || nrep < 1 || (nrep & (nrep - 1)))) return fail("uwm_op_dgrad_upsplit_f16x3: the sums need rstd, sums and a power-of-two nrep");
+  hipStream_t st = (hipStream_t)stream;
+  const int rows = C0 + C1;
+  ConvArgs a; memset(&a, 0, sizeof(a));
+  a.s0 = mk_src(dy, Cout, H, W); a.s1 = a.s0; a.C0 = Cout; a.Ctot = Cout;
+  a.w = w; a.wrows = rows; a.Kpad = (9 * Cout + 31) & ~31; a.ntaps = 9; a.kw = 3;
+  a.N = N; a.Ho = H; a.Wo = W; a.Cout = rows; a.M = N * H * W;
+  a.Hl = H; a.Wl = W; a.smul = 1; a.rmul = -1; a.off = 1; a.sdiv = 1;
+  a.out = gskip; a.out_up = gprev; a.up_c0 = C0; a.up_mask = pmask; a.up_mscale = pscale; a.up_mshift = pshift;
+  a.dv_ctot = make_fastdiv(a.Ctot); a.dv_kw = make_fastdiv(a.kw);
+  static float* xm = nullptr;
+  if (!xm) HIPCHK(hipMalloc((void**)&xm, 32 * sizeof(float)));
+  LCHK(launch_absmax32(dy, (size_t)N * H * W * Cout, xm, st));
+  a.xmax = xm;
+  static float* buf = nullptr; static size_t cap = 0;
+  const size_t need = f16x3_bank_floats(rows, Cout);
+  if (need > cap) {
+    HIPCHK(hipDeviceSynchronize());
+    if (buf) HIPCHK(hipFree(buf));
+    buf = nullptr; cap = 0;
+    HIPCHK(hipMalloc((void**)&buf, need * sizeof(float))); cap = need;
+  }
+  WinoJobs jobs; memset(&jobs, 0, sizeof(jobs)); jobs.n = 1;
+  WinoJob& j = jobs.j[0];
+  j.w = w; j.ut = buf; j.rows = rows; j.chans = Cout; j.Kpad = Kpad; j.mode = 2; j.src_rows = Cout; j.pad_ = 0;
+  LCHK(launch_f16x3_weights_multi(jobs, st));
+  a.wu = buf; a.wu_layout = 0; a.wu_ncb = f16x3_nj(rows); a.wu_rinv_off = (int)f16x3_rinv_off(rows, Cout); a.prec = 2;
+  if (bn_mean) {
+    HIPCHK(hipMemsetAsync(sums, 0, (size_t)nrep * 2 * C0 * sizeof(double), st));
+    a.bnb_mean = bn_mean; a.bnb_rstd = bn_rstd; a.ssum = sums; a.ssq = sums + C0; a.srep = nrep; a.sstride = 2 * C0;
+  }
+  LCHK(launch_conv(a, st, eight_wave ? 602 : 601));
+  return 0;
+}
+int uwm_op_head_dgrad_bn(const float* dlogits, int N, int H, int W, int classes, const float* wd, int C, int KpadD, const float* y,
+                         const float* mean, const float* rstd, const float* gamma, const float* scale, const float* shift, double* sums,
+                         int nrep, int apply_only, float* dy, float* dgamma, float* dbeta, float* xmax, uwm_stream stream) {
+  if (!dlogits || !wd || !y || !mean || !rstd || !gamma || !scale || !shift || !sums || !dy || !dgamma || !dbeta)
+    return fail("uwm_op_head_dgrad_bn: null argument");
+  if (N < 1 || H < 1 || W < 1 || classes < 1 || classes > 4 || (C != 8 && C != 16 && C != 32) || KpadD < 36 || (KpadD & 31) || nrep < 1 || (nrep & (nrep - 1)))
+    return fail("uwm_op_head_dgrad_bn: needs 1..4 classes, C = 8 | 16 | 32, KpadD %% 32 == 0, a power-of-two nrep");
+  hipStream_t st = (hipStream_t)stream;
+  ConvArgs a; memset(&a, 0, sizeof(a));
+  a.s0 = mk_src(dlogits, 4, H, W); a.s1 = a.s0; a.C0 = 4; a.Ctot = 4;
+  a.w = wd; a.wrows = C; a.Kpad = KpadD; a.ntaps = 9; a.kw = 3;
+  a.N = N; a.Ho = H; a.Wo = W; a.Cout = C; a.M = N * H * W;
+  a.Hl = H; a.Wl = W; a.smul = 1; a.rmul = -1; a.off = 1; a.sdiv = 1;
+  a.mask = y; a.mscale = scale; a.mshift = shift; a.live_ch = classes;
+  a.dv_ctot = make_fastdiv(a.Ctot); a.dv_kw = make_fastdiv(a.kw);
+  a.bnb_mean = mean; a.bnb_rstd = rstd; a.ssum = sums; a.ssq = sums + C; a.srep = nrep; a.sstride = 2 * C;
+  if (conv_route(a, -1).k != kConvHeadDgrad) return fail("uwm_op_head_dgrad_bn: the launch does not route to conv_head_dgrad_kernel");
+  if (!apply_only) {
+    HIPCHK(hipMemsetAsync(sums, 0, (size_t)nrep * 2 * C * sizeof(double), st));
+    LCHK(launch_conv(a, st));
+  }
+  if (xmax) HIPCHK(hipMemsetAsync(xmax, 0, 32 * sizeof(float), st));
+  LCHK(launch_conv_head_dgrad_apply(a, gamma, dy, dgamma, dbeta, xmax, st));
+  return 0;
+}
 int uwm_op_wgrad(const uwm_src* s0, const uwm_src* s1, const float* dy, int N, int Ho, int Wo, int Cout, int wrows, int Kpad,
                  int kh, int kw, int stride, int pad, float* dw, int force_igemm, uwm_stream stream) {
   if (!s0 || !dy || !dw) return fail("uwm_op_wgrad: null argument");
diff --git a/unet-watermark_amd/csrc/uwm_backward.inc b/unet-watermark_amd/csrc/uwm_backward.inc
--- a/unet-watermark_amd/csrc/uwm_backward.inc
+++ b/unet-watermark_amd/csrc/uwm_backward.inc
@@ -43,14 +43,17 @@
     LCHK(run_wgrad(c, m->head, d4, nullptr, dlogits, H, W));
     LCHK(launch_colsum(dlogits, (size_t)N * H * W, hd.CoutP, m->grads + hd.bias_off, (double*)c.F(p.colsum_scr), st));
     bool head_sums = false;
+    ConvArgs ha; memset(&ha, 0, sizeof(ha));
     LCHK(run_dgrad(c, m->head, dlogits, H, W, H, W, c.F(p.g[last_c2]), nullptr, d4.ptr, d4.scale, d4.shift, nullptr,
-                   m->convs[last_c2].bn, &head_sums));
+                   m->convs[last_c2].bn, &head_sums, nullptr, (d4.relu && d4.scale) ? &ha : nullptr));
+    const bool head_applied = ha.N > 0;
+    if (head_applied) LCHK(run_head_bn_apply(c, last_c2, ha, c.F(p.g[last_c2])));
     int h = H, w = W;
     bool c2_sums = head_sums;
     for (int i = (int)m->dec.size() - 1; i >= 0; --i) {
       const DecL& dl = m->dec[i];
       const size_t npix = (size_t)N * h * w;
-      LCHK(run_bn_bwd(c, dl.c2, c.F(p.g[dl.c2]), c.F(p.g[dl.c2]), npix, c2_sums));
+      if (!(head_applied && dl.c2 == last_c2)) LCHK(run_bn_bwd(c, dl.c2, c.F(p.g[dl.c2]), c.F(p.g[dl.c2]), npix, c2_sums));
       c2_sums = false;
       Src a1 = lazy_src(c, dl.c1, h, w);
       LCHK(run_wgrad(c, dl.c2, a1, nullptr, c.F(p.g[dl.c2]), h, w));
@@ -96,7 +99,7 @@
         const int nh = H >> nd.lvl, nw = W >> nd.lvl;
         const size_t npix = (size_t)N * nh * nw;
         if (!ginit[5 + i]) return fail("internal: UnetPlusPlus node %d has no consumer", i);
-        LCHK(run_bn_bwd(c, nd.c2, c.F(p.g[nd.c2]), c.F(p.g[nd.c2]), npix, i == (int)m->nodes.size() - 1 && head_sums));
+        if (!(head_applied && nd.c2 == last_c2)) LCHK(run_bn_bwd(c, nd.c2, c.F(p.g[nd.c2]), c.F(p.g[nd.c2]), npix, i == (int)m->nodes.size() - 1 && head_sums));
         Src a1 = lazy_src(c, nd.c1, nh, nw);
         LCHK(run_wgrad(c, nd.c2, a1, nullptr, c.F(p.g[nd.c2]), nh, nw));
         bool c1_sums = false;
diff --git a/unet-watermark_amd/csrc/uwm_kernels.h b/unet-watermark_amd/csrc/uwm_kernels.h
--- a/unet-watermark_amd/csrc/uwm_kernels.h
+++ b/unet-watermark_amd/csrc/uwm_kernels.h
@@ -106,6 +106,69 @@
   const int sw = (row >> 1) & 7;
   *(uwm_u2*)(rb + (((unit >> 1) ^ sw) << 4) + (unit & 1) * 8) = hi;
   *(uwm_u2*)(rb + ((((unit >> 1) + 4) ^ sw) << 4) + (unit & 1) * 8) = lo;
+}
+__device__ __forceinline__ void bn_bwd_fold_load(const double* __restrict__ rep, int nrep, int rep_stride, int C, int half, int q0,
+                                                 double (&b)[4]) {
+  const int Q = C >> 2;
+  const int nq = Q < 256 ? Q : 256, L = 256 / nq;
+  const int j = threadIdx.x % nq, l = threadIdx.x / nq;
+#pragma unroll
+  for (int e = 0; e < 4; ++e) b[e] = 0.0;
+  if (l < L) {
+    const int cj = ((q0 + j) % Q) * 4 + half * C;
+    for (int r = l; r < nrep; r += L) {
+      const double* pr = rep + (size_t)r * rep_stride + cj;
+      b[0] += pr[0]; b[1] += pr[1]; b[2] += pr[2]; b[3] += pr[3];
+    }
+  }
+}
+__device__ __forceinline__ void bn_bwd_fold_finish(const double (&b)[4], int nrep, int C, double* part, double (&sq)[4]) {
+  const int Q = C >> 2;
+  const int nq = Q < 256 ? Q : 256, L = 256 / nq;
+  const int j = threadIdx.x % nq, l = threadIdx.x / nq;
+  if (l < L) {
+    double* o = part + (l * nq + j) * 4;
+    o[0] = b[0]; o[1] = b[1]; o[2] = b[2]; o[3] = b[3];
+  }
+  __syncthreads();
+#pragma unroll
+  for (int e = 0; e < 4; ++e) sq[e] = 0.0;
+  const int Lu = L < nrep ? L : nrep;
+  for (int k = 0; k < Lu; ++k) {
+    const double* o = part + (k * nq + j) * 4;
+#pragma unroll
+    for (int e = 0; e < 4; ++e) sq[e] += o[e];
+  }
+}
+__device__ __forceinline__ void bn_bwd_fold_finish_both(const double (&b0)[4], const double (&b1)[4], int nrep, int C, double* part,
+                                                        double* res, double (&s0)[4], double (&s1)[4]) {
+  const int nq = C >> 2, L = 256 / nq;
+  const int j = threadIdx.x % nq, l = threadIdx.x / nq;
+  if (l < L) {
+    double* o = part + (l * nq + j) * 4;
+    o[0] = b0[0]; o[1] = b0[1]; o[2] = b0[2]; o[3] = b0[3];
+    o += 256 * 4;
+    o[0] = b1[0]; o[1] = b1[1]; o[2] = b1[2]; o[3] = b1[3];
+  }
+  __syncthreads();
+  const int Lu = L < nrep ? L : nrep, t = threadIdx.x;
+  if (t < 2 * nq * 4) {
+    const int half = t / (nq * 4), r = t - half * nq * 4;
+    const double* o = part + half * 256 * 4 + r;
+    double s = 0.0;
+    for (int k = 0; k < Lu; ++k) s += o[k * nq * 4];
+    res[t] = s;
+  }
+  __syncthreads();
+#pragma unroll
+  for (int e = 0; e < 4; ++e) { s0[e] = res[j * 4 + e]; s1[e] = res[nq * 4 + j * 4 + e]; }
+}
+__device__ __forceinline__ void bn_bwd_fold_replicas(const double* __restrict__ rep, int nrep, int rep_stride, int C, int half, int q0,
+                                                     double* part, double (&sq)[4]) {
+  double b[4];
+  bn_bwd_fold_load(rep, nrep, rep_stride, C, half, q0, b);
+  if (half) __syncthreads();
+  bn_bwd_fold_finish(b, nrep, C, part, sq);
 }
 #endif
 
@@ -217,6 +280,8 @@
 hipError_t launch_conv_head(const ConvArgs& a, hipStream_t st);
 bool conv_head_dgrad_applicable(const ConvArgs& a);
 hipError_t launch_conv_head_dgrad(const ConvArgs& a, hipStream_t st);
+hipError_t launch_conv_head_dgrad_apply(const ConvArgs& a, const float* gamma, float* dy, float* gamma_grad, float* beta_grad,
+                                        float* xmax, hipStream_t st, hipEvent_t done = nullptr);
 bool conv_wino8_applicable(const ConvArgs& a);
 hipError_t launch_conv_wino8(const ConvArgs& a, hipStream_t st);
 size_t wino_weights_floats(int wrows, int Ctot);
diff --git a/unet-watermark_amd/csrc/uwm_launch.inc b/unet-watermark_amd/csrc/uwm_launch.inc
--- a/unet-watermark_amd/csrc/uwm_launch.inc
+++ b/unet-watermark_amd/csrc/uwm_launch.inc
@@ -84,7 +84,8 @@
 struct UpSplit { float* gprev; int C0; const float* pmask; const float* pscale; const float* pshift; int accumulate = 0; };
 static hipError_t run_dgrad(const Ctx& c, int ci, const float* dy, int Ho, int Wo, int Hin, int Win, float* dx,
                             const float* addend, const float* mask, const float* mscale, const float* mshift,
-                            const UpSplit* us = nullptr, int bn_fuse = -1, bool* fused = nullptr, const float* bn_y = nullptr) {
+                            const UpSplit* us = nullptr, int bn_fuse = -1, bool* fused = nullptr, const float* bn_y = nullptr,
+                            ConvArgs* head_apply = nullptr) {
   const ConvL& cv = c.m->convs[ci];
   ConvArgs a; memset(&a, 0, sizeof(a));
   a.s0 = mk_src(dy, cv.CoutP, Ho, Wo); a.s1 = a.s0; a.C0 = cv.CoutP; a.Ctot = cv.CoutP;
@@ -127,6 +128,14 @@
   }
   if (!fused || !*fused) a.bnb_y = nullptr;
   a.route_n = c.m->route_n;
+  if (head_apply) {
+    static const bool no_head_apply = dbg_flag("UWM_NO_HEAD_APPLY");
+    head_apply->N = 0;
+    if (fused && *fused && !no_head_apply && !us && !addend && mask && mscale && mshift && conv_route(a, -1).k == kConvHeadDgrad) {
+      a.out = nullptr;
+      *head_apply = a;
+    }
+  }
   return route_rec(c, "dgrad", ci, launch_conv(a, c.st));
 }
 
@@ -182,16 +191,22 @@
                         f + 2 * b.C, f + 3 * b.C, b.C, eps, c.st);
 }
 
-static hipError_t run_bn_bwd(const Ctx& c, int ci, const float* g, float* dy, size_t npix, bool sums_fused = false) {
-  uwm_model* m = c.m; const ConvL& cv = m->convs[ci]; const BNL& b = m->bns[cv.bn];
-  const float* f = c.F(b.f_off); const float* y = c.F(m->plan.y[ci]);
-  double* dg = c.D(b.d_off); double* db = c.D(b.d_off) + b.C;
+static hipEvent_t disp_event(const Ctx& c) {
+  uwm_model* m = c.m;
   hipEvent_t done = nullptr;
   if (c.wst && c.wst != c.st && m->ev_disp && m->disp_fork) {
     hipStreamCaptureStatus cs = hipStreamCaptureStatusNone;
     if (hipStreamIsCapturing(c.st, &cs) != hipSuccess) { cs = hipStreamCaptureStatusNone; (void)hipGetLastError(); }
     if (cs == hipStreamCaptureStatusNone) done = m->ev_disp;
   }
+  return done;
+}
+
+static hipError_t run_bn_bwd(const Ctx& c, int ci, const float* g, float* dy, size_t npix, bool sums_fused = false) {
+  uwm_model* m = c.m; const ConvL& cv = m->convs[ci]; const BNL& b = m->bns[cv.bn];
+  const float* f = c.F(b.f_off); const float* y = c.F(m->plan.y[ci]);
+  double* dg = c.D(b.d_off); double* db = c.D(b.d_off) + b.C;
+  hipEvent_t done = disp_event(c);
   hipError_t e = hipSuccess;
   float* xmax = dy_max_needed(m, (size_t)ci) ? (float*)c.D(b.xmax_off()) : nullptr;
   if (sums_fused)
@@ -203,6 +218,16 @@
     e = launch_bn_bwd_apply(g, y, f, f + b.C, m->params + b.g_off, dg, db, dy, m->grads + b.g_off, m->grads + b.b_off,
                             npix, b.C, c.st, nullptr, 0, 0, done, xmax);
   }
+  if (e == hipSuccess && done) m->disp_cov.push_back(dy);
+  if (e == hipSuccess && xmax) m->dy_max_made[cv.bn] = 1;
+  return e;
+}
+
+static hipError_t run_head_bn_apply(const Ctx& c, int ci, const ConvArgs& ha, float* dy) {
+  uwm_model* m = c.m; const ConvL& cv = m->convs[ci]; const BNL& b = m->bns[cv.bn];
+  hipEvent_t done = disp_event(c);
+  float* xmax = dy_max_needed(m, (size_t)ci) ? (float*)c.D(b.xmax_off()) : nullptr;
+  const hipError_t e = launch_conv_head_dgrad_apply(ha, m->params + b.g_off, dy, m->grads + b.g_off, m->grads + b.b_off, xmax, c.st, done);
   if (e == hipSuccess && done) m->disp_cov.push_back(dy);
   if (e == hipSuccess && xmax) m->dy_max_made[cv.bn] = 1;
   return e;
diff --git a/unet-watermark_amd/csrc/uwm_route.hip b/unet-watermark_amd/csrc/uwm_route.hip
--- a/unet-watermark_amd/csrc/uwm_route.hip
+++ b/unet-watermark_amd/csrc/uwm_route.hip
@@ -22,7 +22,7 @@
 struct RouteSwitches {
   bool trace = dbg_flag("UWM_TRACE_CONV");
   bool no_up2 = dbg_flag("UWM_NO_UP2"), no_up2_wgrad = dbg_flag("UWM_NO_UP2_WGRAD"), no_head = dbg_flag("UWM_NO_CONV_HEAD");
-  bool no_bnb_y = dbg_flag("UWM_NO_BNB_Y"), no_igemm_bnb = dbg_flag("UWM_NO_IGEMM_BNB");
+  bool no_bnb_y = dbg_flag("UWM_NO_BNB_Y"), no_igemm_bnb = dbg_flag("UWM_NO_IGEMM_BNB"), no_f16x3_split_bnb = dbg_flag("UWM_NO_F16X3_SPLIT_BNB");
   bool no_narrow_1x1 = dbg_flag("UWM_NO_NARROW_1X1"), no_wgrad_ig16 = dbg_flag("UWM_NO_WGRAD_IG16");
 };
 static const RouteSwitches& switches() { static const RouteSwitches s; return s; }
@@ -32,7 +32,7 @@
   switch (k) {
     case kConvWino:         return {true, true, true, true};
     case kConvWinoX3:       return {true, false, true, true};
-    case kConvF16x3:        return {true, true, true, false};
+    case kConvF16x3:        return {true, true, true, true};
     case kConvUp2Dgrad: case kConvUp2DgradF16: return {true, false, true, true};
     case kConvF16x3v2: case kConvGemm: case kConvS2Dgrad: case kConvIgemm: return {true, true, false, false};
     case kConvC16F16: case kConvC32F16: case kConvPatch16: case kConvHeadDgrad: return {true, false, false, false};
@@ -105,7 +105,7 @@
 bool conv_epilogue_carries_bnb(const ConvArgs& a) {
   const ConvKernel k = conv_route(a, -1).k;
   const ConvCaps c = conv_caps(k);
-  if (a.out_up) return c.bnb_out_up && !a.bnb_y;
+  if (a.out_up) return c.bnb_out_up && !a.bnb_y && !(k == kConvF16x3 && switches().no_f16x3_split_bnb);
   if (a.bnb_y) return c.bnb_y && a.prec != 1 && !switches().no_bnb_y;
   if (switches().no_igemm_bnb && (k == kConvGemm || k == kConvS2Dgrad || k == kConvIgemm)) return false;
   return c.bnb;
```
